# johndpope/SPEAK-hack

Measured on NVIDIA B200. Metric: irfd_train_pairs_per_sec_256, higher is better.
Workload: dtype bf16

## Files before the change

### include/irfd_b200.h

```cpp
#ifndef IRFD_B200_H_
#define IRFD_B200_H_

#include <stddef.h>
#include <stdint.h>

#ifdef __cplusplus
extern "C" {
#endif

#define IRFD_ABI_VERSION 1

#define IRFD_OK 0
#define IRFD_ERR_INVALID_ARGUMENT (-1)
#define IRFD_ERR_CUDA (-2)

typedef struct CUstream_st* irfd_stream_t;

int irfd_abi_version(void);
const char* irfd_last_error(void);

int irfd_conv_gemm_m_tiles(int n, int h, int w);
int irfd_conv_gemm(const void* x, int n, int h, int w, int cin, const void* wk, int cout, int ksize, void* out,
                   void* out2, int mode, const float* bias, const float* nw, const float* noise, const float* sp1,
                   const float* s1, float* stat_sum, float* stat_sq, int force_block_n, irfd_stream_t stream);

int irfd_conv_gemm_style_split(const void* x, int n, int h, int w, int cin, const void* wk, int cout, int ksize,
                               void* out_a, void* out_y, void* out_y_lo, const float* bias, const float* nw,
                               const float* noise, const float* sp1, const float* s1, int force_block_n,
                               irfd_stream_t stream);

int irfd_conv_gemm_grouped(const void* x, int n, int h, int w, int cin, const void* wk, int cout, int ksize, void* out,
                           int mode, float* stat_sum, float* stat_sq, int wgroups, int a_shared, int force_block_n,
                           irfd_stream_t stream);
int irfd_conv_gemm_affine_grouped(const void* x, int n, int h, int w, int cin, const void* wk, int cout, int ksize,
                                  void* out, const float* scale, const float* shift, const void* res, int relu,
                                  int wgroups, int a_shared, int force_block_n, irfd_stream_t stream);

int irfd_conv_gemm_affine(const void* x, int n, int h, int w, int cin, const void* wk, int cout, int ksize, void* out,
                          const float* scale, const float* shift, const void* res, int relu, int force_block_n,
                          irfd_stream_t stream);

long long irfd_wgrad_workspace_bytes(int n, int h, int w, int cin, int cout, int ksize);
int irfd_conv_wgrad(const void* x, const void* dy, int n, int h, int w, int cin, int cout, int ksize, float* dw,
                    float beta, int reduce_cin, int reduce_taps, void* workspace, long long workspace_bytes,
                    irfd_stream_t stream);
long long irfd_wgrad_workspace_bytes_grouped(int n, int h, int w, int cin, int cout, int ksize, int groups);
int irfd_conv_wgrad_grouped(const void* x, const void* dy, int n, int h, int w, int cin, int cout, int ksize,
                            float* const* dw, float beta, int reduce_cin, int reduce_taps, int groups, int x_shared,
                            void* workspace, long long workspace_bytes, irfd_stream_t stream);

int irfd_bn_finalize(const float* psum, const float* psq, int tiles, int c, long long count, float eps, float momentum,
                     float* mean, float* rstd, float* running_mean, float* running_var, int running_updates,
                     int groups, irfd_stream_t stream);
int irfd_bn_eval_rstd(const float* running_var, float eps, float* rstd, int c, irfd_stream_t stream);
int irfd_bn_eval_affine(const float* running_mean, const float* running_var, const float* gamma, const float* beta,
                        float eps, float* scale, float* shift, int c, irfd_stream_t stream);
int irfd_bn_running_update(const float* mean, const float* rstd, float eps, long long count, float momentum,
                           float* running_mean, float* running_var, int c, irfd_stream_t stream);
int irfd_bn_apply(const void* z, const float* mean, const float* rstd, const float* gamma, const float* beta,
                  const void* res, const float* mean2, const float* rstd2, const float* gamma2, const float* beta2,
                  void* out, long long rows, int c, int relu, int groups, irfd_stream_t stream);
long long irfd_bn_bwd_workspace_bytes(long long rows, int c, int groups);
int irfd_bn_backward(const void* g1, const void* g2, const void* act, const void* z, const float* mean,
                     const float* rstd, const float* gamma, const float* beta, void* dz, void* g_out, float* dgamma,
                     float* dbeta, float grad_beta, int batch_stats, long long rows, int c, int groups, void* workspace,
                     long long workspace_bytes, irfd_stream_t stream);

int irfd_bn_eval_affine_sets(const float* const* running_mean, const float* const* running_var,
                             const float* const* gamma, const float* const* beta, float eps, float* scale, float* shift,
                             int c, int nsets, irfd_stream_t stream);
int irfd_bn_finalize_sets(const float* psum, const float* psq, int tiles, int c, long long count, float eps,
                          float momentum, float* mean, float* rstd, float* const* running_mean,
                          float* const* running_var, int running_updates, int groups, int nsets,
                          irfd_stream_t stream);
int irfd_bn_apply_sets(const void* z, const float* mean, const float* rstd, const float* const* gamma,
                       const float* const* beta, const void* res, const float* mean2, const float* rstd2,
                       const float* const* gamma2, const float* const* beta2, void* out, void* mask_bits,
                       long long rows, int c, int relu, int groups, int nsets, irfd_stream_t stream);
int irfd_bn_backward_sets(const void* g1, const void* g2, const void* act, int act_is_bits, const void* z,
                          const float* mean, const float* rstd, const float* const* gamma, const float* const* beta,
                          void* dz, void* g_out, float* const* dgamma, float* const* dbeta, float grad_beta,
                          int batch_stats, long long rows, int c, int groups, int nsets, void* workspace,
                          long long workspace_bytes, irfd_stream_t stream);

int irfd_conv_gemm_bnbwd_grouped(const void* x, int n, int h, int w, int cin, const void* wk, int cout, int ksize,
                                 void* out, const void* bn_z, const float* bn_mean, const float* bn_rstd,
                                 const float* const* bn_gamma, const float* const* bn_beta, float* partial,
                                 int stat_groups, int wgroups, int force_block_n, irfd_stream_t stream);
int irfd_conv_gemm_bnbwd_res_grouped(const void* x, int n, int h, int w, int cin, const void* wk, int cout, int ksize,
                                     void* out, const void* bn_z, const float* bn_mean, const float* bn_rstd,
                                     const void* g2, const void* mask_bits, float* partial, int stat_groups,
                                     int wgroups, int force_block_n, irfd_stream_t stream);
int irfd_bn_backward_finish_sets(const void* g, const void* z, const float* mean, const float* rstd,
                                 const float* const* gamma, void* dz, float* const* dgamma, float* const* dbeta,
                                 float grad_beta, int batch_stats, long long rows, int c, int groups, int nsets,
                                 const float* partial, int tiles, void* workspace, long long workspace_bytes,
                                 irfd_stream_t stream);

int irfd_pack_conv_weight(const float* w, void* dst, int o, int i, int taps, int mode, int kpad, irfd_stream_t stream);
int irfd_im2col_stem(const float* x, void* col, int n, int h, int w, int kpad, irfd_stream_t stream);
int irfd_im2col_3x3s2(const void* a, void* col, int n, int h, int w, int c, irfd_stream_t stream);
int irfd_col2im_3x3s2(const void* dcol, void* dx, int n, int h, int w, int c, irfd_stream_t stream);
int irfd_subsample2(const void* a, void* out, int n, int h, int w, int c, irfd_stream_t stream);
int irfd_scatter_add_s2(const void* a, const void* b, void* out, int n, int h, int w, int c, irfd_stream_t stream);
int irfd_maxpool_fwd(const void* a, void* out, void* argmax, int n, int h, int w, int c, irfd_stream_t stream);
int irfd_maxpool_bwd(const void* dout, const void* dout2, const void* argmax, void* dx, int n, int h, int w, int c,
                     irfd_stream_t stream);
int irfd_avgpool_fwd(const void* a, float* out, int n, int hw, int c, irfd_stream_t stream);
int irfd_avgpool_bwd(const float* dfeat, void* g, int n, int hw, int c, irfd_stream_t stream);
int irfd_nchw_to_nhwc_bf16(const float* in, void* out, int b, int c, int hw, int c_pad, irfd_stream_t stream);
int irfd_nhwc_bf16_to_nchw(const void* in, float* out, int b, int c, int hw, int c_pad, irfd_stream_t stream);

int irfd_const_input_fwd(const float* cst, const float* bias, const float* nw, const float* noise, const float* sp1,
                         const float* s1, void* a0, void* y0, int b, int c, irfd_stream_t stream);
int irfd_const_input_bwd(const void* dy, const void* a0, const float* noise, const float* sp1, float* dsp1, float* ds1,
                         float* dconst, float* dbias, float* dnw, int b, int c, irfd_stream_t stream);
int irfd_upsample2x_fwd(const void* in, void* out, int b, int h, int w, int c, irfd_stream_t stream);
int irfd_upsample2x_split_fwd(const void* in, const void* in_lo, void* out, int b, int h, int w, int c,
                              irfd_stream_t stream);
int irfd_const_input_split_fwd(const float* cst, const float* bias, const float* nw, const float* noise,
                               const float* sp1, const float* s1, void* a0, void* y0, void* y0_lo, int b, int c,
                               irfd_stream_t stream);
int irfd_upsample2x_bwd(const void* dout, void* din, int b, int h, int w, int c, irfd_stream_t stream);
int irfd_apply_noise_nchw(const float* x, const float* w, const float* noise, float* out, int b, int c, int hw,
                          irfd_stream_t stream);
int irfd_apply_style_nchw(const float* x, const float* style, float* out, int b, int c, int hw, irfd_stream_t stream);
long long irfd_style_bwd_workspace_bytes(int b, int hw, int c);
int irfd_style_bwd(const void* dy, const void* a, const float* noise, const float* sp1, void* dz, float* ds1,
                   float* dsp1, float* dbias, float* dnw, int b, int hw, int c, void* workspace,
                   long long workspace_bytes, irfd_stream_t stream);
int irfd_to_rgb_fwd(const void* y, const float* w, const float* bias, float* out, int b, int hw, int c,
                    irfd_stream_t stream);
long long irfd_to_rgb_bwd_workspace_bytes(int b, int hw, int c);
int irfd_to_rgb_bwd(const float* drgb, const void* y, const float* w, void* dy, float* dw, float* dbias, int b, int hw,
                    int c, void* workspace, long long workspace_bytes, irfd_stream_t stream);

int irfd_linear_fwd(const float* x, const float* w, const float* bias, float* y, int b, int n, int k, float wmul,
                    float bmul, int lrelu, irfd_stream_t stream);
int irfd_lrelu_bwd(const float* dy, const float* y, float* dz, long long n, irfd_stream_t stream);
int irfd_linear_bwd(const float* dz, const float* x, const float* w, float* dx, float dx_beta, float* dw, float* db,
                    float dw_beta, int b, int n, int k, float wmul, float bmul, irfd_stream_t stream);
int irfd_softmax_rows(const float* x, float* y, int b, int n, irfd_stream_t stream);
int irfd_scale_copy(const float* src, float* dst, float scale, long long n, irfd_stream_t stream);
int irfd_split_style(const float* style, float* sp1, float* s1, int b, int c, irfd_stream_t stream);
int irfd_merge_style_grad(const float* dsp1, const float* ds1, float* dstyle, int b, int c, irfd_stream_t stream);

int irfd_style_rows_fwd(const float* w, const float* w2, const int* ctrl, int ctrl_idx, float psi, int cutoff,
                        float* rows_t, int l, int b, int k, irfd_stream_t stream);
int irfd_style_rows_pair_fwd(const float* w, const float* w2, const int* ctrl, int ctrl_idx, float psi, int cutoff,
                             float* rows_t, int l, int b, int k, int b_first, irfd_stream_t stream);
int irfd_style_rows_bwd(const float* drows_t, float psi, int cutoff, float* dw, int l, int b, int k,
                        irfd_stream_t stream);
int irfd_swap_cat_fwd(const float* fi_s, const float* fe_s, const float* fp_s, const float* fi_t, const float* fe_t,
                      const float* fp_t, const int* ctrl, float* gen_s, float* gen_t, int b, int c,
                      irfd_stream_t stream);
int irfd_swap_cat_bwd(const float* dgen_s, const float* dgen_t, const int* ctrl, float* dfi_s, float* dfe_s,
                      float* dfp_s, float* dfi_t, float* dfe_t, float* dfp_t, int b, int c, irfd_stream_t stream);

long long irfd_reduce_workspace_bytes(void);
int irfd_mse_fwd(const float* a, const float* b, long long n, float* out, float out_beta, void* workspace,
                 long long workspace_bytes, irfd_stream_t stream);
int irfd_mse_bwd(const float* a, const float* b, long long n, const float* gscale, float* da, float* db,
                 irfd_stream_t stream);
int irfd_sumsq(const float* g, long long n, float* out, float out_beta, void* workspace, long long workspace_bytes,
               irfd_stream_t stream);
int irfd_adam_step(float* p, const float* g, float* m, float* v, long long n, float lr, float beta1, float beta2,
                   float eps, int step, int* step_dev, const float* total_sumsq, float max_norm, irfd_stream_t stream);

int irfd_from_rgb_fwd(const float* x, const float* w, const float* bias, void* out, int b, int hw, int c, int lrelu,
                      irfd_stream_t stream);
long long irfd_bias_lrelu_bwd_workspace_bytes(long long rows, int c);
int irfd_bias_lrelu_bwd(const void* g, const void* y, void* dz, float* dbias, long long rows, int c, void* workspace,
                        long long workspace_bytes, irfd_stream_t stream);

#ifdef __cplusplus
}
#endif
#endif
```

### speak_hack_b200/csrc/conv_gemm.cu

```cuda
#include <stdlib.h>

#include "host_util.h"
#include "ptx.cuh"

namespace irfd {

enum { EPI_PLAIN = 0, EPI_STATS = 1, EPI_STYLE = 2, EPI_AFFINE = 3, EPI_BNBWD = 4, EPI_BNBWD_RES = 5 };

struct ConvGemmArgs {
  int M_total, N_total;
  int num_m_tiles, num_n_tiles;
  int taps, kw, pad, cin_chunks;
  int H, W, HW, B;
  const float* bias;
  const float* nw;
  const float* noise;
  const float* sp1;
  const float* s1;
  float* stat_sum;
  float* stat_sq;
  const __nv_bfloat16* res;
  __nv_bfloat16* y_lo;
  int wg_tiles;
  int a_mod_tiles;
  int relu;
  const __nv_bfloat16* bn_z;
  const __nv_bfloat16* bn_g2;
  const uint8_t* bn_bits;
  const float* bn_mean;
  const float* bn_rstd;
  const float* bn_gamma[4];
  const float* bn_beta[4];
  int sg_tiles;
  int warp_epi;
};

constexpr int kNumThreads = 320;
constexpr int kEpiThreads = 256;
constexpr int kMiscBytes = 12 * 1024;
constexpr int kStgBytes = 16384;
constexpr int kSmemLimit = 232448;

template <int BLOCK_N, int MODE>
struct GemmCfg {
  static constexpr int A_BYTES = 128 * 128;
  static constexpr int B_BYTES = BLOCK_N * 128;
  static constexpr int STAGE_BYTES = A_BYTES + B_BYTES;
  static constexpr int NUM_OUT = (MODE == EPI_STYLE) ? 2 : 1;
  static constexpr int STG_TOTAL = 4 * kStgBytes;
  static constexpr int RAW_STAGES = (kSmemLimit - 1024 - STG_TOTAL - kMiscBytes) / STAGE_BYTES;
  static constexpr int STAGES = RAW_STAGES > 8 ? 8 : RAW_STAGES;
  static constexpr int SMEM_BYTES = 1024 + STAGES * STAGE_BYTES + STG_TOTAL + kMiscBytes;
  static constexpr uint32_t TMEM_COLS = (2 * BLOCK_N <= 128) ? 128 : (2 * BLOCK_N <= 256 ? 256 : 512);
};

template <int BLOCK_N, int MODE, int NBUF>
__device__ __forceinline__ void epilogue_acc(const ConvGemmArgs& p, const CUtensorMap* map_out,
                                             const CUtensorMap* map_out2, uint32_t tmem_base, uint32_t acc_col,
                                             int m0, int n_tile, uint64_t* release_bar, uint8_t* stg_base, float* vec,
                                             uint32_t& chunk_counter) {
  const int warp = threadIdx.x >> 5;
  const int lane = threadIdx.x & 31;
  const int e = warp - 2;
  const int q = warp & 3;
  const int half = e >> 2;
  const int etid = threadIdx.x - 64;
  const int r = q * 32 + lane;
  float* vb = vec;
  float* vnw = vec + 256;
  float* vsp1 = vec + 512;
  float* vs1 = vec + 1024;
  const int m_tile = m0 >> 7;
  const int ng0 = n_tile * BLOCK_N;
  const int pg0 = (m_tile / p.wg_tiles) * p.N_total + ng0;
  float noise_r = 0.f;
  int img_local = 0;
  if constexpr (MODE == EPI_STYLE) {
    const int nimg = p.HW < 128 ? 128 / p.HW : 1;
    const int b0 = m0 / p.HW;
    for (int i = etid; i < BLOCK_N; i += kEpiThreads) {
      vb[i] = p.bias[ng0 + i];
      vnw[i] = p.nw[ng0 + i];
    }
    for (int i = etid; i < nimg * BLOCK_N; i += kEpiThreads) {
      const int img = i / BLOCK_N, c = i - img * BLOCK_N;
      int bb = b0 + img;
      if (bb >= p.B) bb = p.B - 1;
      vsp1[img * 256 + c] = p.sp1[(size_t)bb * p.N_total + ng0 + c];
      vs1[img * 256 + c] = p.s1[(size_t)bb * p.N_total + ng0 + c];
    }
    named_bar_sync(1, kEpiThreads);
    if (m0 + r < p.M_total) noise_r = p.noise[m0 + r];
    img_local = p.HW < 128 ? r / p.HW : 0;
  } else if constexpr (MODE == EPI_PLAIN) {
    if (p.bias != nullptr) {
      for (int i = etid; i < BLOCK_N; i += kEpiThreads) vb[i] = p.bias[pg0 + i];
      named_bar_sync(1, kEpiThreads);
    }
  } else if constexpr (MODE == EPI_AFFINE) {
    for (int i = etid; i < BLOCK_N; i += kEpiThreads) {
      vb[i] = p.bias[pg0 + i];
      vnw[i] = p.nw[pg0 + i];
    }
    named_bar_sync(1, kEpiThreads);
  }
#pragma unroll 1
  for (int chunk = 0; chunk < BLOCK_N / 64; ++chunk, ++chunk_counter) {
    uint32_t v[32];
    uint32_t zw[16];
    uint32_t gw[16];
    uint8_t bw[16];
    if constexpr (MODE == EPI_BNBWD || MODE == EPI_BNBWD_RES) {
      const size_t cell0 = (size_t)(m0 + (etid >> 5) * 16) * p.N_total + ng0 + chunk * 64 + 2 * (etid & 31);
#pragma unroll
      for (int i = 0; i < 16; ++i) {
        zw[i] = __ldg(reinterpret_cast<const uint32_t*>(p.bn_z + cell0 + (size_t)i * p.N_total));
        if constexpr (MODE == EPI_BNBWD_RES) {
          gw[i] = __ldg(reinterpret_cast<const uint32_t*>(p.bn_g2 + cell0 + (size_t)i * p.N_total));
          bw[i] = __ldg(p.bn_bits + ((cell0 + (size_t)i * p.N_total) >> 3));
        }
      }
    }
    const uint32_t taddr = tmem_base + (uint32_t(q * 32) << 16) + acc_col + chunk * 64 + half * 32;
    tmem_ld32(taddr, v);
    tmem_ld_wait();
    if (chunk == BLOCK_N / 64 - 1 && release_bar != nullptr) {
      tc_fence_before();
      __syncwarp();
      if (lane == 0) mbar_arrive(release_bar);
    }
    const int buf = (NBUF == 2) ? (chunk_counter & 1) : 0;
    uint8_t* stg0 = stg_base + buf * kStgBytes;
    uint8_t* stg1 = stg_base + (NBUF + buf) * kStgBytes;
    if (warp == 2) {
      __syncwarp();
      if (elect_one_sync()) tma_store_wait_read<NBUF - 1>();
    }
    named_bar_sync(1, kEpiThreads);
    const int cbase = chunk * 64 + half * 32;
#pragma unroll
    for (int jj = 0; jj < 4; ++jj) {
      float o[8], o2[8];
      float rres[8];
      if constexpr (MODE == EPI_AFFINE) {
        if (p.res != nullptr && m0 + r < p.M_total) {
          const uint4 u = *reinterpret_cast<const uint4*>(p.res + (size_t)(m0 + r) * p.N_total + ng0 + cbase + jj * 8);
          const float2 a0 = unpack_bf16x2(u.x), a1 = unpack_bf16x2(u.y), a2 = unpack_bf16x2(u.z), a3 = unpack_bf16x2(u.w);
          rres[0] = a0.x; rres[1] = a0.y; rres[2] = a1.x; rres[3] = a1.y;
          rres[4] = a2.x; rres[5] = a2.y; rres[6] = a3.x; rres[7] = a3.y;
        } else {
#pragma unroll
          for (int t = 0; t < 8; ++t) rres[t] = 0.f;
        }
      }
#pragma unroll
      for (int t = 0; t < 8; ++t) {
        const int c = cbase + jj * 8 + t;
        float acc = __uint_as_float(v[jj * 8 + t]);
        if constexpr (MODE == EPI_STYLE) {
          float z = acc + vb[c] + vnw[c] * noise_r;
          float a = z > 0.f ? z : 0.2f * z;
          o[t] = a;
          o2[t] = a * vsp1[img_local * 256 + c] + vs1[img_local * 256 + c];
        } else if constexpr (MODE == EPI_PLAIN) {
          o[t] = (p.bias != nullptr) ? acc + vb[c] : acc;
        } else if constexpr (MODE == EPI_AFFINE) {
          const float y = acc * vnw[c] + vb[c] + rres[t];
          o[t] = p.relu == 1 ? fmaxf(y, 0.f) : (p.relu == 2 ? (y > 0.f ? y : 0.2f * y) : y);
        } else {
          o[t] = acc;
        }
      }
      const int j = half * 4 + jj;
      const int phys = j ^ (r & 7);
      uint4 pk;
      pk.x = pack_bf16x2(o[0], o[1]);
      pk.y = pack_bf16x2(o[2], o[3]);
      pk.z = pack_bf16x2(o[4], o[5]);
      pk.w = pack_bf16x2(o[6], o[7]);
      *reinterpret_cast<uint4*>(stg0 + r * 128 + phys * 16) = pk;
      if constexpr (MODE == EPI_STYLE) {
        uint4 pk2;
        pk2.x = pack_bf16x2(o2[0], o2[1]);
        pk2.y = pack_bf16x2(o2[2], o2[3]);
        pk2.z = pack_bf16x2(o2[4], o2[5]);
        pk2.w = pack_bf16x2(o2[6], o2[7]);
        *reinterpret_cast<uint4*>(stg1 + r * 128 + phys * 16) = pk2;
        if (p.y_lo != nullptr && m0 + r < p.M_total) {
          const float2 h0 = unpack_bf16x2(pk2.x), h1 = unpack_bf16x2(pk2.y), h2 = unpack_bf16x2(pk2.z),
                       h3 = unpack_bf16x2(pk2.w);
          uint4 lo;
          lo.x = pack_bf16x2(o2[0] - h0.x, o2[1] - h0.y);
          lo.y = pack_bf16x2(o2[2] - h1.x, o2[3] - h1.y);
          lo.z = pack_bf16x2(o2[4] - h2.x, o2[5] - h2.y);
          lo.w = pack_bf16x2(o2[6] - h3.x, o2[7] - h3.y);
          *reinterpret_cast<uint4*>(p.y_lo + (size_t)(m0 + r) * p.N_total + ng0 + cbase + jj * 8) = lo;
        }
      }
    }
    fence_proxy_async_smem();
    named_bar_sync(1, kEpiThreads);
    if constexpr (MODE == EPI_BNBWD || MODE == EPI_BNBWD_RES) {
      const int pr = etid & 31;
      const int g = etid >> 5;
      const int cc = ng0 + chunk * 64 + 2 * pr;
      const size_t so = (size_t)(m_tile / p.sg_tiles) * p.N_total + cc;
      const float2 mm = __ldg(reinterpret_cast<const float2*>(p.bn_mean + so));
      const float2 rs = __ldg(reinterpret_cast<const float2*>(p.bn_rstd + so));
      float2 ga = make_float2(0.f, 0.f), be = make_float2(0.f, 0.f);
      if constexpr (MODE == EPI_BNBWD) {
        const int grp = m_tile / p.wg_tiles;
        const float* gam =
            grp == 0 ? p.bn_gamma[0] : (grp == 1 ? p.bn_gamma[1] : (grp == 2 ? p.bn_gamma[2] : p.bn_gamma[3]));
        const float* bet = grp == 0 ? p.bn_beta[0] : (grp == 1 ? p.bn_beta[1] : (grp == 2 ? p.bn_beta[2] : p.bn_beta[3]));
        ga = __ldg(reinterpret_cast<const float2*>(gam + cc));
        be = __ldg(reinterpret_cast<const float2*>(bet + cc));
      }
      const int bit0 = (2 * pr) & 7;
      float s0 = 0.f, s1 = 0.f, q0 = 0.f, q1 = 0.f;
#pragma unroll
      for (int i = 0; i < 16; ++i) {
        const int row = g * 16 + i;
        const int phys = (pr >> 2) ^ (row & 7);
        uint32_t* cell = reinterpret_cast<uint32_t*>(stg0 + row * 128 + phys * 16 + (pr & 3) * 4);
        float2 f = unpack_bf16x2(*cell);
        const float2 z = unpack_bf16x2(zw[i]);
        const float x0 = (z.x - mm.x) * rs.x, x1 = (z.y - mm.y) * rs.y;
        if constexpr (MODE == EPI_BNBWD) {
          f.x = (ga.x * x0 + be.x) > 0.f ? f.x : 0.f;
          f.y = (ga.y * x1 + be.y) > 0.f ? f.y : 0.f;
        } else {
          const float2 h = unpack_bf16x2(gw[i]);
          f.x = ((bw[i] >> bit0) & 1) ? f.x + h.x : 0.f;
          f.y = ((bw[i] >> (bit0 + 1)) & 1) ? f.y + h.y : 0.f;
        }
        *cell = pack_bf16x2(f.x, f.y);
        s0 += f.x;
        q0 += f.x * x0;
        s1 += f.y;
        q1 += f.y * x1;
      }
      float* red = vec;
      red[(g * 64 + 2 * pr) * 2 + 0] = s0;
      red[(g * 64 + 2 * pr) * 2 + 1] = q0;
      red[(g * 64 + 2 * pr + 1) * 2 + 0] = s1;
      red[(g * 64 + 2 * pr + 1) * 2 + 1] = q1;
      fence_proxy_async_smem();
      named_bar_sync(1, kEpiThreads);
      if (warp == 2) {
        __syncwarp();
        if (elect_one_sync()) {
          tma_store_2d(map_out, stg0, ng0 + chunk * 64, m0);
          tma_store_commit();
        }
      }
      if (etid < 128) {
        const int ch = etid & 63, which = etid >> 6;
        float acc = 0.f;
#pragma unroll
        for (int gg = 0; gg < 8; ++gg) acc += red[(gg * 64 + ch) * 2 + which];
        p.stat_sum[((size_t)m_tile * 2 + which) * p.N_total + ng0 + chunk * 64 + ch] = acc;
      }
      continue;
    }
    if (warp == 2) {
      __syncwarp();
      if (elect_one_sync()) {
        tma_store_2d(map_out, stg0, ng0 + chunk * 64, m0);
        if constexpr (MODE == EPI_STYLE) tma_store_2d(map_out2, stg1, ng0 + chunk * 64, m0);
        tma_store_commit();
      }
    }
    if constexpr (MODE == EPI_STATS) {
      const int pr = etid & 31;
      const int g = etid >> 5;
      float s0 = 0.f, s1 = 0.f, q0 = 0.f, q1 = 0.f;
#pragma unroll
      for (int i = 0; i < 16; ++i) {
        const int row = g * 16 + i;
        const int phys = (pr >> 2) ^ (row & 7);
        const uint32_t w = *reinterpret_cast<const uint32_t*>(stg0 + row * 128 + phys * 16 + (pr & 3) * 4);
        const float2 f = unpack_bf16x2(w);
        s0 += f.x;
        q0 += f.x * f.x;
        s1 += f.y;
        q1 += f.y * f.y;
      }
      float* red = vec;
      red[(g * 64 + 2 * pr) * 2 + 0] = s0;
      red[(g * 64 + 2 * pr) * 2 + 1] = q0;
      red[(g * 64 + 2 * pr + 1) * 2 + 0] = s1;
      red[(g * 64 + 2 * pr + 1) * 2 + 1] = q1;
      named_bar_sync(1, kEpiThreads);
      if (etid < 128) {
        const int ch = etid & 63, which = etid >> 6;
        float acc = 0.f;
#pragma unroll
        for (int gg = 0; gg < 8; ++gg) acc += red[(gg * 64 + ch) * 2 + which];
        float* dst = which ? p.stat_sq : p.stat_sum;
        dst[(size_t)m_tile * p.N_total + ng0 + chunk * 64 + ch] = acc;
      }
    }
  }
}

constexpr int kSlabBytes = 4096;

template <int BLOCK_N, int MODE>
__device__ __forceinline__ void epilogue_tile_warp(const ConvGemmArgs& p, const CUtensorMap* map_slab, uint32_t tmem_base,
                                                   uint32_t acc_col, int m0, int n_tile, uint64_t* release_bar,
                                                   uint8_t* stg_base, float* vec, uint32_t& chunk_counter,
                                                   uint32_t& my_slabs, bool release_at_leader = false) {
  static_assert(MODE != EPI_STYLE, "STYLE keeps the two-output epilogue");
  auto release = [&]() {
    if (release_at_leader) mbar_arrive_cluster(release_bar, 0);
    else mbar_arrive(release_bar);
  };
  constexpr int CHUNKS = BLOCK_N / 64;
  constexpr bool kSums = MODE == EPI_STATS || MODE == EPI_BNBWD || MODE == EPI_BNBWD_RES;
  const int warp = threadIdx.x >> 5;
  const int lane = threadIdx.x & 31;
  const int e = warp - 2;
  const int q = warp & 3;
  const int h = e >> 2;
  const int m_tile = m0 >> 7;
  const int ng0 = n_tile * BLOCK_N;
  const int pg0 = (m_tile / p.wg_tiles) * p.N_total + ng0;
  const int row = m0 + q * 32 + lane;
  uint8_t* slabs = stg_base + e * 2 * kSlabBytes;
  float* wvec = vec + e * 128;
  const int first = (h - (int)chunk_counter) & 1;
  const int last_mine = first < CHUNKS ? first + 2 * ((CHUNKS - 1 - first) / 2) : -1;
  if (last_mine < 0) {
    __syncwarp();
    if (lane == 0) release();
  }
#pragma unroll 1
  for (int chunk = first; chunk < CHUNKS; chunk += 2) {
    const int cg0 = ng0 + chunk * 64;
    uint32_t zw[32], gw[32];
    uint8_t bw[32];
    if constexpr (MODE == EPI_BNBWD || MODE == EPI_BNBWD_RES) {
      const size_t cell0 = (size_t)(m0 + q * 32) * p.N_total + cg0 + 2 * lane;
#pragma unroll
      for (int i = 0; i < 32; ++i) {
        zw[i] = __ldg(reinterpret_cast<const uint32_t*>(p.bn_z + cell0 + (size_t)i * p.N_total));
        if constexpr (MODE == EPI_BNBWD_RES) {
          gw[i] = __ldg(reinterpret_cast<const uint32_t*>(p.bn_g2 + cell0 + (size_t)i * p.N_total));
          bw[i] = __ldg(p.bn_bits + ((cell0 + (size_t)i * p.N_total) >> 3));
        }
      }
    }
    if constexpr (MODE == EPI_AFFINE || MODE == EPI_PLAIN) {
      if (MODE == EPI_AFFINE || p.bias != nullptr) {
        __syncwarp();
        wvec[lane] = MODE == EPI_AFFINE ? p.nw[pg0 + chunk * 64 + lane] : 0.f;
        wvec[lane + 32] = MODE == EPI_AFFINE ? p.nw[pg0 + chunk * 64 + 32 + lane] : 0.f;
        wvec[64 + lane] = p.bias[pg0 + chunk * 64 + lane];
        wvec[96 + lane] = p.bias[pg0 + chunk * 64 + 32 + lane];
        __syncwarp();
      }
    }
    uint32_t va[32], vb[32];
    const uint32_t taddr = tmem_base + (uint32_t(q * 32) << 16) + acc_col + chunk * 64;
    tmem_ld32(taddr, va);
    tmem_ld32(taddr + 32, vb);
    tmem_ld_wait();
    if (chunk == last_mine) {
      tc_fence_before();
      __syncwarp();
      if (lane == 0) release();
    }
    uint8_t* slab = slabs + (my_slabs & 1) * kSlabBytes;
    if (lane == 0) tma_store_wait_read<1>();
    __syncwarp();
#pragma unroll
    for (int j = 0; j < 8; ++j) {
      float o[8];
#pragma unroll
      for (int t = 0; t < 8; ++t) {
        const int c = j * 8 + t;
        const float acc = __uint_as_float(c < 32 ? va[c & 31] : vb[c & 31]);
        if constexpr (MODE == EPI_AFFINE) o[t] = acc * wvec[c] + wvec[64 + c];
        else if constexpr (MODE == EPI_PLAIN) o[t] = p.bias != nullptr ? acc + wvec[64 + c] : acc;
        else o[t] = acc;
      }
      if constexpr (MODE == EPI_AFFINE) {
        if (p.res != nullptr && row < p.M_total) {
          const uint4 u = *reinterpret_cast<const uint4*>(p.res + (size_t)row * p.N_total + cg0 + j * 8);
          const float2 a0 = unpack_bf16x2(u.x), a1 = unpack_bf16x2(u.y), a2 = unpack_bf16x2(u.z), a3 = unpack_bf16x2(u.w);
          o[0] += a0.x; o[1] += a0.y; o[2] += a1.x; o[3] += a1.y;
          o[4] += a2.x; o[5] += a2.y; o[6] += a3.x; o[7] += a3.y;
        }
#pragma unroll
        for (int t = 0; t < 8; ++t)
          o[t] = p.relu == 1 ? fmaxf(o[t], 0.f) : (p.relu == 2 ? (o[t] > 0.f ? o[t] : 0.2f * o[t]) : o[t]);
      }
      uint4 pk;
      pk.x = pack_bf16x2(o[0], o[1]);
      pk.y = pack_bf16x2(o[2], o[3]);
      pk.z = pack_bf16x2(o[4], o[5]);
      pk.w = pack_bf16x2(o[6], o[7]);
      *reinterpret_cast<uint4*>(slab + lane * 128 + ((j ^ (lane & 7)) << 4)) = pk;
    }
    if constexpr (kSums) {
      __syncwarp();
      float s0 = 0.f, s1 = 0.f, q0 = 0.f, q1 = 0.f;
      if constexpr (MODE == EPI_STATS) {
#pragma unroll
        for (int i = 0; i < 32; ++i) {
          const uint32_t w = *reinterpret_cast<const uint32_t*>(slab + i * 128 + (((lane >> 2) ^ (i & 7)) << 4) + (lane & 3) * 4);
          const float2 f = unpack_bf16x2(w);
          s0 += f.x;
          q0 += f.x * f.x;
          s1 += f.y;
          q1 += f.y * f.y;
        }
      } else {
        const int cc = cg0 + 2 * lane;
        const size_t so = (size_t)(m_tile / p.sg_tiles) * p.N_total + cc;
        const float2 mm = __ldg(reinterpret_cast<const float2*>(p.bn_mean + so));
        const float2 rs = __ldg(reinterpret_cast<const float2*>(p.bn_rstd + so));
        float2 ga = make_float2(0.f, 0.f), be = make_float2(0.f, 0.f);
        if constexpr (MODE == EPI_BNBWD) {
          const int grp = m_tile / p.wg_tiles;
          const float* gam =
              grp == 0 ? p.bn_gamma[0] : (grp == 1 ? p.bn_gamma[1] : (grp == 2 ? p.bn_gamma[2] : p.bn_gamma[3]));
          const float* bet = grp == 0 ? p.bn_beta[0] : (grp == 1 ? p.bn_beta[1] : (grp == 2 ? p.bn_beta[2] : p.bn_beta[3]));
          ga = __ldg(reinterpret_cast<const float2*>(gam + cc));
          be = __ldg(reinterpret_cast<const float2*>(bet + cc));
        }
        const int bit0 = (2 * lane) & 7;
#pragma unroll
        for (int i = 0; i < 32; ++i) {
          uint32_t* cell = reinterpret_cast<uint32_t*>(slab + i * 128 + (((lane >> 2) ^ (i & 7)) << 4) + (lane & 3) * 4);
          float2 f = unpack_bf16x2(*cell);
          const float2 z = unpack_bf16x2(zw[i]);
          const float x0 = (z.x - mm.x) * rs.x, x1 = (z.y - mm.y) * rs.y;
          if constexpr (MODE == EPI_BNBWD) {
            f.x = (ga.x * x0 + be.x) > 0.f ? f.x : 0.f;
            f.y = (ga.y * x1 + be.y) > 0.f ? f.y : 0.f;
          } else {
            const float2 g2 = unpack_bf16x2(gw[i]);
            f.x = ((bw[i] >> bit0) & 1) ? f.x + g2.x : 0.f;
            f.y = ((bw[i] >> (bit0 + 1)) & 1) ? f.y + g2.y : 0.f;
          }
          *cell = pack_bf16x2(f.x, f.y);
          s0 += f.x;
          q0 += f.x * x0;
          s1 += f.y;
          q1 += f.y * x1;
        }
      }
      float* red = vec + ((((my_slabs & 1) * 2 + h) * 4 + q) * 64) * 2;
      *reinterpret_cast<float4*>(red + 4 * lane) = make_float4(s0, q0, s1, q1);
    }
    fence_proxy_async_smem();
    __syncwarp();
    if (lane == 0) {
      tma_store_2d(map_slab, slab, cg0, m0 + q * 32);
      tma_store_commit();
    }
    if constexpr (kSums) {
      named_bar_sync(1 + h, 128);
      if (q == 0) {
        const float* r0 = vec + ((((my_slabs & 1) * 2 + h) * 4) * 64) * 2 + 4 * lane;
        float4 t = *reinterpret_cast<const float4*>(r0);
#pragma unroll
        for (int k = 1; k < 4; ++k) {
          const float4 u = *reinterpret_cast<const float4*>(r0 + k * 128);
          t.x += u.x;
          t.y += u.y;
          t.z += u.z;
          t.w += u.w;
        }
        if constexpr (MODE == EPI_STATS) {
          const size_t d = (size_t)m_tile * p.N_total + cg0 + 2 * lane;
          *reinterpret_cast<float2*>(p.stat_sum + d) = make_float2(t.x, t.z);
          *reinterpret_cast<float2*>(p.stat_sq + d) = make_float2(t.y, t.w);
        } else {
          const size_t d = (size_t)m_tile * 2 * p.N_total + cg0 + 2 * lane;
          *reinterpret_cast<float2*>(p.stat_sum + d) = make_float2(t.x, t.z);
          *reinterpret_cast<float2*>(p.stat_sum + d + p.N_total) = make_float2(t.y, t.w);
        }
      }
    }
    ++my_slabs;
  }
  chunk_counter += CHUNKS;
}

template <int BLOCK_N, int MODE, int CL = 1, bool MMA2 = false>
__global__ void __launch_bounds__(kNumThreads, 1)
conv_gemm_kernel(const __grid_constant__ CUtensorMap map_a, const __grid_constant__ CUtensorMap map_b,
                 const __grid_constant__ CUtensorMap map_out, const __grid_constant__ CUtensorMap map_out2,
                 const ConvGemmArgs p) {
  using Cfg = GemmCfg<BLOCK_N, MODE>;
  constexpr int STAGES = Cfg::STAGES;
  static_assert(STAGES >= 2, "pipeline too shallow");
  static_assert(!MMA2 || (CL == 2 && MODE != EPI_STYLE), "the 2-SM MMA needs a CTA pair and the per-warp epilogue");

  extern __shared__ uint8_t smem_raw[];
  uint8_t* smem = reinterpret_cast<uint8_t*>((reinterpret_cast<uintptr_t>(smem_raw) + 1023) & ~uintptr_t(1023));
  uint8_t* stg_base = smem + STAGES * Cfg::STAGE_BYTES;
  uint8_t* misc = stg_base + Cfg::STG_TOTAL;
  float* vec = reinterpret_cast<float*>(misc);
  uint64_t* full_bar = reinterpret_cast<uint64_t*>(misc + 8192);
  uint64_t* empty_bar = full_bar + STAGES;
  uint64_t* tmem_full = empty_bar + STAGES;
  uint64_t* tmem_empty = tmem_full + 2;
  uint32_t* tmem_ptr = reinterpret_cast<uint32_t*>(tmem_empty + 2);

  const int warp = threadIdx.x >> 5;
  const int lane = threadIdx.x & 31;
  const int crank = CL > 1 ? (int)cluster_ctarank() : 0;
  const int unit0 = blockIdx.x / CL, unit_step = gridDim.x / CL;
  const int total_units = (p.num_m_tiles / CL) * p.num_n_tiles;
  const int num_kb = p.taps * p.cin_chunks;
  constexpr uint16_t kClusterMask = (1u << CL) - 1;

  if (threadIdx.x == 0) {
    for (int i = 0; i < STAGES; ++i) {
      mbar_init(&full_bar[i], 1);
      mbar_init(&empty_bar[i], MMA2 ? 1 : CL);
    }
    for (int i = 0; i < 2; ++i) {
      mbar_init(&tmem_full[i], 1);
      mbar_init(&tmem_empty[i], MMA2 ? 16 : 8);
    }
    fence_mbar_init();
  }
  __syncwarp();
  if (warp == 0) {
    if (MMA2) tmem_alloc_2sm<Cfg::TMEM_COLS>(tmem_ptr);
    else tmem_alloc<Cfg::TMEM_COLS>(tmem_ptr);
  }
  tc_fence_before();
  __syncthreads();
  if (CL > 1) cluster_sync_all();
  tc_fence_after();
  const uint32_t tmem_base = *tmem_ptr;

  if (warp == 0) {
    {
      if (lane == 0) {
        tma_prefetch_desc(&map_a);
        tma_prefetch_desc(&map_b);
      }
      __syncwarp();
      int stage = 0;
      uint32_t phase = 0;
      for (int unit = unit0; unit < total_units; unit += unit_step) {
        const int m_tile = (unit / p.num_n_tiles) * CL + crank;
        const int n_tile = unit % p.num_n_tiles;
        const int m0 = (p.a_mod_tiles > 0 ? m_tile % p.a_mod_tiles : m_tile) * 128;
        const int w0 = m0 % p.W;
        const int h0 = (m0 / p.W) % p.H;
        const int n0 = m0 / (p.W * p.H);
        const int b_row = (m_tile / p.wg_tiles) * p.N_total + n_tile * BLOCK_N;
        for (int tap = 0; tap < p.taps; ++tap) {
          const int dh = tap / p.kw - p.pad;
          const int dw = tap % p.kw - p.pad;
          for (int ch = 0; ch < p.cin_chunks; ++ch) {
            mbar_wait(&empty_bar[stage], phase ^ 1);
            uint8_t* sa = smem + stage * Cfg::STAGE_BYTES;
            if (MMA2) {
              if (elect_one_sync()) {
                if (crank == 0) mbar_expect_tx(&full_bar[stage], 2 * (Cfg::A_BYTES + Cfg::B_BYTES / 2));
                tma_load_4d_2sm(sa, &map_a, &full_bar[stage], ch * 64, w0 + dw, h0 + dh, n0);
                tma_load_2d_2sm(sa + Cfg::A_BYTES, &map_b, &full_bar[stage], (tap * p.cin_chunks + ch) * 64,
                                b_row + crank * (BLOCK_N / 2));
              }
            } else if (elect_one_sync()) {
              mbar_expect_tx(&full_bar[stage], Cfg::STAGE_BYTES);
              tma_load_4d(sa, &map_a, &full_bar[stage], ch * 64, w0 + dw, h0 + dh, n0);
              if (CL == 1)
                tma_load_2d(sa + Cfg::A_BYTES, &map_b, &full_bar[stage], (tap * p.cin_chunks + ch) * 64, b_row);
              else
                tma_load_2d_mc(sa + Cfg::A_BYTES + crank * (Cfg::B_BYTES / CL), &map_b, &full_bar[stage],
                               (tap * p.cin_chunks + ch) * 64, b_row + crank * (BLOCK_N / CL), kClusterMask);
            }
            __syncwarp();
            if (++stage == STAGES) {
              stage = 0;
              phase ^= 1;
            }
          }
        }
      }
    }
  } else if (warp == 1) {
    if (!MMA2 || crank == 0) {
      constexpr uint32_t idesc = make_idesc_bf16(MMA2 ? 256 : 128, BLOCK_N, 0, 0);
      int stage = 0;
      uint32_t phase = 0;
      int iter = 0;
      for (int unit = unit0; unit < total_units; unit += unit_step, ++iter) {
        const int as = iter & 1;
        const uint32_t aphase = (iter >> 1) & 1;
        mbar_wait(&tmem_empty[as], aphase ^ 1);
        tc_fence_after();
        const uint32_t d_tmem = tmem_base + as * BLOCK_N;
        for (int kb = 0; kb < num_kb; ++kb) {
          mbar_wait(&full_bar[stage], phase);
          tc_fence_after();
          const uint32_t a_addr = smem_u32(smem + stage * Cfg::STAGE_BYTES);
          const uint64_t adesc0 = make_smem_desc_sw128(a_addr, 0, 1024);
          const uint64_t bdesc0 = make_smem_desc_sw128(a_addr + Cfg::A_BYTES, 0, 1024);
          if (elect_one_sync()) {
#pragma unroll
            for (int k = 0; k < 4; ++k)
              if (MMA2) umma_bf16_2sm(d_tmem, adesc0 + 2 * k, bdesc0 + 2 * k, idesc, (kb | k) != 0 ? 1u : 0u);
              else umma_bf16(d_tmem, adesc0 + 2 * k, bdesc0 + 2 * k, idesc, (kb | k) != 0 ? 1u : 0u);
            if (MMA2) umma_commit_2sm_mc(&empty_bar[stage], kClusterMask);
            else if (CL == 1) umma_commit(&empty_bar[stage]);
            else umma_commit_mc(&empty_bar[stage], kClusterMask);
          }
          __syncwarp();
          if (++stage == STAGES) {
            stage = 0;
            phase ^= 1;
          }
        }
        if (elect_one_sync()) {
          if (MMA2) umma_commit_2sm_mc(&tmem_full[as], kClusterMask);
          else umma_commit(&tmem_full[as]);
        }
        __syncwarp();
      }
    }
  } else {
    int iter = 0;
    uint32_t chunk_counter = 0, my_slabs = 0;
    for (int unit = unit0; unit < total_units; unit += unit_step, ++iter) {
      const int as = iter & 1;
      const uint32_t aphase = (iter >> 1) & 1;
      const int m_tile = (unit / p.num_n_tiles) * CL + crank;
      const int n_tile = unit % p.num_n_tiles;
      mbar_wait(&tmem_full[as], aphase);
      tc_fence_after();
      if constexpr (MODE != EPI_STYLE) {
        if (p.warp_epi) {
          epilogue_tile_warp<BLOCK_N, MODE>(p, &map_out2, tmem_base, as * BLOCK_N, m_tile * 128, n_tile, &tmem_empty[as],
                                            stg_base, vec, chunk_counter, my_slabs, MMA2);
          continue;
        }
      }
      epilogue_acc<BLOCK_N, MODE, 2>(p, &map_out, &map_out2, tmem_base, as * BLOCK_N, m_tile * 128, n_tile,
                                     &tmem_empty[as], stg_base, vec, chunk_counter);
    }
    if (MODE != EPI_STYLE && p.warp_epi) {
      if (lane == 0) tma_store_wait_read<0>();
    } else if (warp == 2) {
      __syncwarp();
      if (elect_one_sync()) tma_store_wait_read<0>();
    }
  }

  tc_fence_before();
  __syncthreads();
  if (CL > 1) cluster_sync_all();
  if (warp == 0) {
    if (MMA2) tmem_dealloc_2sm<Cfg::TMEM_COLS>(tmem_base);
    else tmem_dealloc<Cfg::TMEM_COLS>(tmem_base);
  }
}


constexpr int kHaloThreads = 352;
constexpr int kHaloCols = 130;
constexpr int kHaloRows = 4;

template <int BLOCK_N, int MODE>
struct HaloCfg {
  static_assert(BLOCK_N == 64 || BLOCK_N == 128, "two double-buffered accumulators need 4 x BLOCK_N <= 512 TMEM columns");
  static constexpr int A_BYTES = kHaloRows * kHaloCols * 128;
  static constexpr int A_STAGES = 2;
  static constexpr int B_BYTES = BLOCK_N * 128;
  static constexpr int NUM_OUT = (MODE == EPI_STYLE) ? 2 : 1;
  static constexpr int NBUF = (NUM_OUT == 2) ? 1 : 2;
  static constexpr int STG_TOTAL = NUM_OUT * NBUF * kStgBytes;
  static constexpr int RAW_B = (kSmemLimit - 1024 - A_STAGES * A_BYTES - STG_TOTAL - kMiscBytes) / B_BYTES;
  static constexpr int B_STAGES = RAW_B > 8 ? 8 : RAW_B;
  static constexpr int SMEM_BYTES = 1024 + A_STAGES * A_BYTES + B_STAGES * B_BYTES + STG_TOTAL + kMiscBytes;
  static constexpr uint32_t TMEM_COLS = 4 * BLOCK_N <= 256 ? 256 : 512;
  static_assert(A_BYTES % 1024 == 0 && B_STAGES >= 2, "halo stage must keep 1024-byte alignment");
};

struct HaloArgs {
  int wsegs, hpairs;
  int total_tiles;
};

template <int BLOCK_N, int MODE>
__global__ void __launch_bounds__(kHaloThreads, 1)
conv_halo_kernel(const __grid_constant__ CUtensorMap map_a, const __grid_constant__ CUtensorMap map_b,
                 const __grid_constant__ CUtensorMap map_out, const __grid_constant__ CUtensorMap map_out2,
                 const ConvGemmArgs p, const HaloArgs hp) {
  using Cfg = HaloCfg<BLOCK_N, MODE>;
  constexpr int BST = Cfg::B_STAGES;
  extern __shared__ uint8_t smem_raw[];
  uint8_t* smem = reinterpret_cast<uint8_t*>((reinterpret_cast<uintptr_t>(smem_raw) + 1023) & ~uintptr_t(1023));
  uint8_t* smem_b = smem + Cfg::A_STAGES * Cfg::A_BYTES;
  uint8_t* stg_base = smem_b + BST * Cfg::B_BYTES;
  uint8_t* misc = stg_base + Cfg::STG_TOTAL;
  float* vec = reinterpret_cast<float*>(misc);
  uint64_t* full_a = reinterpret_cast<uint64_t*>(misc + 8192);
  uint64_t* empty_a = full_a + 2;
  uint64_t* full_b = empty_a + 2;
  uint64_t* empty_b = full_b + BST;
  uint64_t* tmem_full = empty_b + BST;
  uint64_t* tmem_empty = tmem_full + 2;
  uint32_t* tmem_ptr = reinterpret_cast<uint32_t*>(tmem_empty + 2);

  const int warp = threadIdx.x >> 5;
  const int lane = threadIdx.x & 31;
  const int chunks = p.cin_chunks;

  if (threadIdx.x == 0) {
    for (int i = 0; i < 2; ++i) {
      mbar_init(&full_a[i], 1);
      mbar_init(&empty_a[i], 1);
      mbar_init(&tmem_full[i], 1);
      mbar_init(&tmem_empty[i], 8);
    }
    for (int i = 0; i < BST; ++i) {
      mbar_init(&full_b[i], 1);
      mbar_init(&empty_b[i], 1);
    }
    fence_mbar_init();
  }
  __syncwarp();
  if (warp == 0) tmem_alloc<Cfg::TMEM_COLS>(tmem_ptr);
  tc_fence_before();
  __syncthreads();
  tc_fence_after();
  const uint32_t tmem_base = *tmem_ptr;

  auto decode = [&](int tile, int& n_tile, int& n0, int& h0, int& w0) {
    const int m2 = tile / p.num_n_tiles;
    n_tile = tile - m2 * p.num_n_tiles;
    const int wseg = m2 % hp.wsegs;
    const int t = m2 / hp.wsegs;
    const int hpair = t % hp.hpairs;
    n0 = t / hp.hpairs;
    h0 = hpair * 2;
    w0 = wseg * 128;
  };

  if (warp == 0) {
    {
      if (lane == 0) tma_prefetch_desc(&map_a);
      __syncwarp();
      int stage = 0;
      uint32_t phase = 0;
      for (int tile = blockIdx.x; tile < hp.total_tiles; tile += gridDim.x) {
        int n_tile, n0, h0, w0;
        decode(tile, n_tile, n0, h0, w0);
        for (int ch = 0; ch < chunks; ++ch) {
          mbar_wait(&empty_a[stage], phase ^ 1);
          if (elect_one_sync()) {
            mbar_expect_tx(&full_a[stage], Cfg::A_BYTES);
            tma_load_4d(smem + stage * Cfg::A_BYTES, &map_a, &full_a[stage], ch * 64, w0 - 1, h0 - 1, n0);
          }
          __syncwarp();
          if (++stage == Cfg::A_STAGES) {
            stage = 0;
            phase ^= 1;
          }
        }
      }
    }
  } else if (warp == 10) {
    {
      if (lane == 0) tma_prefetch_desc(&map_b);
      __syncwarp();
      int stage = 0;
      uint32_t phase = 0;
      for (int tile = blockIdx.x; tile < hp.total_tiles; tile += gridDim.x) {
        const int n_tile = tile % p.num_n_tiles;
        for (int ch = 0; ch < chunks; ++ch) {
          for (int tap = 0; tap < 9; ++tap) {
            mbar_wait(&empty_b[stage], phase ^ 1);
            if (elect_one_sync()) {
              mbar_expect_tx(&full_b[stage], Cfg::B_BYTES);
              tma_load_2d(smem_b + stage * Cfg::B_BYTES, &map_b, &full_b[stage], (tap * chunks + ch) * 64,
                          n_tile * BLOCK_N);
            }
            __syncwarp();
            if (++stage == BST) {
              stage = 0;
              phase ^= 1;
            }
          }
        }
      }
    }
  } else if (warp == 1) {
    {
      constexpr uint32_t idesc = make_idesc_bf16(128, BLOCK_N, 0, 0);
      int sa = 0, sb = 0;
      uint32_t pa = 0, pb = 0;
      int iter = 0;
      for (int tile = blockIdx.x; tile < hp.total_tiles; tile += gridDim.x, ++iter) {
        const int as = iter & 1;
        const uint32_t aphase = (iter >> 1) & 1;
        mbar_wait(&tmem_empty[as], aphase ^ 1);
        tc_fence_after();
        const uint32_t d_tmem = tmem_base + as * 2 * BLOCK_N;
        for (int ch = 0; ch < chunks; ++ch) {
          mbar_wait(&full_a[sa], pa);
          const uint64_t adesc0 = make_smem_desc_sw128(smem_u32(smem + sa * Cfg::A_BYTES), 0, 1024);
#pragma unroll
          for (int tap = 0; tap < 9; ++tap) {
            constexpr int kLine = 128 / 16;
            const int dy = tap / 3, dx = tap % 3;
            mbar_wait(&full_b[sb], pb);
            tc_fence_after();
            const uint64_t bdesc0 = make_smem_desc_sw128(smem_u32(smem_b + sb * Cfg::B_BYTES), 0, 1024);
            if (elect_one_sync()) {
#pragma unroll
              for (int j = 0; j < 2; ++j) {
#pragma unroll
                for (int k = 0; k < 4; ++k)
                  umma_bf16(d_tmem + j * BLOCK_N, adesc0 + ((j + dy) * kHaloCols + dx) * kLine + 2 * k, bdesc0 + 2 * k,
                            idesc, (tap | k) != 0 ? 1u : (ch != 0 ? 1u : 0u));
              }
              umma_commit(&empty_b[sb]);
            }
            __syncwarp();
            if (++sb == BST) {
              sb = 0;
              pb ^= 1;
            }
          }
          if (elect_one_sync()) umma_commit(&empty_a[sa]);
          __syncwarp();
          if (++sa == Cfg::A_STAGES) {
            sa = 0;
            pa ^= 1;
          }
        }
        if (elect_one_sync()) umma_commit(&tmem_full[as]);
        __syncwarp();
      }
    }
  } else {
    int iter = 0;
    uint32_t chunk_counter = 0;
    for (int tile = blockIdx.x; tile < hp.total_tiles; tile += gridDim.x, ++iter) {
      const int as = iter & 1;
      const uint32_t aphase = (iter >> 1) & 1;
      int n_tile, n0, h0, w0;
      decode(tile, n_tile, n0, h0, w0);
      const int m0 = (n0 * p.H + h0) * p.W + w0;
      mbar_wait(&tmem_full[as], aphase);
      tc_fence_after();
      epilogue_acc<BLOCK_N, MODE, Cfg::NBUF>(p, &map_out, &map_out2, tmem_base, as * 2 * BLOCK_N, m0, n_tile, nullptr,
                                             stg_base, vec, chunk_counter);
      epilogue_acc<BLOCK_N, MODE, Cfg::NBUF>(p, &map_out, &map_out2, tmem_base, as * 2 * BLOCK_N + BLOCK_N, m0 + p.W,
                                             n_tile, &tmem_empty[as], stg_base, vec, chunk_counter);
    }
    if (warp == 2) {
      __syncwarp();
      if (elect_one_sync()) tma_store_wait_read<0>();
    }
  }

  tc_fence_before();
  __syncthreads();
  if (warp == 0) tmem_dealloc<Cfg::TMEM_COLS>(tmem_base);
}

template <int BLOCK_N, int MODE, int CL = 1, bool MMA2 = false>
static int launch_conv_gemm(const CUtensorMap& ma, const CUtensorMap& mb, const CUtensorMap& mo, const CUtensorMap& mo2,
                            const ConvGemmArgs& a, cudaStream_t stream) {
  using Cfg = GemmCfg<BLOCK_N, MODE>;
  static bool configured = false;
  auto kern = conv_gemm_kernel<BLOCK_N, MODE, CL, MMA2>;
  if (!configured) {
    cudaError_t e = cudaFuncSetAttribute(kern, cudaFuncAttributeMaxDynamicSharedMemorySize, Cfg::SMEM_BYTES);
    if (e != cudaSuccess) {
      set_last_error("cudaFuncSetAttribute(smem=%d): %s", Cfg::SMEM_BYTES, cudaGetErrorString(e));
      return IRFD_ERR_CUDA;
    }
    configured = true;
  }
  const int units = (a.num_m_tiles / CL) * a.num_n_tiles;
  const int slots = num_sms() / CL;
  const int grid = (units < slots ? units : slots) * CL;
  if (CL == 1) {
    kern<<<grid, kNumThreads, Cfg::SMEM_BYTES, stream>>>(ma, mb, mo, mo2, a);
  } else {
    cudaLaunchConfig_t cfg = {};
    cfg.gridDim = dim3(grid);
    cfg.blockDim = dim3(kNumThreads);
    cfg.dynamicSmemBytes = Cfg::SMEM_BYTES;
    cfg.stream = stream;
    cudaLaunchAttribute attr[1];
    attr[0].id = cudaLaunchAttributeClusterDimension;
    attr[0].val.clusterDim.x = CL;
    attr[0].val.clusterDim.y = 1;
    attr[0].val.clusterDim.z = 1;
    cfg.attrs = attr;
    cfg.numAttrs = 1;
    cudaLaunchKernelEx(&cfg, kern, ma, mb, mo, mo2, a);
  }
  IRFD_CHECK_LAUNCH();
  return IRFD_OK;
}

template <int MODE>
static int dispatch_block_n(int block_n, const CUtensorMap& ma, const CUtensorMap& mb, const CUtensorMap& mo,
                            const CUtensorMap& mo2, const ConvGemmArgs& a, cudaStream_t stream, int cluster = 1) {
  if constexpr (MODE == EPI_PLAIN || MODE == EPI_STATS || MODE == EPI_BNBWD) {
    if (cluster == 3) {
      if (block_n == 128) return launch_conv_gemm<128, MODE, 2, true>(ma, mb, mo, mo2, a, stream);
      if (block_n == 256) return launch_conv_gemm<256, MODE, 2, true>(ma, mb, mo, mo2, a, stream);
    }
  }
  if (cluster >= 2) {
    if (block_n == 128) return launch_conv_gemm<128, MODE, 2>(ma, mb, mo, mo2, a, stream);
    if (block_n == 256) return launch_conv_gemm<256, MODE, 2>(ma, mb, mo, mo2, a, stream);
  }
  switch (block_n) {
    case 64: return launch_conv_gemm<64, MODE>(ma, mb, mo, mo2, a, stream);
    case 128: return launch_conv_gemm<128, MODE>(ma, mb, mo, mo2, a, stream);
    case 256: return launch_conv_gemm<256, MODE>(ma, mb, mo, mo2, a, stream);
  }
  set_last_error("bad BLOCK_N %d", block_n);
  return IRFD_ERR_INVALID_ARGUMENT;
}


template <int BLOCK_N, int MODE>
static int launch_conv_halo(const CUtensorMap& ma, const CUtensorMap& mb, const CUtensorMap& mo, const CUtensorMap& mo2,
                            const ConvGemmArgs& a, const HaloArgs& h, cudaStream_t stream) {
  using Cfg = HaloCfg<BLOCK_N, MODE>;
  static bool configured = false;
  auto kern = conv_halo_kernel<BLOCK_N, MODE>;
  if (!configured) {
    cudaError_t e = cudaFuncSetAttribute(kern, cudaFuncAttributeMaxDynamicSharedMemorySize, Cfg::SMEM_BYTES);
    if (e != cudaSuccess) {
      set_last_error("cudaFuncSetAttribute(halo smem=%d): %s", Cfg::SMEM_BYTES, cudaGetErrorString(e));
      return IRFD_ERR_CUDA;
    }
    configured = true;
  }
  const int grid = h.total_tiles < num_sms() ? h.total_tiles : num_sms();
  kern<<<grid, kHaloThreads, Cfg::SMEM_BYTES, stream>>>(ma, mb, mo, mo2, a, h);
  IRFD_CHECK_LAUNCH();
  return IRFD_OK;
}

template <int MODE>
static int dispatch_halo(int block_n, const CUtensorMap& ma, const CUtensorMap& mb, const CUtensorMap& mo,
                         const CUtensorMap& mo2, const ConvGemmArgs& a, const HaloArgs& h, cudaStream_t stream) {
  if (block_n == 64) return launch_conv_halo<64, MODE>(ma, mb, mo, mo2, a, h, stream);
  return launch_conv_halo<128, MODE>(ma, mb, mo, mo2, a, h, stream);
}

static int cluster_mode() {
  const char* e = getenv("IRFD_GEMM_CLUSTER");
  return e ? atoi(e) : 0;
}
static int mma2_mode() {
  const char* e = getenv("IRFD_GEMM_2SM");
  return e ? atoi(e) : 0;
}

static int warp_epi_mode() {
  const char* e = getenv("IRFD_WARP_EPI");
  return e ? atoi(e) : 1;
}

static int halo_mode() {
  const char* e = getenv("IRFD_CONV_HALO");
  return e ? atoi(e) : 1;
}

}

using namespace irfd;

extern "C" int irfd_conv_gemm_m_tiles(int n, int h, int w) {
  long long m = (long long)n * h * w;
  return (int)((m + 127) / 128);
}

struct BnBwdFold {
  const void* z;
  const float *mean, *rstd;
  const float* const* gamma;
  const float* const* beta;
  const void* g2;
  const void* bits;
  int stat_groups;
};

static int conv_gemm_impl(const void* x, int n, int h, int w, int cin, const void* wk, int cout, int ksize, void* out,
                          void* out2, void* out_lo, int mode, const float* bias, const float* nw, const float* noise,
                          const float* sp1, const float* s1, float* stat_sum, float* stat_sq, const void* res, int relu,
                          int force_block_n, cudaStream_t stream, int wgroups = 1, int a_shared = 0,
                          const BnBwdFold* fold = nullptr) {
  IRFD_CHECK_ARG(x && wk && out, "conv_gemm: null pointer");
  IRFD_CHECK_ARG(ksize == 1 || ksize == 3, "conv_gemm: ksize must be 1 or 3 (got %d)", ksize);
  IRFD_CHECK_ARG(cin % 64 == 0 && cin > 0, "conv_gemm: Cin must be a multiple of 64 (got %d)", cin);
  IRFD_CHECK_ARG(cout % 64 == 0 && cout > 0, "conv_gemm: Cout must be a multiple of 64 (got %d)", cout);
  IRFD_CHECK_ARG(mode >= 0 && mode <= 5, "conv_gemm: bad mode %d", mode);
  const long long m_total_ll = (long long)n * h * w;
  IRFD_CHECK_ARG(m_total_ll > 0 && m_total_ll < (1ll << 31) - 256, "conv_gemm: bad pixel count");
  const int m_total = (int)m_total_ll;
  IRFD_CHECK_ARG(wgroups == 1 || (wgroups > 1 && m_total_ll % (128ll * wgroups) == 0),
                 "conv_gemm: %d weight groups need a whole number of 128-pixel tiles per group (pixels %lld)", wgroups,
                 m_total_ll);
  IRFD_CHECK_ARG(wgroups == 1 || (mode != EPI_STYLE), "conv_gemm: weight groups are not available in STYLE mode");
  IRFD_CHECK_ARG(!a_shared || (ksize == 1 && wgroups > 1), "conv_gemm: a shared A operand needs ksize 1 and groups > 1");

  int H = h, W = w, NB = n;
  if (ksize == 1) {
    H = 1;
    W = a_shared ? m_total / wgroups : m_total;
    NB = 1;
  }
  int tw, th, tn;
  if (W >= 128) {
    IRFD_CHECK_ARG(ksize == 1 || W % 128 == 0, "conv_gemm: W=%d must be a multiple of 128", W);
    tw = 128; th = 1; tn = 1;
  } else {
    IRFD_CHECK_ARG(128 % W == 0, "conv_gemm: W=%d must divide 128", W);
    tw = W;
    const int rows = 128 / W;
    if (H >= rows) {
      IRFD_CHECK_ARG(H % rows == 0, "conv_gemm: H=%d must be a multiple of %d", H, rows);
      th = rows; tn = 1;
    } else {
      IRFD_CHECK_ARG(rows % H == 0, "conv_gemm: H=%d must divide %d", H, rows);
      th = H; tn = rows / H;
    }
  }

  ConvGemmArgs a;
  a.M_total = m_total;
  a.N_total = cout;
  a.num_m_tiles = (m_total + 127) / 128;
  a.taps = ksize * ksize;
  a.kw = ksize;
  a.pad = ksize / 2;
  a.cin_chunks = cin / 64;
  a.H = H; a.W = W; a.HW = h * w; a.B = n;
  a.bias = bias; a.nw = nw; a.noise = noise; a.sp1 = sp1; a.s1 = s1;
  a.stat_sum = stat_sum; a.stat_sq = stat_sq;
  a.res = reinterpret_cast<const __nv_bfloat16*>(res);
  a.y_lo = reinterpret_cast<__nv_bfloat16*>(out_lo);
  a.wg_tiles = wgroups > 1 ? a.num_m_tiles / wgroups : 0x7fffffff;
  a.a_mod_tiles = a_shared ? a.num_m_tiles / wgroups : 0;
  a.relu = relu;
  if (mode == EPI_AFFINE) IRFD_CHECK_ARG(bias && nw, "conv_gemm: AFFINE mode needs scale and shift");
  if (mode == EPI_STYLE) {
    IRFD_CHECK_ARG(bias && nw && noise && sp1 && s1 && out2, "conv_gemm: STYLE mode needs bias/nw/noise/sp1/s1/out2");
    IRFD_CHECK_ARG(h * w >= 64, "conv_gemm: STYLE mode needs >= 64 pixels per image");
  }
  if (mode == EPI_STATS) IRFD_CHECK_ARG(stat_sum && stat_sq, "conv_gemm: STATS mode needs stat buffers");
  a.warp_epi = (mode != EPI_STYLE && m_total % 128 == 0 && warp_epi_mode() != 0) ? 1 : 0;
  a.bn_z = nullptr;
  a.bn_mean = a.bn_rstd = nullptr;
  for (int i = 0; i < 4; ++i) a.bn_gamma[i] = a.bn_beta[i] = nullptr;
  a.sg_tiles = 0x7fffffff;
  a.bn_g2 = nullptr;
  a.bn_bits = nullptr;
  if (mode == EPI_BNBWD || mode == EPI_BNBWD_RES) {
    IRFD_CHECK_ARG(fold && fold->z && fold->mean && fold->rstd && stat_sum,
                   "conv_gemm: BNBWD modes need z, mean, rstd and the partial buffer");
    if (mode == EPI_BNBWD) IRFD_CHECK_ARG(fold->gamma && fold->beta, "conv_gemm: BNBWD mode needs gamma and beta");
    if (mode == EPI_BNBWD_RES)
      IRFD_CHECK_ARG(fold->g2 && fold->bits && cout % 8 == 0, "conv_gemm: BNBWD_RES mode needs g2 and the mask plane");
    IRFD_CHECK_ARG(wgroups <= 4 && m_total % 128 == 0 && fold->stat_groups >= wgroups &&
                       fold->stat_groups % wgroups == 0 && a.num_m_tiles % fold->stat_groups == 0,
                   "conv_gemm: BNBWD needs whole 128-pixel tiles per statistic group (%d tiles, %d groups, %d sets)",
                   a.num_m_tiles, fold->stat_groups, wgroups);
    a.bn_z = reinterpret_cast<const __nv_bfloat16*>(fold->z);
    a.bn_mean = fold->mean;
    a.bn_rstd = fold->rstd;
    for (int i = 0; i < wgroups && mode == EPI_BNBWD; ++i) {
      IRFD_CHECK_ARG(fold->gamma[i] && fold->beta[i], "conv_gemm: BNBWD gamma/beta pointer %d is null", i);
      a.bn_gamma[i] = fold->gamma[i];
      a.bn_beta[i] = fold->beta[i];
    }
    a.bn_g2 = reinterpret_cast<const __nv_bfloat16*>(fold->g2);
    a.bn_bits = reinterpret_cast<const uint8_t*>(fold->bits);
    a.sg_tiles = a.num_m_tiles / fold->stat_groups;
  }

  int block_n = force_block_n;
  if (block_n == 0) {
    block_n = 64;
    const int cands[3] = {256, 128, 64};
    for (int i = 0; i < 3; ++i) {
      if (cout % cands[i] == 0 && (long long)a.num_m_tiles * (cout / cands[i]) >= num_sms()) {
        block_n = cands[i];
        break;
      }
    }
    if (block_n == 64 && cout % 128 == 0 && (long long)a.num_m_tiles * (cout / 128) * 3 >= 2ll * num_sms()) block_n = 128;
  }
  IRFD_CHECK_ARG((block_n == 64 || block_n == 128 || block_n == 256) && cout % block_n == 0,
                 "conv_gemm: BLOCK_N %d incompatible with Cout %d", block_n, cout);
  const int hmode = halo_mode();
  const bool use_halo = hmode != 0 && mode != EPI_BNBWD && mode != EPI_BNBWD_RES && wgroups == 1 && ksize == 3 && W % 128 == 0 && H % 2 == 0 &&
                        (cout == 64 || cout == 128) &&
                        (force_block_n == 0 || force_block_n == cout);
  if (use_halo) block_n = cout;
  a.num_n_tiles = cout / block_n;
  int cluster = 1;
  if (!use_halo && (cluster_mode() != 0 || mma2_mode() != 0) && block_n >= 128 && a.num_m_tiles % 2 == 0 &&
      (wgroups == 1 || a.wg_tiles % 2 == 0) && (a.a_mod_tiles == 0 || a.a_mod_tiles % 2 == 0))
    cluster = (mma2_mode() != 0 && a.warp_epi && (mode == EPI_PLAIN || mode == EPI_STATS || mode == EPI_BNBWD)) ? 3 : 2;

  CUtensorMap ma, mb, mo, mo2;
  {
    const uint64_t dims[4] = {(uint64_t)cin, (uint64_t)W, (uint64_t)H, (uint64_t)NB};
    const uint64_t str[3] = {(uint64_t)cin * 2, (uint64_t)W * cin * 2, (uint64_t)H * W * cin * 2};
    uint32_t box[4] = {64, (uint32_t)tw, (uint32_t)th, (uint32_t)tn};
    if (use_halo) {
      box[1] = kHaloCols;
      box[2] = kHaloRows;
      box[3] = 1;
    }
    int rc = make_tmap_bf16(&ma, x, 4, dims, str, box, true);
    if (rc) return rc;
  }
  {
    const uint64_t ktot = (uint64_t)a.taps * cin;
    const uint64_t dims[2] = {ktot, (uint64_t)cout * wgroups};
    const uint64_t str[1] = {ktot * 2};
    const uint32_t box[2] = {64, (uint32_t)(block_n / (cluster > 1 ? 2 : 1))};
    int rc = make_tmap_bf16(&mb, wk, 2, dims, str, box, true);
    if (rc) return rc;
  }
  {
    const uint64_t dims[2] = {(uint64_t)cout, (uint64_t)m_total};
    const uint64_t str[1] = {(uint64_t)cout * 2};
    const uint32_t box[2] = {64, 128};
    int rc = make_tmap_bf16(&mo, out, 2, dims, str, box, true);
    if (rc) return rc;
    if (mode == EPI_STYLE) {
      rc = make_tmap_bf16(&mo2, out2 ? out2 : out, 2, dims, str, box, true);
    } else {
      const uint32_t slab_box[2] = {64, 32};
      rc = make_tmap_bf16(&mo2, out, 2, dims, str, slab_box, true);
    }
    if (rc) return rc;
  }
  if (use_halo) {
    HaloArgs hargs;
    hargs.wsegs = W / 128;
    hargs.hpairs = H / 2;
    hargs.total_tiles = NB * hargs.hpairs * hargs.wsegs * a.num_n_tiles;
    switch (mode) {
      case EPI_PLAIN: return dispatch_halo<EPI_PLAIN>(block_n, ma, mb, mo, mo2, a, hargs, stream);
      case EPI_STATS: return dispatch_halo<EPI_STATS>(block_n, ma, mb, mo, mo2, a, hargs, stream);
      case EPI_STYLE: return dispatch_halo<EPI_STYLE>(block_n, ma, mb, mo, mo2, a, hargs, stream);
      case EPI_AFFINE: return dispatch_halo<EPI_AFFINE>(block_n, ma, mb, mo, mo2, a, hargs, stream);
    }
    return IRFD_ERR_INVALID_ARGUMENT;
  }
  switch (mode) {
    case EPI_PLAIN: return dispatch_block_n<EPI_PLAIN>(block_n, ma, mb, mo, mo2, a, stream, cluster);
    case EPI_STATS: return dispatch_block_n<EPI_STATS>(block_n, ma, mb, mo, mo2, a, stream, cluster);
    case EPI_STYLE: return dispatch_block_n<EPI_STYLE>(block_n, ma, mb, mo, mo2, a, stream, cluster);
    case EPI_AFFINE: return dispatch_block_n<EPI_AFFINE>(block_n, ma, mb, mo, mo2, a, stream, cluster);
    case EPI_BNBWD: return dispatch_block_n<EPI_BNBWD>(block_n, ma, mb, mo, mo2, a, stream, cluster);
    case EPI_BNBWD_RES: return dispatch_block_n<EPI_BNBWD_RES>(block_n, ma, mb, mo, mo2, a, stream, cluster);
  }
  return IRFD_ERR_INVALID_ARGUMENT;
}

extern "C" int irfd_conv_gemm(const void* x, int n, int h, int w, int cin, const void* wk, int cout, int ksize,
                              void* out, void* out2, int mode, const float* bias, const float* nw, const float* noise,
                              const float* sp1, const float* s1, float* stat_sum, float* stat_sq, int force_block_n,
                              cudaStream_t stream) {
  IRFD_CHECK_ARG(mode >= 0 && mode <= 2, "conv_gemm: bad mode %d", mode);
  return conv_gemm_impl(x, n, h, w, cin, wk, cout, ksize, out, out2, nullptr, mode, bias, nw, noise, sp1, s1, stat_sum,
                        stat_sq, nullptr, 0, force_block_n, stream);
}

extern "C" int irfd_conv_gemm_style_split(const void* x, int n, int h, int w, int cin, const void* wk, int cout,
                                          int ksize, void* out_a, void* out_y, void* out_y_lo, const float* bias,
                                          const float* nw, const float* noise, const float* sp1, const float* s1,
                                          int force_block_n, cudaStream_t stream) {
  IRFD_CHECK_ARG(out_y_lo != nullptr, "conv_gemm_style_split: out_y_lo is required");
  return conv_gemm_impl(x, n, h, w, cin, wk, cout, ksize, out_a, out_y, out_y_lo, EPI_STYLE, bias, nw, noise, sp1, s1,
                        nullptr, nullptr, nullptr, 0, force_block_n, stream);
}

extern "C" int irfd_conv_gemm_grouped(const void* x, int n, int h, int w, int cin, const void* wk, int cout, int ksize,
                                      void* out, int mode, float* stat_sum, float* stat_sq, int wgroups, int a_shared,
                                      int force_block_n, cudaStream_t stream) {
  IRFD_CHECK_ARG(mode == EPI_PLAIN || mode == EPI_STATS, "conv_gemm_grouped: mode must be 0 (plain) or 1 (stats)");
  return conv_gemm_impl(x, n, h, w, cin, wk, cout, ksize, out, nullptr, nullptr, mode, nullptr, nullptr, nullptr,
                        nullptr, nullptr, stat_sum, stat_sq, nullptr, 0, force_block_n, stream, wgroups, a_shared);
}

extern "C" int irfd_conv_gemm_bnbwd_grouped(const void* x, int n, int h, int w, int cin, const void* wk, int cout,
                                            int ksize, void* out, const void* bn_z, const float* bn_mean,
                                            const float* bn_rstd, const float* const* bn_gamma,
                                            const float* const* bn_beta, float* partial, int stat_groups, int wgroups,
                                            int force_block_n, cudaStream_t stream) {
  IRFD_CHECK_ARG(wgroups >= 1 && wgroups <= 4, "conv_gemm_bnbwd: 1..4 weight groups");
  const BnBwdFold fold{bn_z, bn_mean, bn_rstd, bn_gamma, bn_beta, nullptr, nullptr, stat_groups};
  return conv_gemm_impl(x, n, h, w, cin, wk, cout, ksize, out, nullptr, nullptr, EPI_BNBWD, nullptr, nullptr, nullptr,
                        nullptr, nullptr, partial, nullptr, nullptr, 0, force_block_n, stream, wgroups, 0, &fold);
}

extern "C" int irfd_conv_gemm_bnbwd_res_grouped(const void* x, int n, int h, int w, int cin, const void* wk, int cout,
                                                int ksize, void* out, const void* bn_z, const float* bn_mean,
                                                const float* bn_rstd, const void* g2, const void* mask_bits,
                                                float* partial, int stat_groups, int wgroups, int force_block_n,
                                                cudaStream_t stream) {
  IRFD_CHECK_ARG(wgroups >= 1 && wgroups <= 4, "conv_gemm_bnbwd_res: 1..4 weight groups");
  const BnBwdFold fold{bn_z, bn_mean, bn_rstd, nullptr, nullptr, g2, mask_bits, stat_groups};
  return conv_gemm_impl(x, n, h, w, cin, wk, cout, ksize, out, nullptr, nullptr, EPI_BNBWD_RES, nullptr, nullptr,
                        nullptr, nullptr, nullptr, partial, nullptr, nullptr, 0, force_block_n, stream, wgroups, 0,
                        &fold);
}

extern "C" int irfd_conv_gemm_affine_grouped(const void* x, int n, int h, int w, int cin, const void* wk, int cout,
                                             int ksize, void* out, const float* scale, const float* shift,
                                             const void* res, int relu, int wgroups, int a_shared, int force_block_n,
                                             cudaStream_t stream) {
  return conv_gemm_impl(x, n, h, w, cin, wk, cout, ksize, out, nullptr, nullptr, EPI_AFFINE, shift, scale, nullptr,
                        nullptr, nullptr, nullptr, nullptr, res, relu, force_block_n, stream, wgroups, a_shared);
}

extern "C" int irfd_conv_gemm_affine(const void* x, int n, int h, int w, int cin, const void* wk, int cout, int ksize,
                                     void* out, const float* scale, const float* shift, const void* res, int relu,
                                     int force_block_n, cudaStream_t stream) {
  return conv_gemm_impl(x, n, h, w, cin, wk, cout, ksize, out, nullptr, nullptr, EPI_AFFINE, shift, scale, nullptr, nullptr,
                        nullptr, nullptr, nullptr, res, relu, force_block_n, stream);
}
```

### speak_hack_b200/csrc/host_util.cu

```cuda
#include "host_util.h"

#include <mutex>
#include <unordered_set>

#include <stdarg.h>
#include <string.h>

namespace irfd {

static thread_local char g_last_error[512] = "";

void set_last_error(const char* fmt, ...) {
  va_list ap;
  va_start(ap, fmt);
  vsnprintf(g_last_error, sizeof(g_last_error), fmt, ap);
  va_end(ap);
}

EncodeTiledFn get_encode_tiled() {
  static EncodeTiledFn fn = nullptr;
  if (fn) return fn;
  void* p = nullptr;
  cudaDriverEntryPointQueryResult qres;
  cudaError_t e = cudaGetDriverEntryPoint("cuTensorMapEncodeTiled", &p, cudaEnableDefault, &qres);
  if (e != cudaSuccess || qres != cudaDriverEntryPointSuccess || p == nullptr) {
    set_last_error("cuTensorMapEncodeTiled entry point unavailable: %s", cudaGetErrorString(e));
    return nullptr;
  }
  fn = reinterpret_cast<EncodeTiledFn>(p);
  return fn;
}

int num_sms() {
  static int n = 0;
  if (n) return n;
  int dev = 0;
  cudaGetDevice(&dev);
  cudaDeviceGetAttribute(&n, cudaDevAttrMultiProcessorCount, dev);
  if (n <= 0) n = 148;
  return n;
}

int make_tmap_bf16(CUtensorMap* out, const void* base, int rank, const uint64_t* dims, const uint64_t* strides_bytes,
                   const uint32_t* box, bool swizzle128) {
  EncodeTiledFn enc = get_encode_tiled();
  if (!enc) return IRFD_ERR_CUDA;
  cuuint64_t gdims[5];
  cuuint64_t gstr[4];
  cuuint32_t gbox[5];
  cuuint32_t estr[5];
  for (int i = 0; i < rank; ++i) {
    gdims[i] = dims[i];
    gbox[i] = box[i];
    estr[i] = 1;
  }
  for (int i = 0; i + 1 < rank; ++i) gstr[i] = strides_bytes[i];
  CUresult r = enc(out, CU_TENSOR_MAP_DATA_TYPE_BFLOAT16, (cuuint32_t)rank, const_cast<void*>(base), gdims, gstr, gbox,
                   estr, CU_TENSOR_MAP_INTERLEAVE_NONE,
                   swizzle128 ? CU_TENSOR_MAP_SWIZZLE_128B : CU_TENSOR_MAP_SWIZZLE_NONE,
                   CU_TENSOR_MAP_L2_PROMOTION_L2_256B, CU_TENSOR_MAP_FLOAT_OOB_FILL_NONE);
  if (r != CUDA_SUCCESS) {
    set_last_error("cuTensorMapEncodeTiled failed (CUresult %d) rank=%d dims=[%llu,%llu,%llu,%llu] box=[%u,%u,%u,%u]",
                   (int)r, rank, (unsigned long long)dims[0], (unsigned long long)(rank > 1 ? dims[1] : 0),
                   (unsigned long long)(rank > 2 ? dims[2] : 0), (unsigned long long)(rank > 3 ? dims[3] : 0), box[0],
                   rank > 1 ? box[1] : 0, rank > 2 ? box[2] : 0, rank > 3 ? box[3] : 0);
    return IRFD_ERR_CUDA;
  }
  return IRFD_OK;
}

}

extern "C" const char* irfd_last_error(void) { return irfd::g_last_error; }

namespace irfd {
void prefer_max_shared_carveout(const void* kernel) {
  static std::mutex mu;
  static std::unordered_set<const void*> done;
  std::lock_guard<std::mutex> lock(mu);
  if (done.insert(kernel).second)
    cudaFuncSetAttribute(kernel, cudaFuncAttributePreferredSharedMemoryCarveout, cudaSharedmemCarveoutMaxShared);
}
}

extern "C" int irfd_abi_version(void) { return IRFD_ABI_VERSION; }
```

### speak_hack_b200/csrc/host_util.h

```cpp
#pragma once
#include <cuda.h>
#include <cuda_runtime.h>
#include <stdint.h>
#include <stdio.h>

#include "../../include/irfd_b200.h"

namespace irfd {

typedef CUresult (*EncodeTiledFn)(CUtensorMap*, CUtensorMapDataType, cuuint32_t, void*, const cuuint64_t*,
                                  const cuuint64_t*, const cuuint32_t*, const cuuint32_t*, CUtensorMapInterleave,
                                  CUtensorMapSwizzle, CUtensorMapL2promotion, CUtensorMapFloatOOBfill);

EncodeTiledFn get_encode_tiled();
int num_sms();
void set_last_error(const char* fmt, ...);

int make_tmap_bf16(CUtensorMap* out, const void* base, int rank, const uint64_t* dims, const uint64_t* strides_bytes,
                   const uint32_t* box, bool swizzle128);

void prefer_max_shared_carveout(const void* kernel);

#define IRFD_CHECK_ARG(cond, ...)            \
  do {                                       \
    if (!(cond)) {                           \
      irfd::set_last_error(__VA_ARGS__);     \
      return IRFD_ERR_INVALID_ARGUMENT;      \
    }                                        \
  } while (0)

#define IRFD_CHECK_LAUNCH()                                                        \
  do {                                                                             \
    cudaError_t e__ = cudaGetLastError();                                          \
    if (e__ != cudaSuccess) {                                                      \
      irfd::set_last_error("%s:%d CUDA launch: %s", __FILE__, __LINE__, cudaGetErrorString(e__)); \
      return IRFD_ERR_CUDA;                                                        \
    }                                                                              \
  } while (0)

}
```

### speak_hack_b200/csrc/ptx.cuh

```cuda
#pragma once
#include <cuda.h>
#include <cuda_runtime.h>
#include <cuda_bf16.h>
#include <stdint.h>

namespace irfd {

__device__ __forceinline__ uint32_t smem_u32(const void* p) {
  return static_cast<uint32_t>(__cvta_generic_to_shared(p));
}
__device__ __forceinline__ uint32_t lane_id() { return threadIdx.x & 31u; }

__device__ __forceinline__ bool elect_one_sync() {
  uint32_t pred;
  asm volatile(
      "{\n\t.reg .pred P;\n\t"
      "elect.sync _|P, 0xffffffff;\n\t"
      "selp.u32 %0, 1, 0, P;\n\t}"
      : "=r"(pred));
  return pred != 0;
}

__device__ __forceinline__ void mbar_init(uint64_t* bar, uint32_t count) {
  asm volatile("mbarrier.init.shared::cta.b64 [%0], %1;" ::"r"(smem_u32(bar)), "r"(count) : "memory");
}
__device__ __forceinline__ void fence_mbar_init() {
  asm volatile("fence.mbarrier_init.release.cluster;" ::: "memory");
}
__device__ __forceinline__ void mbar_expect_tx(uint64_t* bar, uint32_t bytes) {
  asm volatile("mbarrier.arrive.expect_tx.shared::cta.b64 _, [%0], %1;" ::"r"(smem_u32(bar)), "r"(bytes)
               : "memory");
}
__device__ __forceinline__ void mbar_arrive(uint64_t* bar) {
  asm volatile("mbarrier.arrive.shared::cta.b64 _, [%0];" ::"r"(smem_u32(bar)) : "memory");
}
__device__ __forceinline__ bool mbar_try_wait(uint64_t* bar, uint32_t parity) {
  uint32_t ok;
  asm volatile(
      "{\n\t.reg .pred p;\n\t"
      "mbarrier.try_wait.parity.shared::cta.b64 p, [%1], %2;\n\t"
      "selp.u32 %0, 1, 0, p;\n\t}"
      : "=r"(ok)
      : "r"(smem_u32(bar)), "r"(parity)
      : "memory");
  return ok != 0;
}
__device__ __forceinline__ void mbar_wait(uint64_t* bar, uint32_t parity) {
  uint32_t spins = 0;
  long long t0 = 0;
  while (!mbar_try_wait(bar, parity)) {
    if ((++spins & 1023u) == 0) {
      const long long now = clock64();
      if (t0 == 0) t0 = now;
      else if (now - t0 > 4000000000ll) __trap();
    }
  }
}

__device__ __forceinline__ void fence_proxy_async_smem() {
  asm volatile("fence.proxy.async.shared::cta;" ::: "memory");
}
__device__ __forceinline__ void named_bar_sync(uint32_t id, uint32_t nthreads) {
  asm volatile("bar.sync %0, %1;" ::"r"(id), "r"(nthreads) : "memory");
}

__device__ __forceinline__ void tma_prefetch_desc(const CUtensorMap* m) {
  asm volatile("prefetch.tensormap [%0];" ::"l"(reinterpret_cast<uint64_t>(m)) : "memory");
}
__device__ __forceinline__ void tma_load_2d(void* dst, const CUtensorMap* m, uint64_t* bar, int c0, int c1) {
  asm volatile(
      "cp.async.bulk.tensor.2d.shared::cluster.global.tile.mbarrier::complete_tx::bytes [%0], [%1, {%3, %4}], [%2];"
      ::"r"(smem_u32(dst)), "l"(reinterpret_cast<uint64_t>(m)), "r"(smem_u32(bar)), "r"(c0), "r"(c1)
      : "memory");
}
__device__ __forceinline__ void tma_load_2d_mc(void* dst, const CUtensorMap* m, uint64_t* bar, int c0, int c1,
                                               uint16_t cta_mask) {
  asm volatile(
      "cp.async.bulk.tensor.2d.shared::cluster.global.mbarrier::complete_tx::bytes.multicast::cluster [%0], [%1, {%3, %4}], "
      "[%2], %5;" ::"r"(smem_u32(dst)),
      "l"(reinterpret_cast<uint64_t>(m)), "r"(smem_u32(bar)), "r"(c0), "r"(c1), "h"(cta_mask)
      : "memory");
}
__device__ __forceinline__ uint32_t cluster_ctarank() {
  uint32_t r;
  asm volatile("mov.u32 %0, %%cluster_ctarank;" : "=r"(r));
  return r;
}
__device__ __forceinline__ void cluster_sync_all() {
  asm volatile("barrier.cluster.arrive.release.aligned;" ::: "memory");
  asm volatile("barrier.cluster.wait.acquire.aligned;" ::: "memory");
}
__device__ __forceinline__ void tma_load_4d(void* dst, const CUtensorMap* m, uint64_t* bar, int c0, int c1, int c2,
                                            int c3) {
  asm volatile(
      "cp.async.bulk.tensor.4d.shared::cluster.global.tile.mbarrier::complete_tx::bytes [%0], [%1, {%3, %4, %5, %6}], "
      "[%2];" ::"r"(smem_u32(dst)),
      "l"(reinterpret_cast<uint64_t>(m)), "r"(smem_u32(bar)), "r"(c0), "r"(c1), "r"(c2), "r"(c3)
      : "memory");
}
__device__ __forceinline__ void tma_store_2d(const CUtensorMap* m, const void* src, int c0, int c1) {
  asm volatile("cp.async.bulk.tensor.2d.global.shared::cta.tile.bulk_group [%0, {%2, %3}], [%1];" ::"l"(
                   reinterpret_cast<uint64_t>(m)),
               "r"(smem_u32(src)), "r"(c0), "r"(c1)
               : "memory");
}
__device__ __forceinline__ void tma_store_commit() { asm volatile("cp.async.bulk.commit_group;" ::: "memory"); }
template <int N>
__device__ __forceinline__ void tma_store_wait_read() {
  asm volatile("cp.async.bulk.wait_group.read %0;" ::"n"(N) : "memory");
}
template <int N>
__device__ __forceinline__ void tma_store_wait_all() {
  asm volatile("cp.async.bulk.wait_group %0;" ::"n"(N) : "memory");
}

template <uint32_t NCOLS>
__device__ __forceinline__ void tmem_alloc(uint32_t* dst_smem) {
  asm volatile("tcgen05.alloc.cta_group::1.sync.aligned.shared::cta.b32 [%0], %1;" ::"r"(smem_u32(dst_smem)),
               "n"(NCOLS)
               : "memory");
  asm volatile("tcgen05.relinquish_alloc_permit.cta_group::1.sync.aligned;" ::: "memory");
}
template <uint32_t NCOLS>
__device__ __forceinline__ void tmem_dealloc(uint32_t taddr) {
  asm volatile("tcgen05.dealloc.cta_group::1.sync.aligned.b32 %0, %1;" ::"r"(taddr), "n"(NCOLS) : "memory");
}
__device__ __forceinline__ void tc_fence_before() { asm volatile("tcgen05.fence::before_thread_sync;" ::: "memory"); }
__device__ __forceinline__ void tc_fence_after() { asm volatile("tcgen05.fence::after_thread_sync;" ::: "memory"); }

__device__ __forceinline__ void umma_bf16(uint32_t tmem_d, uint64_t adesc, uint64_t bdesc, uint32_t idesc,
                                          uint32_t accumulate) {
  asm volatile(
      "{\n\t.reg .pred p;\n\t"
      "setp.ne.b32 p, %4, 0;\n\t"
      "tcgen05.mma.cta_group::1.kind::f16 [%0], %1, %2, %3, p;\n\t}" ::"r"(tmem_d),
      "l"(adesc), "l"(bdesc), "r"(idesc), "r"(accumulate)
      : "memory");
}
template <uint32_t NCOLS>
__device__ __forceinline__ void tmem_alloc_2sm(uint32_t* dst_smem) {
  asm volatile("tcgen05.alloc.cta_group::2.sync.aligned.shared::cta.b32 [%0], %1;" ::"r"(smem_u32(dst_smem)),
               "n"(NCOLS)
               : "memory");
  asm volatile("tcgen05.relinquish_alloc_permit.cta_group::2.sync.aligned;" ::: "memory");
}
template <uint32_t NCOLS>
__device__ __forceinline__ void tmem_dealloc_2sm(uint32_t taddr) {
  asm volatile("tcgen05.dealloc.cta_group::2.sync.aligned.b32 %0, %1;" ::"r"(taddr), "n"(NCOLS) : "memory");
}
__device__ __forceinline__ void umma_bf16_2sm(uint32_t tmem_d, uint64_t adesc, uint64_t bdesc, uint32_t idesc,
                                              uint32_t accumulate) {
  asm volatile(
      "{\n\t.reg .pred p;\n\t"
      "setp.ne.b32 p, %4, 0;\n\t"
      "tcgen05.mma.cta_group::2.kind::f16 [%0], %1, %2, %3, p;\n\t}" ::"r"(tmem_d),
      "l"(adesc), "l"(bdesc), "r"(idesc), "r"(accumulate)
      : "memory");
}
__device__ __forceinline__ void umma_commit_2sm_mc(uint64_t* bar, uint16_t cta_mask) {
  asm volatile("tcgen05.commit.cta_group::2.mbarrier::arrive::one.shared::cluster.multicast::cluster.b64 [%0], %1;" ::"r"(
                   smem_u32(bar)),
               "h"(cta_mask)
               : "memory");
}
constexpr uint32_t kPeerBitMask = 0xFEFFFFFFu;
__device__ __forceinline__ void tma_load_2d_2sm(void* dst, const CUtensorMap* m, uint64_t* bar, int c0, int c1) {
  asm volatile(
      "cp.async.bulk.tensor.2d.cta_group::2.shared::cluster.global.mbarrier::complete_tx::bytes [%0], [%1, {%3, %4}], [%2];"
      ::"r"(smem_u32(dst)), "l"(reinterpret_cast<uint64_t>(m)), "r"(smem_u32(bar) & kPeerBitMask), "r"(c0), "r"(c1)
      : "memory");
}
__device__ __forceinline__ void tma_load_4d_2sm(void* dst, const CUtensorMap* m, uint64_t* bar, int c0, int c1, int c2,
                                                int c3) {
  asm volatile(
      "cp.async.bulk.tensor.4d.cta_group::2.shared::cluster.global.mbarrier::complete_tx::bytes [%0], [%1, {%3, %4, %5, "
      "%6}], [%2];" ::"r"(smem_u32(dst)),
      "l"(reinterpret_cast<uint64_t>(m)), "r"(smem_u32(bar) & kPeerBitMask), "r"(c0), "r"(c1), "r"(c2), "r"(c3)
      : "memory");
}
__device__ __forceinline__ void mbar_arrive_cluster(uint64_t* bar, uint32_t rank) {
  asm volatile(
      "{\n\t.reg .b32 ra;\n\t"
      "mapa.shared::cluster.u32 ra, %0, %1;\n\t"
      "mbarrier.arrive.release.cluster.shared::cluster.b64 _, [ra];\n\t}" ::"r"(smem_u32(bar)),
      "r"(rank)
      : "memory");
}

__device__ __forceinline__ void umma_commit(uint64_t* bar) {
  asm volatile("tcgen05.commit.cta_group::1.mbarrier::arrive::one.shared::cluster.b64 [%0];" ::"r"(smem_u32(bar))
               : "memory");
}
__device__ __forceinline__ void umma_commit_mc(uint64_t* bar, uint16_t cta_mask) {
  asm volatile("tcgen05.commit.cta_group::1.mbarrier::arrive::one.shared::cluster.multicast::cluster.b64 [%0], %1;" ::"r"(
                   smem_u32(bar)),
               "h"(cta_mask)
               : "memory");
}
__device__ __forceinline__ void tmem_ld32(uint32_t taddr, uint32_t (&v)[32]) {
  asm volatile(
      "tcgen05.ld.sync.aligned.32x32b.x32.b32 "
      "{%0, %1, %2, %3, %4, %5, %6, %7, %8, %9, %10, %11, %12, %13, %14, %15, "
      "%16, %17, %18, %19, %20, %21, %22, %23, %24, %25, %26, %27, %28, %29, %30, %31}, [%32];"
      : "=r"(v[0]), "=r"(v[1]), "=r"(v[2]), "=r"(v[3]), "=r"(v[4]), "=r"(v[5]), "=r"(v[6]), "=r"(v[7]), "=r"(v[8]),
        "=r"(v[9]), "=r"(v[10]), "=r"(v[11]), "=r"(v[12]), "=r"(v[13]), "=r"(v[14]), "=r"(v[15]), "=r"(v[16]),
        "=r"(v[17]), "=r"(v[18]), "=r"(v[19]), "=r"(v[20]), "=r"(v[21]), "=r"(v[22]), "=r"(v[23]), "=r"(v[24]),
        "=r"(v[25]), "=r"(v[26]), "=r"(v[27]), "=r"(v[28]), "=r"(v[29]), "=r"(v[30]), "=r"(v[31])
      : "r"(taddr)
      : "memory");
}
__device__ __forceinline__ void tmem_ld_wait() { asm volatile("tcgen05.wait::ld.sync.aligned;" ::: "memory"); }

__host__ __device__ constexpr uint32_t make_idesc_bf16(uint32_t M, uint32_t N, uint32_t a_mn, uint32_t b_mn) {
  return (1u << 4)
         | (1u << 7)
         | (1u << 10)
         | (a_mn << 15) | (b_mn << 16) | ((N >> 3) << 17) | ((M >> 4) << 24);
}
__device__ __forceinline__ uint64_t make_smem_desc_sw128(uint32_t smem_addr, uint32_t lbo, uint32_t sbo) {
  uint64_t d = 0;
  d |= static_cast<uint64_t>((smem_addr >> 4) & 0x3FFFu);
  d |= static_cast<uint64_t>((lbo >> 4) & 0x3FFFu) << 16;
  d |= static_cast<uint64_t>((sbo >> 4) & 0x3FFFu) << 32;
  d |= 1ull << 46;
  d |= 2ull << 61;
  return d;
}

__device__ __forceinline__ uint32_t pack_bf16x2(float lo, float hi) {
  __nv_bfloat162 t = __floats2bfloat162_rn(lo, hi);
  return *reinterpret_cast<uint32_t*>(&t);
}
__device__ __forceinline__ float2 unpack_bf16x2(uint32_t u) {
  __nv_bfloat162 t = *reinterpret_cast<__nv_bfloat162*>(&u);
  return __bfloat1622float2(t);
}
__device__ __forceinline__ float warp_sum(float v) {
#pragma unroll
  for (int o = 16; o > 0; o >>= 1) v += __shfl_xor_sync(0xffffffffu, v, o);
  return v;
}

}
```

### speak_hack_b200/csrc/wgrad_gemm.cu

```cuda
#include <stdlib.h>

#include "host_util.h"
#include "ptx.cuh"

namespace irfd {

struct WgradArgs {
  int M_total, N_total, K_total;
  int num_pairs, num_n_tiles, splits;
  int num_kb, kb_per_split;
  int taps, kw, pad, cin_chunks, num_atoms;
  int H, W;
  float* partial;
  int groups, x_shared;
};

constexpr int kMaxWgGroups = 4;
struct WgDst {
  float* p[kMaxWgGroups];
};

constexpr int kWgThreads = 192;
constexpr int kWgWaves = 1;
constexpr int kWgMinKb = 16;

template <int BLOCK_N>
struct WgCfg {
  static constexpr int A_BYTES = 2 * 8192;
  static constexpr int B_BYTES = (BLOCK_N / 64) * 8192;
  static constexpr int STAGE_BYTES = A_BYTES + B_BYTES;
  static constexpr int RAW_STAGES = (200704 - 1024 - 1024) / STAGE_BYTES;
  static constexpr int STAGES = RAW_STAGES > 8 ? 8 : RAW_STAGES;
  static constexpr int SMEM_BYTES = 1024 + STAGES * STAGE_BYTES + 1024;
  static constexpr uint32_t TMEM_COLS = BLOCK_N <= 64 ? 64 : (BLOCK_N <= 128 ? 128 : 256);
};

template <int BLOCK_N>
__global__ void __launch_bounds__(kWgThreads, 1)
wgrad_gemm_kernel(const __grid_constant__ CUtensorMap map_x, const __grid_constant__ CUtensorMap map_dy,
                  const WgradArgs p) {
  using Cfg = WgCfg<BLOCK_N>;
  constexpr int STAGES = Cfg::STAGES;
  extern __shared__ uint8_t smem_raw[];
  uint8_t* smem = reinterpret_cast<uint8_t*>((reinterpret_cast<uintptr_t>(smem_raw) + 1023) & ~uintptr_t(1023));
  uint64_t* full_bar = reinterpret_cast<uint64_t*>(smem + STAGES * Cfg::STAGE_BYTES);
  uint64_t* empty_bar = full_bar + STAGES;
  uint64_t* done_bar = empty_bar + STAGES;
  uint32_t* tmem_ptr = reinterpret_cast<uint32_t*>(done_bar + 1);

  const int warp = threadIdx.x >> 5;
  const int lane = threadIdx.x & 31;

  int item = blockIdx.x;
  const int split = item % p.splits;
  item /= p.splits;
  const int n_tile = item % p.num_n_tiles;
  item /= p.num_n_tiles;
  const int pair = item % p.num_pairs;
  const int grp = item / p.num_pairs;
  int kb_begin = split * p.kb_per_split;
  int kb_end = kb_begin + p.kb_per_split;
  if (kb_end > p.num_kb) kb_end = p.num_kb;
  const int my_kb = kb_end > kb_begin ? kb_end - kb_begin : 0;
  const int kb_off = grp * p.num_kb;
  const int kb_off_x = p.x_shared ? 0 : kb_off;

  if (threadIdx.x == 0) {
    for (int i = 0; i < STAGES; ++i) {
      mbar_init(&full_bar[i], 1);
      mbar_init(&empty_bar[i], 1);
    }
    mbar_init(done_bar, 1);
    fence_mbar_init();
  }
  __syncwarp();
  if (warp == 0) tmem_alloc<Cfg::TMEM_COLS>(tmem_ptr);
  tc_fence_before();
  __syncthreads();
  tc_fence_after();
  const uint32_t tmem_base = *tmem_ptr;

  if (warp == 0) {
    if (lane == 0) {
      tma_prefetch_desc(&map_x);
      tma_prefetch_desc(&map_dy);
    }
    __syncwarp();
    int atom[2];
    atom[0] = pair * 2;
    atom[1] = pair * 2 + 1 < p.num_atoms ? pair * 2 + 1 : p.num_atoms - 1;
    int dh[2], dw[2], c0[2];
#pragma unroll
    for (int i = 0; i < 2; ++i) {
      const int tap = atom[i] / p.cin_chunks;
      c0[i] = (atom[i] - tap * p.cin_chunks) * 64;
      dh[i] = tap / p.kw - p.pad;
      dw[i] = tap % p.kw - p.pad;
    }
    int stage = 0;
    uint32_t phase = 0;
    for (int kb = kb_begin; kb < kb_end; ++kb) {
      const int p0 = (kb + kb_off) * 64;
      const int px = (kb + kb_off_x) * 64;
      const int w0 = px % p.W;
      const int h0 = (px / p.W) % p.H;
      const int n0 = px / (p.W * p.H);
      mbar_wait(&empty_bar[stage], phase ^ 1);
      uint8_t* sa = smem + stage * Cfg::STAGE_BYTES;
      uint8_t* sb = sa + Cfg::A_BYTES;
      if (elect_one_sync()) {
        mbar_expect_tx(&full_bar[stage], Cfg::STAGE_BYTES);
        tma_load_4d(sa, &map_x, &full_bar[stage], c0[0], w0 + dw[0], h0 + dh[0], n0);
        tma_load_4d(sa + 8192, &map_x, &full_bar[stage], c0[1], w0 + dw[1], h0 + dh[1], n0);
#pragma unroll
        for (int j = 0; j < BLOCK_N / 64; ++j)
          tma_load_2d(sb + j * 8192, &map_dy, &full_bar[stage], n_tile * BLOCK_N + j * 64, p0);
      }
      __syncwarp();
      if (++stage == STAGES) {
        stage = 0;
        phase ^= 1;
      }
    }
  } else if (warp == 1) {
    constexpr uint32_t idesc = make_idesc_bf16(128, BLOCK_N, 1, 1);
    int stage = 0;
    uint32_t phase = 0;
    for (int i = 0; i < my_kb; ++i) {
      mbar_wait(&full_bar[stage], phase);
      tc_fence_after();
      const uint32_t a_addr = smem_u32(smem + stage * Cfg::STAGE_BYTES);
      const uint64_t adesc0 = make_smem_desc_sw128(a_addr, 8192, 1024);
      const uint64_t bdesc0 = make_smem_desc_sw128(a_addr + Cfg::A_BYTES, 8192, 1024);
      if (elect_one_sync()) {
#pragma unroll
        for (int k = 0; k < 4; ++k)
          umma_bf16(tmem_base, adesc0 + 128 * k, bdesc0 + 128 * k, idesc, (i | k) != 0 ? 1u : 0u);
        umma_commit(&empty_bar[stage]);
      }
      __syncwarp();
      if (++stage == STAGES) {
        stage = 0;
        phase ^= 1;
      }
    }
    if (elect_one_sync()) umma_commit(done_bar);
    __syncwarp();
  } else {
    const int q = warp & 3;
    const int r = q * 32 + lane;
    const int atom_i = r >> 6;
    const bool valid = (pair * 2 + atom_i) < p.num_atoms;
    const size_t krow = (size_t)pair * 128 + r;
    float* dst = p.partial + (((size_t)grp * p.splits + split) * p.K_total + krow) * p.N_total + (size_t)n_tile * BLOCK_N;
    if (my_kb > 0) {
      mbar_wait(done_bar, 0);
      tc_fence_after();
    }
#pragma unroll 1
    for (int chunk = 0; chunk < BLOCK_N / 32; ++chunk) {
      uint32_t v[32];
      if (my_kb > 0) {
        tmem_ld32(tmem_base + (uint32_t(q * 32) << 16) + chunk * 32, v);
        tmem_ld_wait();
      } else {
#pragma unroll
        for (int t = 0; t < 32; ++t) v[t] = 0u;
      }
      if (valid) {
#pragma unroll
        for (int t = 0; t < 8; ++t) {
          float4 o = make_float4(__uint_as_float(v[4 * t]), __uint_as_float(v[4 * t + 1]),
                                 __uint_as_float(v[4 * t + 2]), __uint_as_float(v[4 * t + 3]));
          *reinterpret_cast<float4*>(dst + chunk * 32 + 4 * t) = o;
        }
      }
    }
  }
  tc_fence_before();
  __syncthreads();
  if (warp == 0) tmem_dealloc<Cfg::TMEM_COLS>(tmem_base);
}

template <int LANES>
__global__ void __launch_bounds__(256)
wgrad_reduce_kernel(const float* __restrict__ partial, WgDst dws, int splits, int K_total, int N_total, int cin,
                    int taps, float beta) {
  constexpr int OUTS = 256 / LANES;
  float* __restrict__ dw = dws.p[blockIdx.y];
  partial += (size_t)blockIdx.y * splits * K_total * N_total;
  __shared__ float part[LANES][OUTS + 1];
  const int o = threadIdx.x % OUTS, w = threadIdx.x / OUTS;
  const size_t idx = (size_t)blockIdx.x * OUTS + o;
  const size_t stride = (size_t)K_total * N_total;
  const bool in_range = idx < stride;
  float a0 = 0.f, a1 = 0.f, a2 = 0.f, a3 = 0.f;
  if (in_range) {
    const float* p = partial + idx;
    int s = w;
    for (; s + 3 * LANES < splits; s += 4 * LANES) {
      a0 += __ldg(p + (size_t)s * stride);
      a1 += __ldg(p + (size_t)(s + LANES) * stride);
      a2 += __ldg(p + (size_t)(s + 2 * LANES) * stride);
      a3 += __ldg(p + (size_t)(s + 3 * LANES) * stride);
    }
    for (; s < splits; s += LANES) a0 += __ldg(p + (size_t)s * stride);
  }
  float acc = (a0 + a1) + (a2 + a3);
  if (LANES > 1) {
    part[w][o] = acc;
    __syncthreads();
    if (w != 0) return;
    acc = 0.f;
#pragma unroll
    for (int i = 0; i < LANES; ++i) acc += part[i][o];
  }
  if (!in_range) return;
  const int n = (int)(idx % N_total);
  const int k = (int)(idx / N_total);
  if (k >= cin * taps) return;
  const int tap = k / cin, c = k - tap * cin;
  float* d = dw + ((size_t)n * cin + c) * taps + tap;
  *d = (beta != 0.f) ? beta * (*d) + acc : acc;
}

template <int TAPS>
__global__ void __launch_bounds__(256)
wgrad_reduce_transpose_kernel(const float* __restrict__ partial, WgDst dws, int splits, int K_total, int N_total,
                              int cin, float beta) {
  constexpr int ROW = 32 * TAPS;
  float* __restrict__ dw = dws.p[blockIdx.z];
  partial += (size_t)blockIdx.z * splits * K_total * N_total;
  __shared__ float tile[32][ROW + 1];
  const int tx = threadIdx.x & 31, ty = threadIdx.x >> 5;
  const int n0 = blockIdx.x * 32, c0 = blockIdx.y * 32;
  const size_t stride = (size_t)K_total * N_total;
  for (int i0 = ty; i0 < ROW; i0 += 32) {
    const float* p[4];
    float acc[4] = {0.f, 0.f, 0.f, 0.f};
#pragma unroll
    for (int u = 0; u < 4; ++u) {
      const int i = i0 + 8 * u, tap = i >> 5, cl = i & 31;
      p[u] = partial + ((size_t)tap * cin + c0 + cl) * N_total + n0 + tx;
    }
    for (int sidx = 0; sidx < splits; ++sidx) {
#pragma unroll
      for (int u = 0; u < 4; ++u) acc[u] += __ldg(p[u] + (size_t)sidx * stride);
    }
#pragma unroll
    for (int u = 0; u < 4; ++u) {
      const int i = i0 + 8 * u;
      tile[tx][(i & 31) * TAPS + (i >> 5)] = acc[u];
    }
  }
  __syncthreads();
  for (int r = ty; r < 32; r += 8) {
    float* d = dw + ((size_t)(n0 + r) * cin + c0) * TAPS;
    for (int j = tx; j < ROW; j += 32) d[j] = (beta != 0.f) ? beta * d[j] + tile[r][j] : tile[r][j];
  }
}

static void launch_wgrad_reduce(const float* partial, const WgDst& dws, int groups, int splits, int K_total, int N_total,
                                int cin, int taps, float beta, cudaStream_t stream) {
  const size_t total = (size_t)K_total * N_total;
  const bool tileable = cin % 32 == 0 && N_total % 32 == 0 && K_total == cin * taps && (taps == 9 || taps == 1);
  if (splits <= 6 && tileable && total >= (size_t)1 << 18) {
    const dim3 grid(N_total / 32, cin / 32, groups);
    if (taps == 9)
      wgrad_reduce_transpose_kernel<9><<<grid, 256, 0, stream>>>(partial, dws, splits, K_total, N_total, cin, beta);
    else
      wgrad_reduce_transpose_kernel<1><<<grid, 256, 0, stream>>>(partial, dws, splits, K_total, N_total, cin, beta);
    return;
  }
  if (splits <= 6)
    wgrad_reduce_kernel<1><<<dim3((unsigned)((total + 255) / 256), groups), 256, 0, stream>>>(
        partial, dws, splits, K_total, N_total, cin, taps, beta);
  else if (splits <= 24)
    wgrad_reduce_kernel<4><<<dim3((unsigned)((total + 63) / 64), groups), 256, 0, stream>>>(
        partial, dws, splits, K_total, N_total, cin, taps, beta);
  else
    wgrad_reduce_kernel<8><<<dim3((unsigned)((total + 31) / 32), groups), 256, 0, stream>>>(
        partial, dws, splits, K_total, N_total, cin, taps, beta);
}

struct WgHaloArgs {
  int N_total, K_total, cin;
  int chunks, num_n_tiles, splits;
  int num_kb, kb_per_split;
  int H, W, TH, TW, P;
  int hblocks, wsegs;
  int spr_shift;
  int a_tx_bytes;
  float* partial;
  int groups;
};

constexpr int kWhA = 50176;
constexpr int kWhB = 16384;
constexpr int kWhStages = 3;
constexpr int kWhSmem = 1024 + kWhStages * (kWhA + kWhB) + 1024;

__global__ void __launch_bounds__(kWgThreads, 1)
wgrad_halo_kernel(const __grid_constant__ CUtensorMap map_x, const __grid_constant__ CUtensorMap map_dy,
                  const WgHaloArgs p) {
  extern __shared__ uint8_t smem_raw[];
  uint8_t* smem = reinterpret_cast<uint8_t*>((reinterpret_cast<uintptr_t>(smem_raw) + 1023) & ~uintptr_t(1023));
  uint64_t* full_bar = reinterpret_cast<uint64_t*>(smem + kWhStages * (kWhA + kWhB));
  uint64_t* empty_bar = full_bar + kWhStages;
  uint64_t* done_bar = empty_bar + kWhStages;
  uint32_t* tmem_ptr = reinterpret_cast<uint32_t*>(done_bar + 1);

  const int warp = threadIdx.x >> 5;
  const int lane = threadIdx.x & 31;

  int item = blockIdx.x;
  const int split = item % p.splits;
  item /= p.splits;
  const int n_tile = item % p.num_n_tiles;
  item /= p.num_n_tiles;
  const int chunk = item % p.chunks;
  const int grp = item / p.chunks;
  const int kb_begin = split * p.kb_per_split;
  int kb_end = kb_begin + p.kb_per_split;
  if (kb_end > p.num_kb) kb_end = p.num_kb;
  const int my_kb = kb_end > kb_begin ? kb_end - kb_begin : 0;
  const int kb_off = grp * p.num_kb;

  if (threadIdx.x == 0) {
    for (int i = 0; i < kWhStages; ++i) {
      mbar_init(&full_bar[i], 1);
      mbar_init(&empty_bar[i], 1);
    }
    mbar_init(done_bar, 1);
    fence_mbar_init();
  }
  __syncwarp();
  if (warp == 0) tmem_alloc<512>(tmem_ptr);
  tc_fence_before();
  __syncthreads();
  tc_fence_after();
  const uint32_t tmem_base = *tmem_ptr;

  if (warp == 0) {
    if (lane == 0) {
      tma_prefetch_desc(&map_x);
      tma_prefetch_desc(&map_dy);
    }
    __syncwarp();
    int stage = 0;
    uint32_t phase = 0;
    for (int kbl = kb_begin; kbl < kb_end; ++kbl) {
      const int kb = kbl + kb_off;
      const int wseg = kb % p.wsegs;
      const int t = kb / p.wsegs;
      const int hb = t % p.hblocks;
      const int n0 = t / p.hblocks;
      const int h0 = hb * p.TH, w0 = wseg * p.TW;
      const int m0 = (n0 * p.H + h0) * p.W + w0;
      mbar_wait(&empty_bar[stage], phase ^ 1);
      uint8_t* sa = smem + stage * (kWhA + kWhB);
      if (elect_one_sync()) {
        mbar_expect_tx(&full_bar[stage], p.a_tx_bytes + kWhB);
        tma_load_4d(sa, &map_x, &full_bar[stage], chunk * 64, w0 - 1, h0 - 1, n0);
        tma_load_2d(sa + kWhA, &map_dy, &full_bar[stage], n_tile * 64, m0);
      }
      __syncwarp();
      if (++stage == kWhStages) {
        stage = 0;
        phase ^= 1;
      }
    }
  } else if (warp == 1) {
    constexpr uint32_t idesc = make_idesc_bf16(128, 64, 1, 1);
    const uint32_t P = (uint32_t)p.P;
    const uint32_t off[5] = {0u, 2u, P + 1u, 2u * P, 2u * P + 2u};
    const uint32_t lbo[5] = {1u, P - 2u, 1u, 1u, 1u};
    const uint32_t spr_mask = (1u << p.spr_shift) - 1u;
    int stage = 0;
    uint32_t phase = 0;
    for (int i = 0; i < my_kb; ++i) {
      mbar_wait(&full_bar[stage], phase);
      tc_fence_after();
      const uint32_t a_addr = smem_u32(smem + stage * (kWhA + kWhB));
      const uint64_t bdesc0 = make_smem_desc_sw128(a_addr + kWhA, 8192, 1024);
      uint64_t adesc[5];
#pragma unroll
      for (int q = 0; q < 5; ++q) adesc[q] = make_smem_desc_sw128(a_addr + off[q] * 128u, lbo[q] * 128u, 1024);
      if (elect_one_sync()) {
#pragma unroll
        for (int ks = 0; ks < 8; ++ks) {
          const uint32_t r = (uint32_t)ks >> p.spr_shift, sg = (uint32_t)ks & spr_mask;
          const uint64_t a_step = (uint64_t)((r * P + sg * 16u) * 8u);
#pragma unroll
          for (int q = 0; q < 5; ++q)
            umma_bf16(tmem_base + q * 64, adesc[q] + a_step, bdesc0 + 128 * ks, idesc, (i | ks) != 0 ? 1u : 0u);
        }
        umma_commit(&empty_bar[stage]);
      }
      __syncwarp();
      if (++stage == kWhStages) {
        stage = 0;
        phase ^= 1;
      }
    }
    if (elect_one_sync()) umma_commit(done_bar);
    __syncwarp();
  } else {
    const int q4 = warp & 3;
    const int ci = (q4 & 1) * 32 + lane;
    if (my_kb > 0) {
      mbar_wait(done_bar, 0);
      tc_fence_after();
    }
#pragma unroll 1
    for (int pr = 0; pr < 5; ++pr) {
      const int tap = 2 * pr + (q4 >> 1);
      const size_t krow = (size_t)tap * p.cin + (size_t)chunk * 64 + ci;
      float* dst = p.partial + (((size_t)grp * p.splits + split) * p.K_total + krow) * p.N_total + (size_t)n_tile * 64;
#pragma unroll 1
      for (int half = 0; half < 2; ++half) {
        uint32_t v[32];
        if (my_kb > 0) {
          tmem_ld32(tmem_base + (uint32_t(q4 * 32) << 16) + pr * 64 + half * 32, v);
          tmem_ld_wait();
        } else {
#pragma unroll
          for (int t = 0; t < 32; ++t) v[t] = 0u;
        }
        if (tap < 9) {
#pragma unroll
          for (int t = 0; t < 8; ++t) {
            float4 o = make_float4(__uint_as_float(v[4 * t]), __uint_as_float(v[4 * t + 1]),
                                   __uint_as_float(v[4 * t + 2]), __uint_as_float(v[4 * t + 3]));
            *reinterpret_cast<float4*>(dst + half * 32 + 4 * t) = o;
          }
        }
      }
    }
  }
  tc_fence_before();
  __syncthreads();
  if (warp == 0) tmem_dealloc<512>(tmem_base);
}

static int grouped_splits(int base_per_group, int groups, int num_kb, int max_splits) {
  const int sms = num_sms();
  if (max_splits < 1) max_splits = 1;
  int fit = sms / (base_per_group * groups);
  if (fit >= 1) return fit < max_splits ? fit : max_splits;
  int best = 1;
  long long best_cost = -1;
  for (int s = 1; s <= max_splits && s <= 8; ++s) {
    const long long ctas = (long long)base_per_group * groups * s;
    const long long waves = (ctas + sms - 1) / sms;
    const long long cost = waves * ((num_kb + s - 1) / s) * 16 + s;
    if (best_cost < 0 || cost < best_cost) {
      best_cost = cost;
      best = s;
    }
  }
  return best;
}

static bool wgrad_halo_plan(int n, int h, int w, int cin, int cout, int ksize, WgHaloArgs* a, int groups = 1) {
  const char* e = getenv("IRFD_WGRAD_HALO");
  if (e && atoi(e) == 0) return false;
  if (ksize != 3 || w < 16 || w % 16 != 0 || cin % 64 != 0 || cout % 64 != 0) return false;
  if (!(e && atoi(e) == 2) && (cout > 128 || w < 64)) return false;
  int TW, TH;
  if (w >= 128) {
    if (w % 128 != 0) return false;
    TW = 128;
    TH = 1;
  } else {
    if (128 % w != 0 || h % (128 / w) != 0) return false;
    TW = w;
    TH = 128 / w;
  }
  a->N_total = cout;
  a->K_total = 9 * cin;
  a->cin = cin;
  a->chunks = cin / 64;
  a->num_n_tiles = cout / 64;
  a->H = h; a->W = w; a->TH = TH; a->TW = TW; a->P = TW + 2;
  a->hblocks = h / TH;
  a->wsegs = w / TW;
  a->num_kb = n * a->hblocks * a->wsegs;
  int spr = TW / 16, sh = 0;
  while ((1 << sh) < spr) ++sh;
  a->spr_shift = sh;
  a->a_tx_bytes = (TH + 2) * (TW + 2) * 128;
  a->groups = groups;
  const int base = a->chunks * a->num_n_tiles;
  int splits;
  if (groups == 1) {
    splits = num_sms() / base;
    if (splits > a->num_kb) splits = a->num_kb;
    if (splits < 1) splits = 1;
  } else {
    splits = grouped_splits(base, groups, a->num_kb, a->num_kb);
  }
  a->kb_per_split = (a->num_kb + splits - 1) / splits;
  a->splits = (a->num_kb + a->kb_per_split - 1) / a->kb_per_split;
  return true;
}

template <int BLOCK_N>
static int launch_wgrad(const CUtensorMap& mx, const CUtensorMap& mdy, const WgradArgs& a, cudaStream_t stream) {
  using Cfg = WgCfg<BLOCK_N>;
  static bool configured = false;
  auto kern = wgrad_gemm_kernel<BLOCK_N>;
  if (!configured) {
    cudaError_t e = cudaFuncSetAttribute(kern, cudaFuncAttributeMaxDynamicSharedMemorySize, Cfg::SMEM_BYTES);
    if (e != cudaSuccess) {
      set_last_error("cudaFuncSetAttribute(smem=%d): %s", Cfg::SMEM_BYTES, cudaGetErrorString(e));
      return IRFD_ERR_CUDA;
    }
    configured = true;
  }
  const int grid = a.groups * a.num_pairs * a.num_n_tiles * a.splits;
  kern<<<grid, kWgThreads, Cfg::SMEM_BYTES, stream>>>(mx, mdy, a);
  IRFD_CHECK_LAUNCH();
  return IRFD_OK;
}

static void wgrad_plan(int n, int h, int w, int cin, int cout, int ksize, WgradArgs* a, int* block_n, int groups = 1) {
  const long long m_total = (long long)n * h * w;
  a->groups = groups;
  a->x_shared = 0;
  a->M_total = (int)m_total;
  a->N_total = cout;
  a->taps = ksize * ksize;
  a->kw = ksize;
  a->pad = ksize / 2;
  a->cin_chunks = cin / 64;
  a->K_total = a->taps * cin;
  a->num_atoms = a->taps * a->cin_chunks;
  a->num_pairs = (a->num_atoms + 1) / 2;
  *block_n = cout % 256 == 0 ? 256 : (cout % 128 == 0 ? 128 : 64);
  a->num_n_tiles = cout / *block_n;
  a->num_kb = (int)((m_total + 63) / 64);
  const int base = a->num_pairs * a->num_n_tiles;
  const int max_splits = (a->num_kb + kWgMinKb - 1) / kWgMinKb;
  int splits;
  if (groups == 1) {
    splits = (kWgWaves * num_sms()) / base;
    if (splits > max_splits) splits = max_splits;
    if (splits < 1) splits = 1;
  } else {
    splits = grouped_splits(base, groups, a->num_kb, max_splits);
  }
  a->kb_per_split = (a->num_kb + splits - 1) / splits;
  a->splits = (a->num_kb + a->kb_per_split - 1) / a->kb_per_split;
}

}

using namespace irfd;

static long long wgrad_ws_bytes(int n_g, int h, int w, int cin, int cout, int ksize, int groups) {
  WgHaloArgs ha;
  if (wgrad_halo_plan(n_g, h, w, cin, cout, ksize, &ha, groups))
    return (long long)groups * ha.splits * ha.K_total * ha.N_total * 4;
  WgradArgs a;
  int bn;
  wgrad_plan(n_g, h, w, cin, cout, ksize, &a, &bn, groups);
  return (long long)groups * a.splits * a.K_total * a.N_total * 4;
}

extern "C" long long irfd_wgrad_workspace_bytes(int n, int h, int w, int cin, int cout, int ksize) {
  return wgrad_ws_bytes(n, h, w, cin, cout, ksize, 1);
}

extern "C" long long irfd_wgrad_workspace_bytes_grouped(int n, int h, int w, int cin, int cout, int ksize, int groups) {
  if (groups < 1 || groups > kMaxWgGroups) return -1;
  if (n % groups == 0) return wgrad_ws_bytes(n / groups, h, w, cin, cout, ksize, groups);
  return wgrad_ws_bytes(1, 1, (int)(((long long)n * h * w) / groups), cin, cout, ksize, groups);
}

static int conv_wgrad_impl(const void* x, const void* dy, int n, int h, int w, int cin, int cout, int ksize,
                           const WgDst& dws, int groups, int x_shared, float beta, int reduce_cin, int reduce_taps,
                           void* workspace, long long workspace_bytes, cudaStream_t stream) {
  IRFD_CHECK_ARG(x && dy && workspace, "conv_wgrad: null pointer");
  IRFD_CHECK_ARG(ksize == 1 || ksize == 3, "conv_wgrad: ksize must be 1 or 3");
  IRFD_CHECK_ARG(cin % 64 == 0 && cout % 64 == 0, "conv_wgrad: channels must be multiples of 64");
  IRFD_CHECK_ARG(!x_shared || ksize == 1, "conv_wgrad: a shared x operand needs ksize 1");
  const long long m_group = (long long)n * h * w;
  IRFD_CHECK_ARG(groups == 1 || m_group % 128 == 0, "conv_wgrad: grouped launches need 128-pixel multiples per group");
  WgHaloArgs ha;
  if (!x_shared && wgrad_halo_plan(n, h, w, cin, cout, ksize, &ha, groups)) {
    IRFD_CHECK_ARG(workspace_bytes >= (long long)groups * ha.splits * ha.K_total * ha.N_total * 4,
                   "conv_wgrad: workspace too small");
    ha.partial = reinterpret_cast<float*>(workspace);
    CUtensorMap mx, mdy;
    {
      const uint64_t dims[4] = {(uint64_t)cin, (uint64_t)w, (uint64_t)h, (uint64_t)n * groups};
      const uint64_t str[3] = {(uint64_t)cin * 2, (uint64_t)w * cin * 2, (uint64_t)h * w * cin * 2};
      const uint32_t box[4] = {64, (uint32_t)(ha.TW + 2), (uint32_t)(ha.TH + 2), 1};
      int rc = make_tmap_bf16(&mx, x, 4, dims, str, box, true);
      if (rc) return rc;
    }
    {
      const uint64_t dims[2] = {(uint64_t)cout, (uint64_t)(m_group * groups)};
      const uint64_t str[1] = {(uint64_t)cout * 2};
      const uint32_t box[2] = {64, 128};
      int rc = make_tmap_bf16(&mdy, dy, 2, dims, str, box, true);
      if (rc) return rc;
    }
    static bool configured = false;
    if (!configured) {
      cudaError_t e = cudaFuncSetAttribute(wgrad_halo_kernel, cudaFuncAttributeMaxDynamicSharedMemorySize, kWhSmem);
      if (e != cudaSuccess) {
        set_last_error("cudaFuncSetAttribute(wgrad halo smem=%d): %s", kWhSmem, cudaGetErrorString(e));
        return IRFD_ERR_CUDA;
      }
      configured = true;
    }
    wgrad_halo_kernel<<<groups * ha.chunks * ha.num_n_tiles * ha.splits, kWgThreads, kWhSmem, stream>>>(mx, mdy, ha);
    IRFD_CHECK_LAUNCH();
    launch_wgrad_reduce(ha.partial, dws, groups, ha.splits, ha.K_total, ha.N_total, reduce_cin > 0 ? reduce_cin : cin,
                        reduce_cin > 0 ? reduce_taps : 9, beta, stream);
    IRFD_CHECK_LAUNCH();
    return IRFD_OK;
  }
  WgradArgs a;
  int block_n;
  wgrad_plan(n, h, w, cin, cout, ksize, &a, &block_n, groups);
  a.x_shared = x_shared;
  IRFD_CHECK_ARG(workspace_bytes >= (long long)groups * a.splits * a.K_total * a.N_total * 4,
                 "conv_wgrad: workspace too small");
  a.partial = reinterpret_cast<float*>(workspace);

  const int xg = x_shared ? 1 : groups;
  int H = h, W = w, NB = n * xg;
  if (ksize == 1) {
    H = 1; W = (int)(m_group * xg); NB = 1;
  }
  int tw, th, tn;
  if (W >= 64) {
    IRFD_CHECK_ARG(ksize == 1 || W % 64 == 0, "conv_wgrad: W=%d must be a multiple of 64", W);
    tw = 64; th = 1; tn = 1;
  } else {
    IRFD_CHECK_ARG(64 % W == 0, "conv_wgrad: W=%d must divide 64", W);
    tw = W;
    const int rows = 64 / W;
    if (H >= rows) {
      IRFD_CHECK_ARG(H % rows == 0, "conv_wgrad: H=%d must be a multiple of %d", H, rows);
      th = rows; tn = 1;
    } else {
      IRFD_CHECK_ARG(rows % H == 0, "conv_wgrad: H=%d must divide %d", H, rows);
      th = H; tn = rows / H;
    }
  }
  a.H = H; a.W = W;

  CUtensorMap mx, mdy;
  {
    const uint64_t dims[4] = {(uint64_t)cin, (uint64_t)W, (uint64_t)H, (uint64_t)NB};
    const uint64_t str[3] = {(uint64_t)cin * 2, (uint64_t)W * cin * 2, (uint64_t)H * W * cin * 2};
    const uint32_t box[4] = {64, (uint32_t)tw, (uint32_t)th, (uint32_t)tn};
    int rc = make_tmap_bf16(&mx, x, 4, dims, str, box, true);
    if (rc) return rc;
  }
  {
    const uint64_t dims[2] = {(uint64_t)cout, (uint64_t)(m_group * groups)};
    const uint64_t str[1] = {(uint64_t)cout * 2};
    const uint32_t box[2] = {64, 64};
    int rc = make_tmap_bf16(&mdy, dy, 2, dims, str, box, true);
    if (rc) return rc;
  }
  int rc;
  switch (block_n) {
    case 64: rc = launch_wgrad<64>(mx, mdy, a, stream); break;
    case 128: rc = launch_wgrad<128>(mx, mdy, a, stream); break;
    default: rc = launch_wgrad<256>(mx, mdy, a, stream); break;
  }
  if (rc) return rc;
  launch_wgrad_reduce(a.partial, dws, groups, a.splits, a.K_total, a.N_total, reduce_cin > 0 ? reduce_cin : cin,
                      reduce_cin > 0 ? reduce_taps : a.taps, beta, stream);
  IRFD_CHECK_LAUNCH();
  return IRFD_OK;
}

extern "C" int irfd_conv_wgrad(const void* x, const void* dy, int n, int h, int w, int cin, int cout, int ksize,
                               float* dw, float beta, int reduce_cin, int reduce_taps, void* workspace,
                               long long workspace_bytes, cudaStream_t stream) {
  IRFD_CHECK_ARG(dw != nullptr, "conv_wgrad: null pointer");
  WgDst dws;
  for (int i = 0; i < kMaxWgGroups; ++i) dws.p[i] = i == 0 ? dw : nullptr;
  return conv_wgrad_impl(x, dy, n, h, w, cin, cout, ksize, dws, 1, 0, beta, reduce_cin, reduce_taps, workspace,
                         workspace_bytes, stream);
}

extern "C" int irfd_conv_wgrad_grouped(const void* x, const void* dy, int n, int h, int w, int cin, int cout, int ksize,
                                       float* const* dw, float beta, int reduce_cin, int reduce_taps, int groups,
                                       int x_shared, void* workspace, long long workspace_bytes, cudaStream_t stream) {
  IRFD_CHECK_ARG(dw != nullptr && groups >= 1 && groups <= kMaxWgGroups, "conv_wgrad_grouped: 1..4 groups");
  WgDst dws;
  for (int i = 0; i < kMaxWgGroups; ++i) dws.p[i] = i < groups ? dw[i] : nullptr;
  for (int i = 0; i < groups; ++i) IRFD_CHECK_ARG(dws.p[i] != nullptr, "conv_wgrad_grouped: null gradient pointer");
  int ng = n, hg = h, wg = w;
  if (n % groups == 0) {
    ng = n / groups;
  } else {
    IRFD_CHECK_ARG(n == 1 && h == 1 && w % groups == 0, "conv_wgrad_grouped: rows do not split into groups");
    wg = w / groups;
  }
  return conv_wgrad_impl(x, dy, ng, hg, wg, cin, cout, ksize, dws, groups, x_shared, beta, reduce_cin, reduce_taps,
                         workspace, workspace_bytes, stream);
}
```

### speak_hack_b200/encoder_group.py

```python
from __future__ import annotations

import os
from typing import Dict, List, Optional

import torch
import torch.nn as nn

from . import ops
from .encoder import BN_EPS, BN_MOMENTUM, ResNet50Encoder


fold_bn_reduce = os.environ.get("IRFD_BN_FOLD", "1") != "0"
fold_bn3_reduce = os.environ.get("IRFD_BN3_FOLD", "0") != "0"


def _stack_pack(convs, mode, kpad=0):
    return ops.pack_conv_weights_stacked([c.weight for c in convs], mode, kpad)


class _Stats:
    __slots__ = ("mean", "rstd")

    def __init__(self, mean, rstd):
        self.mean, self.rstd = mean, rstd


def _group_inference(grp: "EncoderGroup", x, col0=None):
    encs = grp.encoders
    E = len(encs)
    x = x.contiguous().to(torch.float32)
    n, _, h, w = x.shape
    if col0 is None:
        col0 = ops.im2col_stem(x, 192)
    sc, sh = ops.bn_eval_affine_sets([e[1] for e in encs])
    a0 = ops.conv_gemm_affine_grouped(col0, _stack_pack([e[0] for e in encs], ops.PACK_FLAT, 192), 1, sc, sh, relu=True,
                                      wgroups=E, a_shared=True).view(E * n, h // 2, w // 2, 64)
    cur, _ = ops.maxpool_fwd(a0)
    for li in range(4, 8):
        for bi in range(len(encs[0][li])):
            blks = [e[li][bi] for e in encs]
            nb, hh, ww, _cin = cur.shape
            sc, sh = ops.bn_eval_affine_sets([b.bn1 for b in blks])
            a1 = ops.conv_gemm_affine_grouped(cur, _stack_pack([b.conv1 for b in blks], ops.PACK_FPROP), 1, sc, sh,
                                              relu=True, wgroups=E)
            planes = a1.shape[-1]
            sc, sh = ops.bn_eval_affine_sets([b.bn2 for b in blks])
            wk2 = _stack_pack([b.conv2 for b in blks], ops.PACK_FPROP)
            if blks[0].stride == 1:
                a2 = ops.conv_gemm_affine_grouped(a1, wk2, 3, sc, sh, relu=True, wgroups=E)
            else:
                col2 = ops.im2col_3x3s2(a1)
                a2 = ops.conv_gemm_affine_grouped(col2.view(1, 1, col2.shape[0], 9 * planes), wk2, 1, sc, sh, relu=True,
                                                  wgroups=E).view(nb, hh // 2, ww // 2, planes)
            if blks[0].downsample is not None:
                xs = ops.subsample2(cur) if blks[0].stride == 2 else cur
                sc, sh = ops.bn_eval_affine_sets([b.downsample[1] for b in blks])
                idn = ops.conv_gemm_affine_grouped(xs, _stack_pack([b.downsample[0] for b in blks], ops.PACK_FPROP), 1,
                                                   sc, sh, relu=False, wgroups=E)
            else:
                idn = cur
            sc, sh = ops.bn_eval_affine_sets([b.bn3 for b in blks])
            cur = ops.conv_gemm_affine_grouped(a2, _stack_pack([b.conv3 for b in blks], ops.PACK_FPROP), 1, sc, sh,
                                               res=idn, relu=True, wgroups=E)
    return ops.avgpool_fwd(cur).view(E, n, -1, 1, 1)


class _EncoderGroupFn(torch.autograd.Function):

    @staticmethod
    def forward(ctx, x, grp, stat_groups, col0, recorded, *params):
        encs: List[ResNet50Encoder] = grp.encoders
        E = len(encs)
        G = stat_groups
        GT = E * G
        U = 2 if (recorded and all(getattr(e, "_recompute_bn_update", False) for e in encs)) else 1
        x = x.contiguous().to(torch.float32)
        n, _, h, w = x.shape

        def stats(bns, s, q, rows_total):
            mean, rstd = ops.bn_finalize_sets(s, q, rows_total // GT, BN_EPS, BN_MOMENTUM,
                                              [b.running_mean for b in bns], [b.running_var for b in bns], U, G, E)
            return _Stats(mean, rstd)

        def apply(z, st, bns, relu=True, res=None, bn2=None, want_mask=False):
            return ops.bn_apply_sets(z, st.mean, st.rstd, [b.weight for b in bns], [b.bias for b in bns], res=res,
                                     bn2=bn2, relu=relu, groups=GT, want_mask=want_mask)

        S = {}
        if col0 is None:
            col0 = ops.im2col_stem(x, 192)
        bn0 = [e[1] for e in encs]
        z0, s, q = ops.conv_gemm_grouped(col0, _stack_pack([e[0] for e in encs], ops.PACK_FLAT, 192), 1, ops.EPI_STATS,
                                         wgroups=E, a_shared=True)
        h1, w1 = h // 2, w // 2
        z0 = z0.view(E * n, h1, w1, 64)
        st0 = stats(bn0, s, q, E * n * h1 * w1)
        a0 = apply(z0, st0, bn0)
        cur, arg0 = ops.maxpool_fwd(a0)
        S["stem"] = (col0, z0, st0, a0, arg0)
        S["blocks"] = []
        for li in range(4, 8):
            for bi in range(len(encs[0][li])):
                blks = [e[li][bi] for e in encs]
                xin = cur
                nb, hh, ww, _cin = xin.shape
                z1, s, q = ops.conv_gemm_grouped(xin, _stack_pack([b.conv1 for b in blks], ops.PACK_FPROP), 1,
                                                 ops.EPI_STATS, wgroups=E)
                bn1 = [b.bn1 for b in blks]
                st1 = stats(bn1, s, q, nb * hh * ww)
                a1 = apply(z1, st1, bn1)
                planes = a1.shape[-1]
                wk2 = _stack_pack([b.conv2 for b in blks], ops.PACK_FPROP)
                col2 = None
                if blks[0].stride == 1:
                    z2, s, q = ops.conv_gemm_grouped(a1, wk2, 3, ops.EPI_STATS, wgroups=E)
                    ho, wo = hh, ww
                else:
                    col2 = ops.im2col_3x3s2(a1)
                    ho, wo = hh // 2, ww // 2
                    z2, s, q = ops.conv_gemm_grouped(col2.view(1, 1, col2.shape[0], 9 * planes), wk2, 1, ops.EPI_STATS,
                                                     wgroups=E)
                    z2 = z2.view(nb, ho, wo, planes)
                bn2 = [b.bn2 for b in blks]
                st2 = stats(bn2, s, q, nb * ho * wo)
                a2 = apply(z2, st2, bn2)
                z3, s, q = ops.conv_gemm_grouped(a2, _stack_pack([b.conv3 for b in blks], ops.PACK_FPROP), 1,
                                                 ops.EPI_STATS, wgroups=E)
                bn3 = [b.bn3 for b in blks]
                st3 = stats(bn3, s, q, nb * ho * wo)
                xs = zd = std = None
                if blks[0].downsample is not None:
                    xs = ops.subsample2(xin) if blks[0].stride == 2 else xin
                    zd, s, q = ops.conv_gemm_grouped(xs, _stack_pack([b.downsample[0] for b in blks], ops.PACK_FPROP), 1,
                                                     ops.EPI_STATS, wgroups=E)
                    dbn = [b.downsample[1] for b in blks]
                    std = stats(dbn, s, q, nb * ho * wo)
                    out = apply(z3, st3, bn3, res=zd, want_mask=recorded,
                                bn2=(std.mean, std.rstd, [b.weight for b in dbn], [b.bias for b in dbn]))
                else:
                    out = apply(z3, st3, bn3, res=xin, want_mask=recorded)
                out, obits = out if recorded else (out, None)
                S["blocks"].append((li, blks, xin, z1, st1, a1, col2, z2, st2, a2, z3, st3, xs, zd, std, obits))
                cur = out
        feat = ops.avgpool_fwd(cur)
        counters = [c for e in encs for c in e._bn_counters()]
        torch._foreach_add_(counters, G * U)
        S["final_hw"] = (cur.shape[1], cur.shape[2])
        ctx.grp, ctx.S, ctx.G = grp, S, G
        return feat.view(E, n, -1, 1, 1)

    @staticmethod
    def backward(ctx, dfeat):
        grp, S, G = ctx.grp, ctx.S, ctx.G
        encs = grp.encoders
        E = len(encs)
        GT = E * G
        cb = grp._bwd_cb
        ops.side_stream(dfeat.device).join()
        if cb is not None:
            cb("pre", None)
        targets: Optional[Dict[nn.Parameter, torch.Tensor]] = grp.grad_targets
        grads = {}
        dfeat = dfeat.contiguous().view(dfeat.shape[0] * dfeat.shape[1], -1).to(torch.float32)
        fh, fw = S["final_hw"]
        g, g2 = ops.avgpool_bwd(dfeat, fh, fw), None

        def tgt(p):
            if targets is not None:
                return targets[p]
            t = torch.empty_like(p, dtype=torch.float32)
            grads[p] = t
            return t

        def bn_bwd(bns, st, g1, g2_, act, z, want_g_out=False, mask_from_z=False, act_bits=None):
            r = ops.bn_backward_sets(g1, g2_, None if mask_from_z else act, z, st.mean, st.rstd,
                                     [b.weight for b in bns], [b.bias for b in bns] if mask_from_z else None,
                                     dgammas=[tgt(b.weight) for b in bns], dbetas=[tgt(b.bias) for b in bns],
                                     want_g_out=want_g_out, batch_stats=True, groups=GT, act_bits=act_bits)
            return (r[0], r[3]) if want_g_out else r[0]

        def dgrad_bn(dy, convs, ksize, bns, st, z):
            wk = _stack_pack(convs, ops.PACK_DGRAD)
            if not fold_bn_reduce:
                d_a = ops.conv_gemm_grouped(dy, wk, ksize, wgroups=E)
                return lambda: bn_bwd(bns, st, d_a, None, None, z, mask_from_z=True)
            gm, part = ops.conv_gemm_bnbwd_grouped(dy, wk, ksize, z, st.mean, st.rstd, [b.weight for b in bns],
                                                   [b.bias for b in bns], GT)
            return lambda: ops.bn_backward_finish_sets(gm, z, st.mean, st.rstd, [b.weight for b in bns], part,
                                                       dgammas=[tgt(b.weight) for b in bns],
                                                       dbetas=[tgt(b.bias) for b in bns], groups=GT)[0]

        side = ops.side_stream(dfeat.device)

        def wgrad(convs, xx, dy, ksize, **kw):
            dws = [tgt(c.weight) for c in convs]
            side.launch(lambda: ops.conv_wgrad_grouped(xx, dy, ksize, dws, **kw), xx, dy, *dws)

        cur_li = None
        pre = None
        blocks = S["blocks"]
        for bidx in range(len(blocks) - 1, -1, -1):
            li, blks, xin, z1, st1, a1, col2, z2, st2, a2, z3, st3, xs, zd, std, obits = blocks[bidx]
            if cur_li is not None and li != cur_li and cb is not None:
                cb("stage", cur_li)
            cur_li = li
            nb, hh, ww, _cin = xin.shape
            planes = a1.shape[-1]
            if pre is not None:
                gmask, part3 = pre
                bn3 = [b.bn3 for b in blks]
                dz3 = ops.bn_backward_finish_sets(gmask, z3, st3.mean, st3.rstd, [b.weight for b in bn3], part3,
                                                  dgammas=[tgt(b.weight) for b in bn3],
                                                  dbetas=[tgt(b.bias) for b in bn3], groups=GT)[0]
                pre = None
            else:
                dz3, gmask = bn_bwd([b.bn3 for b in blks], st3, g, g2, None, z3, want_g_out=True, act_bits=obits)
            finish = dgrad_bn(dz3, [b.conv3 for b in blks], 1, [b.bn2 for b in blks], st2, z2)
            wgrad([b.conv3 for b in blks], a2, dz3, 1)
            dz2 = finish()
            if blks[0].stride == 1:
                finish = dgrad_bn(dz2, [b.conv2 for b in blks], 3, [b.bn1 for b in blks], st1, z1)
                wgrad([b.conv2 for b in blks], a1, dz2, 3)
                dz1 = finish()
            else:
                m2 = dz2.numel() // planes
                dcol = ops.conv_gemm_grouped(dz2.view(1, 1, m2, planes),
                                             _stack_pack([b.conv2 for b in blks], ops.PACK_DCOL), 1, wgroups=E)
                wgrad([b.conv2 for b in blks], col2, dz2.view(m2, planes), 1, reduce_cin=planes, reduce_taps=9)
                d_a1 = ops.col2im_3x3s2(dcol.view(m2, 9 * planes), nb, hh, ww, planes)
                dz1 = bn_bwd([b.bn1 for b in blks], st1, d_a1, None, a1, z1, mask_from_z=True)
            wk1 = _stack_pack([b.conv1 for b in blks], ops.PACK_DGRAD)
            if blks[0].downsample is None and fold_bn3_reduce:
                prev = blocks[bidx - 1]
                pre = ops.conv_gemm_bnbwd_res_grouped(dz1, wk1, 1, prev[10], prev[11].mean, prev[11].rstd, gmask,
                                                      prev[15], GT, wgroups=E)
                wgrad([b.conv1 for b in blks], xin, dz1, 1)
                continue
            d_in = ops.conv_gemm_grouped(dz1, wk1, 1, wgroups=E)
            wgrad([b.conv1 for b in blks], xin, dz1, 1)
            if blks[0].downsample is not None:
                dzd = bn_bwd([b.downsample[1] for b in blks], std, gmask, None, None, zd)
                d_xs = ops.conv_gemm_grouped(dzd, _stack_pack([b.downsample[0] for b in blks], ops.PACK_DGRAD), 1,
                                             wgroups=E)
                wgrad([b.downsample[0] for b in blks], xs, dzd, 1)
                if blks[0].stride == 2:
                    g, g2 = ops.scatter_add_s2(d_in, d_xs), None
                else:
                    g, g2 = d_in, d_xs
            else:
                g, g2 = d_in, gmask
        if cb is not None and cur_li is not None:
            cb("stage", cur_li)
        col0, z0, st0, a0, arg0 = S["stem"]
        d_a0 = ops.maxpool_bwd(g, arg0, g2)
        dz0 = bn_bwd([e[1] for e in encs], st0, d_a0, None, a0, z0, mask_from_z=True)
        wgrad([e[0] for e in encs], col0, dz0.view(-1, 64), 1, x_shared=True, reduce_cin=147, reduce_taps=1)
        side.join()
        if cb is not None:
            cb("stage", 3)
            cb("post", None)
        ctx.S = None
        if targets is not None:
            return (None,) * (5 + sum(len(e._flat_params()) for e in encs))
        return (None, None, None, None, None) + tuple(grads.get(p) for e in encs for p in e._flat_params())


class EncoderGroup:

    def __init__(self, encoders: List[ResNet50Encoder]):
        self.encoders = list(encoders)
        self.grad_targets: Optional[Dict[nn.Parameter, torch.Tensor]] = None
        self._bwd_cb = None

    def can_run(self, x: torch.Tensor, groups: int) -> bool:
        encs = self.encoders
        if not (x.is_cuda and x.dim() == 4 and x.shape[1] == 3 and x.size(0) % groups == 0):
            return False
        if x.shape[2] % 32 or x.shape[3] % 32 or len({e.training for e in encs}) != 1:
            return False
        per_group = x.size(0) // groups
        return (per_group * (x.shape[2] // 32) * (x.shape[3] // 32)) % 128 == 0

    def __call__(self, x: torch.Tensor, groups: int = 1, stem_cols=None):
        if not self.can_run(x, groups):
            raise ops._lib.IrfdError(f"EncoderGroup: shape {tuple(x.shape)} / modes cannot run as one grouped pass")
        encs = self.encoders
        params = [p for e in encs for p in e._flat_params()]
        recorded = torch.is_grad_enabled() and (x.requires_grad or any(p.requires_grad for p in params))
        if not encs[0].training:
            if recorded:
                raise ops._lib.IrfdError("EncoderGroup: eval-mode passes with autograd run per encoder")
            return _group_inference(self, x, stem_cols)
        return _EncoderGroupFn.apply(x, self, groups, stem_cols, recorded, *params)
```

### speak_hack_b200/ops.py

```python
from __future__ import annotations

import ctypes
import os
import weakref
from typing import Optional

import torch

from . import _lib

BF16 = torch.bfloat16
F32 = torch.float32

EPI_PLAIN, EPI_STATS, EPI_STYLE = 0, 1, 2
PACK_FPROP, PACK_DGRAD, PACK_DCOL, PACK_FLAT = 0, 1, 2, 3

launch_count = 0


def _stream() -> int:
    return torch.cuda.current_stream().cuda_stream


def _ptr(t: Optional[torch.Tensor]) -> Optional[int]:
    return None if t is None else t.data_ptr()


def _chk(t: torch.Tensor, dtype, name: str) -> None:
    if not t.is_cuda:
        raise _lib.IrfdError(f"{name}: expected a CUDA tensor (the IRFD hot path has no CPU fallback)")
    if t.dtype != dtype:
        raise _lib.IrfdError(f"{name}: expected dtype {dtype}, got {t.dtype}")
    if not t.is_contiguous():
        raise _lib.IrfdError(f"{name}: expected a contiguous tensor")


def _call(name: str, *args, launches: int = 1) -> None:
    global launch_count
    rc = getattr(_lib.load(), name)(*args)
    _lib.check(rc, name)
    launch_count += launches


_gemm_timing = None


def gemm_timing_begin() -> None:
    global _gemm_timing
    _gemm_timing = []


def gemm_timing_end():
    global _gemm_timing
    rec, _gemm_timing = _gemm_timing or [], None
    fam = {}
    for name, flops, nbytes, e0, e1 in rec:
        f = fam.setdefault(name, {"name": name, "ms": 0.0, "flops": 0.0, "bytes": 0.0, "launches": 0, "records": []})
        ms = e0.elapsed_time(e1)
        f["ms"] += ms
        f["flops"] += flops
        f["bytes"] += nbytes
        f["launches"] += 1
        f["records"].append((ms, flops, nbytes))
    return fam


class _timed:

    def __init__(self, name, flops, nbytes=0.0):
        self.name, self.flops, self.nbytes = name, flops, nbytes

    def __enter__(self):
        if _gemm_timing is not None:
            self.e0 = torch.cuda.Event(enable_timing=True)
            self.e1 = torch.cuda.Event(enable_timing=True)
            self.e0.record()
        return self

    def __exit__(self, *exc):
        if _gemm_timing is not None:
            self.e1.record()
            _gemm_timing.append((self.name, self.flops, self.nbytes, self.e0, self.e1))
        return False


use_side_stream = os.environ.get("IRFD_SIDE_STREAM", "1") != "0"
_side_streams = {}


class SideStream:
    def __init__(self, device):
        self.stream = torch.cuda.Stream(device)
        self.keep = []
        self.active = False

    def launch(self, fn, *keep):
        if not use_side_stream:
            fn()
            return
        ev = torch.cuda.Event()
        ev.record()
        self.stream.wait_event(ev)
        with torch.cuda.stream(self.stream):
            fn()
        self.keep.extend(keep)
        self.active = True

    def join(self):
        if self.active:
            torch.cuda.current_stream().wait_stream(self.stream)
            self.active = False
        self.keep.clear()


def side_stream(device) -> SideStream:
    key = device.index if device.index is not None else torch.cuda.current_device()
    s = _side_streams.get(key)
    if s is None:
        s = _side_streams[key] = SideStream(device)
    return s


_workspace = {}
_workspace_retired = []


def workspace(nbytes: int, device) -> torch.Tensor:
    key = (device.type, device.index, torch.cuda.current_stream(device).cuda_stream if device.type == "cuda" else 0)
    buf = _workspace.get(key)
    if buf is None or buf.numel() < nbytes:
        if buf is not None:
            _workspace_retired.append(buf)
        buf = torch.empty(max(int(nbytes), 1 << 22), dtype=torch.uint8, device=device)
        _workspace[key] = buf
    return buf


def conv_gemm(x, wk, ksize, mode=EPI_PLAIN, bias=None, nw=None, noise=None, sp1=None, s1=None, force_block_n=0,
              split_y=False):
    lib = _lib.load()
    _chk(x, BF16, "x")
    _chk(wk, BF16, "wk")
    n, h, w, cin = x.shape
    cout = wk.shape[0]
    if wk.shape[1] != ksize * ksize * cin:
        raise _lib.IrfdError(f"wk shape {tuple(wk.shape)} does not match ksize={ksize}, cin={cin}")
    out = torch.empty((n, h, w, cout), dtype=BF16, device=x.device)
    out2 = torch.empty_like(out) if mode == EPI_STYLE else None
    ssum = ssq = None
    if mode == EPI_STATS:
        mt = lib.irfd_conv_gemm_m_tiles(n, h, w)
        ssum = torch.empty((mt, cout), dtype=F32, device=x.device)
        ssq = torch.empty((mt, cout), dtype=F32, device=x.device)
    for t, nm in ((bias, "bias"), (nw, "nw"), (noise, "noise"), (sp1, "sp1"), (s1, "s1")):
        if t is not None:
            _chk(t, F32, nm)
    m = n * h * w
    nbytes = 2.0 * m * cin + 2.0 * m * cout * (2 if mode == EPI_STYLE else 1) + 2.0 * cin * cout * ksize * ksize
    out_lo = torch.empty_like(out) if (mode == EPI_STYLE and split_y) else None
    with _timed("conv_gemm_kernel (tcgen05 fprop/dgrad)", 2.0 * m * cout * cin * ksize * ksize, nbytes):
        if out_lo is not None:
            _call("irfd_conv_gemm_style_split", x.data_ptr(), n, h, w, cin, wk.data_ptr(), cout, ksize, out.data_ptr(),
                  out2.data_ptr(), out_lo.data_ptr(), _ptr(bias), _ptr(nw), _ptr(noise), _ptr(sp1), _ptr(s1),
                  force_block_n, _stream())
        else:
            _call("irfd_conv_gemm", x.data_ptr(), n, h, w, cin, wk.data_ptr(), cout, ksize, out.data_ptr(), _ptr(out2),
                  mode, _ptr(bias), _ptr(nw), _ptr(noise), _ptr(sp1), _ptr(s1), _ptr(ssum), _ptr(ssq), force_block_n,
                  _stream())
    if mode == EPI_STATS:
        return out, ssum, ssq
    if mode == EPI_STYLE:
        return (out, out2, out_lo) if split_y else (out, out2)
    return out


def conv_gemm_affine(x, wk, ksize, scale, shift, res=None, relu=True, force_block_n=0):
    _chk(x, BF16, "x")
    _chk(wk, BF16, "wk")
    n, h, w, cin = x.shape
    cout = wk.shape[0]
    out = torch.empty((n, h, w, cout), dtype=BF16, device=x.device)
    if res is not None:
        _chk(res, BF16, "res")
        if res.numel() != out.numel():
            raise _lib.IrfdError("conv_gemm_affine: residual shape mismatch")
    m = n * h * w
    nbytes = 2.0 * m * cin + 2.0 * m * cout * (2 if res is not None else 1) + 2.0 * cin * cout * ksize * ksize
    with _timed("conv_gemm_kernel (tcgen05 fprop/dgrad)", 2.0 * m * cout * cin * ksize * ksize, nbytes):
        _call("irfd_conv_gemm_affine", x.data_ptr(), n, h, w, cin, wk.data_ptr(), cout, ksize, out.data_ptr(),
              scale.data_ptr(), shift.data_ptr(), _ptr(res), int(relu), force_block_n, _stream())
    return out


def conv_gemm_grouped(x, wk, ksize, mode=EPI_PLAIN, wgroups=3, a_shared=False, rows=None, force_block_n=0):
    lib = _lib.load()
    _chk(x, BF16, "x")
    _chk(wk, BF16, "wk")
    if wk.shape[0] % wgroups:
        raise _lib.IrfdError(f"conv_gemm_grouped: {wk.shape[0]} weight rows do not split into {wgroups} groups")
    cout = wk.shape[0] // wgroups
    if a_shared:
        m_g, cin = x.shape
        n, h, w = 1, 1, m_g * wgroups
        out = torch.empty((m_g * wgroups, cout), dtype=BF16, device=x.device)
    else:
        n, h, w, cin = x.shape
        out = torch.empty((n, h, w, cout), dtype=BF16, device=x.device)
    if wk.shape[1] != ksize * ksize * cin:
        raise _lib.IrfdError(f"wk shape {tuple(wk.shape)} does not match ksize={ksize}, cin={cin}")
    m = n * h * w
    ssum = ssq = None
    if mode == EPI_STATS:
        mt = lib.irfd_conv_gemm_m_tiles(n, h, w)
        ssum = torch.empty((mt, cout), dtype=F32, device=x.device)
        ssq = torch.empty((mt, cout), dtype=F32, device=x.device)
    nbytes = 2.0 * m * cin / (wgroups if a_shared else 1) + 2.0 * m * cout + 2.0 * wgroups * cin * cout * ksize * ksize
    with _timed("conv_gemm_kernel (tcgen05 fprop/dgrad)", 2.0 * m * cout * cin * ksize * ksize, nbytes):
        _call("irfd_conv_gemm_grouped", x.data_ptr(), n, h, w, cin, wk.data_ptr(), cout, ksize, out.data_ptr(), mode,
              _ptr(ssum), _ptr(ssq), wgroups, 1 if a_shared else 0, force_block_n, _stream())
    if mode == EPI_STATS:
        return out, ssum, ssq
    return out


def conv_gemm_bnbwd_grouped(dy, wk, ksize, z, mean, rstd, gammas, betas, stat_groups, force_block_n=0):
    lib = _lib.load()
    _chk(dy, BF16, "dy")
    _chk(wk, BF16, "wk")
    _chk(z, BF16, "z")
    wgroups = len(gammas)
    n, h, w, cin = dy.shape
    cout = wk.shape[0] // wgroups
    if wk.shape[0] % wgroups or wk.shape[1] != ksize * ksize * cin or z.shape != (n, h, w, cout):
        raise _lib.IrfdError(f"conv_gemm_bnbwd_grouped: wk {tuple(wk.shape)} / z {tuple(z.shape)} do not match dy "
                             f"{tuple(dy.shape)}, ksize={ksize}, {wgroups} groups")
    m = n * h * w
    out = torch.empty((n, h, w, cout), dtype=BF16, device=dy.device)
    partial = torch.empty((lib.irfd_conv_gemm_m_tiles(n, h, w), 2, cout), dtype=F32, device=dy.device)
    nbytes = 2.0 * m * cin + 2 * 2.0 * m * cout + 2.0 * wgroups * cin * cout * ksize * ksize
    with _timed("conv_gemm_kernel (tcgen05 fprop/dgrad)", 2.0 * m * cout * cin * ksize * ksize, nbytes):
        _call("irfd_conv_gemm_bnbwd_grouped", dy.data_ptr(), n, h, w, cin, wk.data_ptr(), cout, ksize, out.data_ptr(),
              z.data_ptr(), mean.data_ptr(), rstd.data_ptr(), _ptr_array(gammas), _ptr_array(betas), partial.data_ptr(),
              stat_groups, wgroups, force_block_n, _stream())
    return out, partial


def conv_gemm_bnbwd_res_grouped(dy, wk, ksize, z, mean, rstd, g2, bits, stat_groups, wgroups=3, force_block_n=0):
    lib = _lib.load()
    _chk(dy, BF16, "dy")
    _chk(wk, BF16, "wk")
    _chk(z, BF16, "z")
    _chk(g2, BF16, "g2")
    n, h, w, cin = dy.shape
    cout = wk.shape[0] // wgroups
    m = n * h * w
    if (wk.shape[0] % wgroups or wk.shape[1] != ksize * ksize * cin or z.shape != (n, h, w, cout) or g2.shape != z.shape
            or bits.dtype != torch.uint8 or bits.numel() != m * cout // 8):
        raise _lib.IrfdError(f"conv_gemm_bnbwd_res_grouped: wk {tuple(wk.shape)} / z {tuple(z.shape)} / g2 "
                             f"{tuple(g2.shape)} / bits {tuple(bits.shape)} do not match dy {tuple(dy.shape)}")
    out = torch.empty((n, h, w, cout), dtype=BF16, device=dy.device)
    partial = torch.empty((lib.irfd_conv_gemm_m_tiles(n, h, w), 2, cout), dtype=F32, device=dy.device)
    nbytes = 2.0 * m * cin + (3 + 1.0 / 16) * 2.0 * m * cout + 2.0 * wgroups * cin * cout * ksize * ksize
    with _timed("conv_gemm_kernel (tcgen05 fprop/dgrad)", 2.0 * m * cout * cin * ksize * ksize, nbytes):
        _call("irfd_conv_gemm_bnbwd_res_grouped", dy.data_ptr(), n, h, w, cin, wk.data_ptr(), cout, ksize, out.data_ptr(),
              z.data_ptr(), mean.data_ptr(), rstd.data_ptr(), g2.data_ptr(), bits.data_ptr(), partial.data_ptr(),
              stat_groups, wgroups, force_block_n, _stream())
    return out, partial


def conv_gemm_affine_grouped(x, wk, ksize, scale, shift, res=None, relu=True, wgroups=3, a_shared=False,
                             force_block_n=0):
    _chk(x, BF16, "x")
    _chk(wk, BF16, "wk")
    _chk(scale, F32, "scale")
    _chk(shift, F32, "shift")
    cout = wk.shape[0] // wgroups
    if a_shared:
        m_g, cin = x.shape
        n, h, w = 1, 1, m_g * wgroups
        out = torch.empty((m_g * wgroups, cout), dtype=BF16, device=x.device)
    else:
        n, h, w, cin = x.shape
        out = torch.empty((n, h, w, cout), dtype=BF16, device=x.device)
    if scale.numel() != wgroups * cout or shift.numel() != wgroups * cout:
        raise _lib.IrfdError("conv_gemm_affine_grouped: scale/shift must be [wgroups, Cout]")
    if res is not None:
        _chk(res, BF16, "res")
        if res.numel() != out.numel():
            raise _lib.IrfdError("conv_gemm_affine_grouped: residual shape mismatch")
    m = n * h * w
    nbytes = (2.0 * m * cin / (wgroups if a_shared else 1) + 2.0 * m * cout * (2 if res is not None else 1)
              + 2.0 * wgroups * cin * cout * ksize * ksize)
    with _timed("conv_gemm_kernel (tcgen05 fprop/dgrad)", 2.0 * m * cout * cin * ksize * ksize, nbytes):
        _call("irfd_conv_gemm_affine_grouped", x.data_ptr(), n, h, w, cin, wk.data_ptr(), cout, ksize, out.data_ptr(),
              scale.data_ptr(), shift.data_ptr(), _ptr(res), int(relu), wgroups, 1 if a_shared else 0, force_block_n,
              _stream())
    return out


def bn_eval_affine(bn):
    c = bn.weight.numel()
    scale = torch.empty(c, dtype=F32, device=bn.weight.device)
    shift = torch.empty(c, dtype=F32, device=bn.weight.device)
    _call("irfd_bn_eval_affine", bn.running_mean.data_ptr(), bn.running_var.data_ptr(), bn.weight.data_ptr(),
          bn.bias.data_ptr(), float(bn.eps), scale.data_ptr(), shift.data_ptr(), c, _stream())
    return scale, shift


def gemm_rows(a2d, wk, mode=EPI_PLAIN):
    m, k = a2d.shape
    r = conv_gemm(a2d.view(1, 1, m, k), wk, 1, mode)
    if mode == EPI_STATS:
        return r[0].view(m, -1), r[1], r[2]
    return r.view(m, -1)


def conv_wgrad(x, dy, ksize, dw=None, beta=0.0, reduce_cin=0, reduce_taps=0, out_shape=None):
    lib = _lib.load()
    _chk(x, BF16, "x")
    _chk(dy, BF16, "dy")
    n, h, w, cin = x.shape
    cout = dy.shape[-1]
    if dw is None:
        shape = out_shape if out_shape is not None else (cout, cin, ksize, ksize)
        dw = torch.empty(shape, dtype=F32, device=x.device)
        beta = 0.0
    _chk(dw, F32, "dw")
    need = lib.irfd_wgrad_workspace_bytes(n, h, w, cin, cout, ksize)
    ws = workspace(need, x.device)
    nbytes = 2.0 * n * h * w * (cin + cout) + 4.0 * cin * cout * ksize * ksize
    with _timed("wgrad_gemm_kernel (tcgen05 split-K + reduce)", 2.0 * n * h * w * cout * cin * ksize * ksize, nbytes):
        _call("irfd_conv_wgrad", x.data_ptr(), dy.data_ptr(), n, h, w, cin, cout, ksize, dw.data_ptr(), beta,
              reduce_cin, reduce_taps, ws.data_ptr(), ws.numel(), _stream(), launches=2)
    return dw


def conv_wgrad_grouped(x, dy, ksize, dws, x_shared=False, reduce_cin=0, reduce_taps=0):
    lib = _lib.load()
    _chk(x, BF16, "x")
    _chk(dy, BF16, "dy")
    groups = len(dws)
    for d in dws:
        _chk(d, F32, "dw")
    cin, cout = x.shape[-1], dy.shape[-1]
    if dy.dim() == 4 and not x_shared:
        n, h, w = dy.shape[0], dy.shape[1], dy.shape[2]
    else:
        n, h, w = 1, 1, dy.numel() // cout
    need = lib.irfd_wgrad_workspace_bytes_grouped(n, h, w, cin, cout, ksize, groups)
    if need < 0:
        raise _lib.IrfdError(f"conv_wgrad_grouped: {groups} groups not supported")
    ws = workspace(need, x.device)
    m = n * h * w
    nbytes = 2.0 * m * cout + 2.0 * m * cin / (groups if x_shared else 1) + 4.0 * groups * cin * cout * ksize * ksize
    with _timed("wgrad_gemm_kernel (tcgen05 split-K + reduce)", 2.0 * m * cout * cin * ksize * ksize, nbytes):
        _call("irfd_conv_wgrad_grouped", x.data_ptr(), dy.data_ptr(), n, h, w, cin, cout, ksize, _ptr_array(dws), 0.0,
              reduce_cin, reduce_taps, groups, 1 if x_shared else 0, ws.data_ptr(), ws.numel(), _stream(), launches=2)
    return dws


_pack_cache = {}


def invalidate_packed(params) -> None:
    ptrs = {p.data_ptr() for p in params}
    def hit(k0):
        return any(q in ptrs for q in k0) if isinstance(k0, tuple) else k0 in ptrs

    for key in [k for k in _pack_cache if hit(k[0])]:
        del _pack_cache[key]


def pack_conv_weight(w: torch.Tensor, mode: int, kpad: int = 0) -> torch.Tensor:
    key = (w.data_ptr(), mode, kpad, tuple(w.shape))
    hit = _pack_cache.get(key)
    if hit is not None and hit[0] == w._version and hit[2]() is w:
        return hit[1]
    packed = _pack_conv_weight(w, mode, kpad)
    _pack_cache[key] = (w._version, packed, weakref.ref(w))
    return packed


def prepack_conv_weights(items, side) -> int:
    todo = []
    for w, mode in items:
        key = (w.data_ptr(), mode, 0, tuple(w.shape))
        hit = _pack_cache.get(key)
        if hit is not None and hit[0] == w._version and hit[2]() is w:
            continue
        o, i, kh, kw = w.shape
        shape = (o, kh * kw * i) if mode == PACK_FPROP else (i, kh * kw * o)
        dst = torch.empty(shape, dtype=BF16, device=w.device)
        todo.append((w, mode, dst))
        _pack_cache[key] = (w._version, dst, weakref.ref(w))
    if todo:
        side.launch(lambda: [_pack_conv_weight(w, m, out=d) for w, m, d in todo], *[d for _, _, d in todo])
    return len(todo)


def pack_conv_weights_stacked(ws, mode: int, kpad: int = 0) -> torch.Tensor:
    key = (tuple(w.data_ptr() for w in ws), mode, kpad, tuple(ws[0].shape))
    vers = tuple(w._version for w in ws)
    hit = _pack_cache.get(key)
    if hit is not None and hit[0] == vers and all(r() is w for r, w in zip(hit[2], ws)):
        return hit[1]
    o, i, kh, kw = ws[0].shape
    taps = kh * kw
    rows, cols = {PACK_FPROP: (o, taps * i), PACK_DGRAD: (i, taps * o), PACK_DCOL: (taps * i, o)}.get(mode, (o, kpad))
    dst = torch.empty((len(ws) * rows, cols), dtype=BF16, device=ws[0].device)
    for e, w in enumerate(ws):
        _pack_conv_weight(w, mode, kpad, out=dst[e * rows: (e + 1) * rows])
    _pack_cache[key] = (vers, dst, [weakref.ref(w) for w in ws])
    return dst


def _pack_conv_weight(w: torch.Tensor, mode: int, kpad: int = 0, out: Optional[torch.Tensor] = None) -> torch.Tensor:
    _chk(w, F32, "w")
    o, i, kh, kw = w.shape
    taps = kh * kw
    if mode == PACK_FPROP:
        shape = (o, taps * i)
    elif mode == PACK_DGRAD:
        shape = (i, taps * o)
    elif mode == PACK_DCOL:
        shape = (taps * i, o)
    else:
        shape = (o, kpad)
    dst = out if out is not None else torch.empty(shape, dtype=BF16, device=w.device)
    if tuple(dst.shape) != tuple(shape) or not dst.is_contiguous():
        raise _lib.IrfdError(f"_pack_conv_weight: destination {tuple(dst.shape)} != {tuple(shape)}")
    _call("irfd_pack_conv_weight", w.data_ptr(), dst.data_ptr(), o, i, taps, mode, kpad, _stream())
    return dst


def bn_finalize(ssum, ssq, count, eps, momentum, running_mean=None, running_var=None, running_updates=1, groups=1):
    tiles, c = ssum.shape
    if tiles % groups:
        raise _lib.IrfdError(f"bn_finalize: {tiles} tiles do not split into {groups} groups")
    shape = (c,) if groups == 1 else (groups, c)
    mean = torch.empty(shape, dtype=F32, device=ssum.device)
    rstd = torch.empty(shape, dtype=F32, device=ssum.device)
    _call("irfd_bn_finalize", ssum.data_ptr(), ssq.data_ptr(), tiles // groups, c, int(count), eps, momentum,
          mean.data_ptr(), rstd.data_ptr(), _ptr(running_mean), _ptr(running_var), running_updates, groups, _stream())
    return mean, rstd


def bn_running_update(mean, rstd, eps, count, momentum, running_mean, running_var):
    _call("irfd_bn_running_update", mean.data_ptr(), rstd.data_ptr(), eps, int(count), momentum,
          running_mean.data_ptr(), running_var.data_ptr(), mean.numel(), _stream())


def bn_eval_rstd(running_var, eps):
    rstd = torch.empty_like(running_var)
    _call("irfd_bn_eval_rstd", running_var.data_ptr(), eps, rstd.data_ptr(), running_var.numel(), _stream())
    return rstd


def bn_apply(z, mean, rstd, gamma, beta, res=None, bn2=None, relu=True, groups=1):
    _chk(z, BF16, "z")
    c = z.shape[-1]
    rows = z.numel() // c
    out = torch.empty_like(z)
    m2 = r2 = g2 = b2 = None
    if bn2 is not None:
        m2, r2, g2, b2 = bn2
    _call("irfd_bn_apply", z.data_ptr(), mean.data_ptr(), rstd.data_ptr(), gamma.data_ptr(), beta.data_ptr(),
          _ptr(res), _ptr(m2), _ptr(r2), _ptr(g2), _ptr(b2), out.data_ptr(), rows, c, 1 if relu else 0, groups,
          _stream())
    return out


def bn_backward(g1, g2, act, z, mean, rstd, gamma, want_g_out=False, batch_stats=True, groups=1, beta=None):
    lib = _lib.load()
    c = z.shape[-1]
    rows = z.numel() // c
    dz = torch.empty_like(z)
    g_out = torch.empty_like(z) if want_g_out else None
    dgamma = torch.empty(c, dtype=F32, device=z.device)
    dbeta = torch.empty(c, dtype=F32, device=z.device)
    ws = workspace(lib.irfd_bn_bwd_workspace_bytes(rows, c, groups), z.device)
    nbytes = _bn_bwd_bytes(rows, c, g2 is not None, 1.0 if act is not None else 0.0, want_g_out)
    with _timed("bn_backward (reduce+finalize+apply, HBM)", nbytes):
        _bn_backward_call(g1, g2, act, z, mean, rstd, gamma, beta, dz, g_out, dgamma, dbeta, batch_stats, rows, c, groups,
                          ws)
    if want_g_out:
        return dz, dgamma, dbeta, g_out
    return dz, dgamma, dbeta


def _bn_backward_call(g1, g2, act, z, mean, rstd, gamma, beta, dz, g_out, dgamma, dbeta, batch_stats, rows, c, groups, ws):
    _call("irfd_bn_backward", g1.data_ptr(), _ptr(g2), _ptr(act), z.data_ptr(), mean.data_ptr(), rstd.data_ptr(),
          gamma.data_ptr(), _ptr(beta), dz.data_ptr(), _ptr(g_out), dgamma.data_ptr(), dbeta.data_ptr(), 0.0,
          1 if batch_stats else 0, rows, c, groups,
          ws.data_ptr(), ws.numel(), _stream(), launches=3)


def _ptr_array(tensors):
    if tensors is None:
        return None
    return (ctypes.c_void_p * len(tensors))(*[None if t is None else t.data_ptr() for t in tensors])


def bn_eval_affine_sets(bns):
    c = bns[0].weight.numel()
    dev = bns[0].weight.device
    scale = torch.empty((len(bns), c), dtype=F32, device=dev)
    shift = torch.empty((len(bns), c), dtype=F32, device=dev)
    _call("irfd_bn_eval_affine_sets", _ptr_array([b.running_mean for b in bns]), _ptr_array([b.running_var for b in bns]),
          _ptr_array([b.weight for b in bns]), _ptr_array([b.bias for b in bns]), float(bns[0].eps), scale.data_ptr(),
          shift.data_ptr(), c, len(bns), _stream())
    return scale, shift


def bn_finalize_sets(ssum, ssq, count, eps, momentum, running_means, running_vars, running_updates, groups, nsets):
    tiles, c = ssum.shape
    tot = groups * nsets
    if tiles % tot:
        raise _lib.IrfdError(f"bn_finalize_sets: {tiles} tiles do not split into {nsets} sets x {groups} groups")
    mean = torch.empty((tot, c), dtype=F32, device=ssum.device)
    rstd = torch.empty((tot, c), dtype=F32, device=ssum.device)
    _call("irfd_bn_finalize_sets", ssum.data_ptr(), ssq.data_ptr(), tiles // tot, c, int(count), eps, momentum,
          mean.data_ptr(), rstd.data_ptr(), _ptr_array(running_means), _ptr_array(running_vars), running_updates, groups,
          nsets, _stream())
    return mean, rstd


def bn_apply_sets(z, mean, rstd, gammas, betas, res=None, bn2=None, relu=True, groups=1, want_mask=False):
    _chk(z, BF16, "z")
    c = z.shape[-1]
    rows = z.numel() // c
    out = torch.empty_like(z)
    bits = torch.empty((rows, c // 8), dtype=torch.uint8, device=z.device) if want_mask else None
    m2 = r2 = g2 = b2 = None
    if bn2 is not None:
        m2, r2, g2, b2 = bn2
    _call("irfd_bn_apply_sets", z.data_ptr(), mean.data_ptr(), rstd.data_ptr(), _ptr_array(gammas), _ptr_array(betas),
          _ptr(res), _ptr(m2), _ptr(r2), _ptr_array(g2) if g2 is not None else _ptr_array([None] * len(gammas)),
          _ptr_array(b2) if b2 is not None else _ptr_array([None] * len(gammas)), out.data_ptr(), _ptr(bits), rows, c,
          1 if relu else 0, groups, len(gammas), _stream())
    return (out, bits) if want_mask else out


def _bn_bwd_bytes(rows, c, has_g2, mask_units, want_g_out):
    n_in = 2 + (1 if has_g2 else 0) + mask_units
    if want_g_out:
        return 2.0 * rows * c * (n_in + 1 + 3)
    return 2.0 * rows * c * (2 * n_in + 1)


def bn_backward_sets(g1, g2, act, z, mean, rstd, gammas, betas=None, dgammas=None, dbetas=None, want_g_out=False,
                     batch_stats=True, groups=1, act_bits=None):
    lib = _lib.load()
    c = z.shape[-1]
    rows = z.numel() // c
    nsets = len(gammas)
    dz = torch.empty_like(z)
    g_out = torch.empty_like(z) if want_g_out else None
    if dgammas is None:
        dg_all = torch.empty((nsets, c), dtype=F32, device=z.device)
        db_all = torch.empty((nsets, c), dtype=F32, device=z.device)
        dgammas, dbetas = list(dg_all.unbind(0)), list(db_all.unbind(0))
    ws = workspace(lib.irfd_bn_bwd_workspace_bytes(rows, c, groups), z.device)
    if act_bits is not None and act is not None:
        raise _lib.IrfdError("bn_backward_sets: pass act or act_bits, not both")
    mask_units = 1.0 if act is not None else (1.0 / 16 if act_bits is not None else 0.0)
    nbytes = _bn_bwd_bytes(rows, c, g2 is not None, mask_units, want_g_out)
    with _timed("bn_backward (reduce+finalize+apply, HBM)", nbytes):
        _call("irfd_bn_backward_sets", g1.data_ptr(), _ptr(g2), _ptr(act if act_bits is None else act_bits),
              0 if act_bits is None else 1, z.data_ptr(), mean.data_ptr(),
              rstd.data_ptr(), _ptr_array(gammas), _ptr_array(betas) if betas is not None else None, dz.data_ptr(),
              _ptr(g_out), _ptr_array(dgammas), _ptr_array(dbetas), 0.0, 1 if batch_stats else 0, rows, c, groups, nsets,
              ws.data_ptr(), ws.numel(), _stream(), launches=3)
    if want_g_out:
        return dz, dgammas, dbetas, g_out
    return dz, dgammas, dbetas


def bn_backward_finish_sets(g, z, mean, rstd, gammas, partial, dgammas=None, dbetas=None, batch_stats=True, groups=1):
    c = z.shape[-1]
    rows = z.numel() // c
    nsets = len(gammas)
    dz = torch.empty_like(z)
    if dgammas is None:
        dg_all = torch.empty((nsets, c), dtype=F32, device=z.device)
        db_all = torch.empty((nsets, c), dtype=F32, device=z.device)
        dgammas, dbetas = list(dg_all.unbind(0)), list(db_all.unbind(0))
    if partial.shape[0] % groups:
        raise _lib.IrfdError("bn_backward_finish_sets: partial rows do not split into the statistic groups")
    ws = workspace(2 * groups * c * 4, z.device)
    with _timed("bn_backward (reduce+finalize+apply, HBM)", 2.0 * rows * c * 3):
        _call("irfd_bn_backward_finish_sets", g.data_ptr(), z.data_ptr(), mean.data_ptr(), rstd.data_ptr(),
              _ptr_array(gammas), dz.data_ptr(), _ptr_array(dgammas), _ptr_array(dbetas), 0.0, 1 if batch_stats else 0,
              rows, c, groups, nsets, partial.data_ptr(), partial.shape[0] // groups, ws.data_ptr(), ws.numel(), _stream(),
              launches=2)
    return dz, dgammas, dbetas


def im2col_stem(x: torch.Tensor, kpad: int = 192) -> torch.Tensor:
    _chk(x, F32, "x")
    n, c, h, w = x.shape
    if c != 3:
        raise _lib.IrfdError("im2col_stem expects 3 input channels")
    col = torch.empty((n * (h // 2) * (w // 2), kpad), dtype=BF16, device=x.device)
    _call("irfd_im2col_stem", x.data_ptr(), col.data_ptr(), n, h, w, kpad, _stream())
    return col


def im2col_3x3s2(a: torch.Tensor) -> torch.Tensor:
    n, h, w, c = a.shape
    col = torch.empty((n * (h // 2) * (w // 2), 9 * c), dtype=BF16, device=a.device)
    _call("irfd_im2col_3x3s2", a.data_ptr(), col.data_ptr(), n, h, w, c, _stream())
    return col


def col2im_3x3s2(dcol: torch.Tensor, n, h, w, c) -> torch.Tensor:
    dx = torch.empty((n, h, w, c), dtype=BF16, device=dcol.device)
    _call("irfd_col2im_3x3s2", dcol.data_ptr(), dx.data_ptr(), n, h, w, c, _stream())
    return dx


def subsample2(a: torch.Tensor) -> torch.Tensor:
    n, h, w, c = a.shape
    out = torch.empty((n, h // 2, w // 2, c), dtype=BF16, device=a.device)
    _call("irfd_subsample2", a.data_ptr(), out.data_ptr(), n, h, w, c, _stream())
    return out


def scatter_add_s2(a: Optional[torch.Tensor], b: torch.Tensor) -> torch.Tensor:
    n, h2, w2, c = b.shape
    out = torch.empty((n, h2 * 2, w2 * 2, c), dtype=BF16, device=b.device)
    _call("irfd_scatter_add_s2", _ptr(a), b.data_ptr(), out.data_ptr(), n, h2 * 2, w2 * 2, c, _stream())
    return out


def maxpool_fwd(a: torch.Tensor):
    n, h, w, c = a.shape
    out = torch.empty((n, h // 2, w // 2, c), dtype=BF16, device=a.device)
    arg = torch.empty((n, h // 2, w // 2, c), dtype=torch.uint8, device=a.device)
    _call("irfd_maxpool_fwd", a.data_ptr(), out.data_ptr(), arg.data_ptr(), n, h, w, c, _stream())
    return out, arg


def maxpool_bwd(dout: torch.Tensor, arg: torch.Tensor, dout2: Optional[torch.Tensor] = None) -> torch.Tensor:
    n, h2, w2, c = dout.shape
    dx = torch.empty((n, h2 * 2, w2 * 2, c), dtype=BF16, device=dout.device)
    _call("irfd_maxpool_bwd", dout.data_ptr(), _ptr(dout2), arg.data_ptr(), dx.data_ptr(), n, h2 * 2, w2 * 2, c,
          _stream())
    return dx


def avgpool_fwd(a: torch.Tensor) -> torch.Tensor:
    n, h, w, c = a.shape
    out = torch.empty((n, c), dtype=F32, device=a.device)
    _call("irfd_avgpool_fwd", a.data_ptr(), out.data_ptr(), n, h * w, c, _stream())
    return out


def avgpool_bwd(dfeat: torch.Tensor, h: int, w: int) -> torch.Tensor:
    _chk(dfeat, F32, "dfeat")
    n, c = dfeat.shape
# ... 292 lines not shown
```

Measured before the change: 915.6.

## Read stride-2 convolution inputs through parity tensor-map views instead of im2col

Adds a 5D parity-split TMA descriptor so stride-2 3x3 and 1x1 downsample convolutions, plus their weight gradients, load directly from the full-resolution NHWC input. This removes the im2col, subsample and scatter-add staging copies. The downsample dgrad now adds its result in place into the strided positions of d_in through the epilogue with a 5D TMA store. The cost is that these spatial paths turn off the halo and cluster/2-SM modes, and the in-place add rounds through bf16 twice.

```diff
diff --git a/include/irfd_b200.h b/include/irfd_b200.h
--- a/include/irfd_b200.h
+++ b/include/irfd_b200.h
@@ -35,6 +35,11 @@
 int irfd_conv_gemm_affine_grouped(const void* x, int n, int h, int w, int cin, const void* wk, int cout, int ksize,
                                   void* out, const float* scale, const float* shift, const void* res, int relu,
                                   int wgroups, int a_shared, int force_block_n, irfd_stream_t stream);
+int irfd_conv_gemm_s2_grouped(const void* x, int n, int h, int w, int cin, const void* wk, int cout, int ksize,
+                              void* out, int mode, float* stat_sum, float* stat_sq, const float* scale,
+                              const float* shift, int relu, int wgroups, int force_block_n, irfd_stream_t stream);
+int irfd_conv_gemm_dgrad_add_s2_grouped(const void* dy, int n, int h, int w, int cin, const void* wk, int cout,
+                                        void* d_in, int wgroups, int force_block_n, irfd_stream_t stream);
 
 int irfd_conv_gemm_affine(const void* x, int n, int h, int w, int cin, const void* wk, int cout, int ksize, void* out,
                           const float* scale, const float* shift, const void* res, int relu, int force_block_n,
@@ -48,6 +53,10 @@
 int irfd_conv_wgrad_grouped(const void* x, const void* dy, int n, int h, int w, int cin, int cout, int ksize,
                             float* const* dw, float beta, int reduce_cin, int reduce_taps, int groups, int x_shared,
                             void* workspace, long long workspace_bytes, irfd_stream_t stream);
+long long irfd_wgrad_workspace_bytes_s2_grouped(int n, int h, int w, int cin, int cout, int ksize, int groups);
+int irfd_conv_wgrad_s2_grouped(const void* x, const void* dy, int n, int h, int w, int cin, int cout, int ksize,
+                               float* const* dw, int groups, void* workspace, long long workspace_bytes,
+                               irfd_stream_t stream);
 
 int irfd_bn_finalize(const float* psum, const float* psq, int tiles, int c, long long count, float eps, float momentum,
                      float* mean, float* rstd, float* running_mean, float* running_var, int running_updates,
diff --git a/speak_hack_b200/csrc/conv_gemm.cu b/speak_hack_b200/csrc/conv_gemm.cu
--- a/speak_hack_b200/csrc/conv_gemm.cu
+++ b/speak_hack_b200/csrc/conv_gemm.cu
@@ -33,6 +33,8 @@
   const float* bn_beta[4];
   int sg_tiles;
   int warp_epi;
+  int s2;
+  const __nv_bfloat16* add_s2;
 };
 
 constexpr int kNumThreads = 320;
@@ -327,6 +329,13 @@
   const int ng0 = n_tile * BLOCK_N;
   const int pg0 = (m_tile / p.wg_tiles) * p.N_total + ng0;
   const int row = m0 + q * 32 + lane;
+  const __nv_bfloat16* add_row = nullptr;
+  if constexpr (MODE == EPI_PLAIN) {
+    if (p.add_s2 != nullptr) {
+      const int ow = row % p.W, oh = (row / p.W) % p.H, img = row / (p.W * p.H);
+      add_row = p.add_s2 + (((size_t)img * 2 * p.H + 2 * oh) * 2 * p.W + 2 * ow) * p.N_total;
+    }
+  }
   uint8_t* slabs = stg_base + e * 2 * kSlabBytes;
   float* wvec = vec + e * 128;
   const int first = (h - (int)chunk_counter) & 1;
@@ -395,6 +404,19 @@
 #pragma unroll
         for (int t = 0; t < 8; ++t)
           o[t] = p.relu == 1 ? fmaxf(o[t], 0.f) : (p.relu == 2 ? (o[t] > 0.f ? o[t] : 0.2f * o[t]) : o[t]);
+      }
+      if constexpr (MODE == EPI_PLAIN) {
+        if (add_row != nullptr) {
+          const uint4 u = *reinterpret_cast<const uint4*>(add_row + cg0 + j * 8);
+          const uint32_t uw[4] = {u.x, u.y, u.z, u.w};
+#pragma unroll
+          for (int t = 0; t < 4; ++t) {
+            const float2 mine = unpack_bf16x2(pack_bf16x2(o[2 * t], o[2 * t + 1]));
+            const float2 old = unpack_bf16x2(uw[t]);
+            o[2 * t] = old.x + mine.x;
+            o[2 * t + 1] = old.y + mine.y;
+          }
+        }
       }
       uint4 pk;
       pk.x = pack_bf16x2(o[0], o[1]);
@@ -458,7 +480,12 @@
     fence_proxy_async_smem();
     __syncwarp();
     if (lane == 0) {
-      tma_store_2d(map_slab, slab, cg0, m0 + q * 32);
+      if (MODE == EPI_PLAIN && add_row != nullptr) {
+        const int r0 = m0 + q * 32;
+        tma_store_5d(map_slab, slab, cg0, r0 % p.W, 0, (r0 / p.W) % p.H, r0 / (p.W * p.H));
+      } else {
+        tma_store_2d(map_slab, slab, cg0, m0 + q * 32);
+      }
       tma_store_commit();
     }
     if constexpr (kSums) {
@@ -564,7 +591,14 @@
           for (int ch = 0; ch < p.cin_chunks; ++ch) {
             mbar_wait(&empty_bar[stage], phase ^ 1);
             uint8_t* sa = smem + stage * Cfg::STAGE_BYTES;
-            if (MMA2) {
+            if (p.s2) {
+              if (elect_one_sync()) {
+                mbar_expect_tx(&full_bar[stage], Cfg::STAGE_BYTES);
+                tma_load_5d(sa, &map_a, &full_bar[stage], (dw & 1) * p.cin_chunks * 64 + ch * 64, w0 + (dw >> 1), dh & 1,
+                            h0 + (dh >> 1), n0);
+                tma_load_2d(sa + Cfg::A_BYTES, &map_b, &full_bar[stage], (tap * p.cin_chunks + ch) * 64, b_row);
+              }
+            } else if (MMA2) {
               if (elect_one_sync()) {
                 if (crank == 0) mbar_expect_tx(&full_bar[stage], 2 * (Cfg::A_BYTES + Cfg::B_BYTES / 2));
                 tma_load_4d_2sm(sa, &map_a, &full_bar[stage], ch * 64, w0 + dw, h0 + dh, n0);
@@ -1002,12 +1036,21 @@
                           void* out2, void* out_lo, int mode, const float* bias, const float* nw, const float* noise,
                           const float* sp1, const float* s1, float* stat_sum, float* stat_sq, const void* res, int relu,
                           int force_block_n, cudaStream_t stream, int wgroups = 1, int a_shared = 0,
-                          const BnBwdFold* fold = nullptr) {
+                          const BnBwdFold* fold = nullptr, int stride = 1, void* add_s2 = nullptr) {
   IRFD_CHECK_ARG(x && wk && out, "conv_gemm: null pointer");
   IRFD_CHECK_ARG(ksize == 1 || ksize == 3, "conv_gemm: ksize must be 1 or 3 (got %d)", ksize);
   IRFD_CHECK_ARG(cin % 64 == 0 && cin > 0, "conv_gemm: Cin must be a multiple of 64 (got %d)", cin);
   IRFD_CHECK_ARG(cout % 64 == 0 && cout > 0, "conv_gemm: Cout must be a multiple of 64 (got %d)", cout);
   IRFD_CHECK_ARG(mode >= 0 && mode <= 5, "conv_gemm: bad mode %d", mode);
+  IRFD_CHECK_ARG(stride == 1 || (stride == 2 && h % 2 == 0 && w % 2 == 0 && mode != EPI_STYLE && !a_shared),
+                 "conv_gemm: stride 2 needs even H, W (got %dx%d), no STYLE epilogue and no shared A operand", h, w);
+  IRFD_CHECK_ARG(!add_s2 || (mode == EPI_PLAIN && ksize == 1 && stride == 1 && !bias),
+                 "conv_gemm: the in-place parity add is a plain 1x1 stride-1 GEMM");
+  const int ih = h, iw = w;
+  if (stride == 2) {
+    h /= 2;
+    w /= 2;
+  }
   const long long m_total_ll = (long long)n * h * w;
   IRFD_CHECK_ARG(m_total_ll > 0 && m_total_ll < (1ll << 31) - 256, "conv_gemm: bad pixel count");
   const int m_total = (int)m_total_ll;
@@ -1018,14 +1061,15 @@
   IRFD_CHECK_ARG(!a_shared || (ksize == 1 && wgroups > 1), "conv_gemm: a shared A operand needs ksize 1 and groups > 1");
 
   int H = h, W = w, NB = n;
-  if (ksize == 1) {
+  const bool spatial = stride == 2 || add_s2 != nullptr;
+  if (ksize == 1 && !spatial) {
     H = 1;
     W = a_shared ? m_total / wgroups : m_total;
     NB = 1;
   }
   int tw, th, tn;
   if (W >= 128) {
-    IRFD_CHECK_ARG(ksize == 1 || W % 128 == 0, "conv_gemm: W=%d must be a multiple of 128", W);
+    IRFD_CHECK_ARG((ksize == 1 && !spatial) || W % 128 == 0, "conv_gemm: W=%d must be a multiple of 128", W);
     tw = 128; th = 1; tn = 1;
   } else {
     IRFD_CHECK_ARG(128 % W == 0, "conv_gemm: W=%d must divide 128", W);
@@ -1063,6 +1107,12 @@
   }
   if (mode == EPI_STATS) IRFD_CHECK_ARG(stat_sum && stat_sq, "conv_gemm: STATS mode needs stat buffers");
   a.warp_epi = (mode != EPI_STYLE && m_total % 128 == 0 && warp_epi_mode() != 0) ? 1 : 0;
+  a.s2 = stride == 2;
+  a.add_s2 = reinterpret_cast<const __nv_bfloat16*>(add_s2);
+  if (add_s2) {
+    IRFD_CHECK_ARG(m_total % 128 == 0, "conv_gemm: the in-place parity add needs whole 128-pixel tiles");
+    a.warp_epi = 1;
+  }
   a.bn_z = nullptr;
   a.bn_mean = a.bn_rstd = nullptr;
   for (int i = 0; i < 4; ++i) a.bn_gamma[i] = a.bn_beta[i] = nullptr;
@@ -1107,13 +1157,13 @@
   IRFD_CHECK_ARG((block_n == 64 || block_n == 128 || block_n == 256) && cout % block_n == 0,
                  "conv_gemm: BLOCK_N %d incompatible with Cout %d", block_n, cout);
   const int hmode = halo_mode();
-  const bool use_halo = hmode != 0 && mode != EPI_BNBWD && mode != EPI_BNBWD_RES && wgroups == 1 && ksize == 3 && W % 128 == 0 && H % 2 == 0 &&
+  const bool use_halo = hmode != 0 && !spatial && mode != EPI_BNBWD && mode != EPI_BNBWD_RES && wgroups == 1 && ksize == 3 && W % 128 == 0 && H % 2 == 0 &&
                         (cout == 64 || cout == 128) &&
                         (force_block_n == 0 || force_block_n == cout);
   if (use_halo) block_n = cout;
   a.num_n_tiles = cout / block_n;
   int cluster = 1;
-  if (!use_halo && (cluster_mode() != 0 || mma2_mode() != 0) && block_n >= 128 && a.num_m_tiles % 2 == 0 &&
+  if (!use_halo && !spatial && (cluster_mode() != 0 || mma2_mode() != 0) && block_n >= 128 && a.num_m_tiles % 2 == 0 &&
       (wgroups == 1 || a.wg_tiles % 2 == 0) && (a.a_mod_tiles == 0 || a.a_mod_tiles % 2 == 0))
     cluster = (mma2_mode() != 0 && a.warp_epi && (mode == EPI_PLAIN || mode == EPI_STATS || mode == EPI_BNBWD)) ? 3 : 2;
 
@@ -1127,7 +1177,8 @@
       box[2] = kHaloRows;
       box[3] = 1;
     }
-    int rc = make_tmap_bf16(&ma, x, 4, dims, str, box, true);
+    int rc = stride == 2 ? make_tmap_parity_bf16(&ma, x, n, ih, iw, cin, tw, th, tn)
+                         : make_tmap_bf16(&ma, x, 4, dims, str, box, true);
     if (rc) return rc;
   }
   {
@@ -1146,6 +1197,10 @@
     if (rc) return rc;
     if (mode == EPI_STYLE) {
       rc = make_tmap_bf16(&mo2, out2 ? out2 : out, 2, dims, str, box, true);
+    } else if (add_s2) {
+      int sw, sh, sn;
+      IRFD_CHECK_ARG(pixel_box(h, w, 32, &sw, &sh, &sn), "conv_gemm: %dx%d does not tile into 32-pixel slabs", h, w);
+      rc = make_tmap_parity_bf16(&mo2, add_s2, n, 2 * h, 2 * w, cout, sw, sh, sn);
     } else {
       const uint32_t slab_box[2] = {64, 32};
       rc = make_tmap_bf16(&mo2, out, 2, dims, str, slab_box, true);
@@ -1239,3 +1294,23 @@
   return conv_gemm_impl(x, n, h, w, cin, wk, cout, ksize, out, nullptr, nullptr, EPI_AFFINE, shift, scale, nullptr, nullptr,
                         nullptr, nullptr, nullptr, res, relu, force_block_n, stream);
 }
+
+extern "C" int irfd_conv_gemm_s2_grouped(const void* x, int n, int h, int w, int cin, const void* wk, int cout,
+                                         int ksize, void* out, int mode, float* stat_sum, float* stat_sq,
+                                         const float* scale, const float* shift, int relu, int wgroups,
+                                         int force_block_n, cudaStream_t stream) {
+  IRFD_CHECK_ARG(mode == EPI_PLAIN || mode == EPI_STATS || mode == EPI_AFFINE,
+                 "conv_gemm_s2_grouped: mode must be 0 (plain), 1 (stats) or 3 (affine)");
+  return conv_gemm_impl(x, n, h, w, cin, wk, cout, ksize, out, nullptr, nullptr, mode,
+                        mode == EPI_AFFINE ? shift : nullptr, mode == EPI_AFFINE ? scale : nullptr, nullptr, nullptr,
+                        nullptr, stat_sum, stat_sq, nullptr, relu, force_block_n, stream, wgroups, 0, nullptr, 2);
+}
+
+extern "C" int irfd_conv_gemm_dgrad_add_s2_grouped(const void* dy, int n, int h, int w, int cin, const void* wk,
+                                                   int cout, void* d_in, int wgroups, int force_block_n,
+                                                   cudaStream_t stream) {
+  IRFD_CHECK_ARG(d_in != nullptr, "conv_gemm_dgrad_add_s2: null pointer");
+  return conv_gemm_impl(dy, n, h, w, cin, wk, cout, 1, d_in, nullptr, nullptr, EPI_PLAIN, nullptr, nullptr, nullptr,
+                        nullptr, nullptr, nullptr, nullptr, nullptr, 0, force_block_n, stream, wgroups, 0, nullptr, 1,
+                        d_in);
+}
diff --git a/speak_hack_b200/csrc/host_util.cu b/speak_hack_b200/csrc/host_util.cu
--- a/speak_hack_b200/csrc/host_util.cu
+++ b/speak_hack_b200/csrc/host_util.cu
@@ -69,6 +69,29 @@
   return IRFD_OK;
 }
 
+int make_tmap_parity_bf16(CUtensorMap* out, const void* x, int n, int h, int w, int c, int tw, int th, int tn) {
+  const uint64_t dims[5] = {2ull * c, (uint64_t)w / 2, 2, (uint64_t)h / 2, (uint64_t)n};
+  const uint64_t str[4] = {2ull * c * 2, (uint64_t)w * c * 2, 2ull * w * c * 2, (uint64_t)h * w * c * 2};
+  const uint32_t box[5] = {64, (uint32_t)tw, 1, (uint32_t)th, (uint32_t)tn};
+  return make_tmap_bf16(out, x, 5, dims, str, box, true);
+}
+
+bool pixel_box(int h, int w, int npix, int* tw, int* th, int* tn) {
+  if (w >= npix) {
+    *tw = npix; *th = 1; *tn = 1;
+    return w % npix == 0;
+  }
+  if (npix % w) return false;
+  *tw = w;
+  const int rows = npix / w;
+  if (h >= rows) {
+    *th = rows; *tn = 1;
+    return h % rows == 0;
+  }
+  *th = h; *tn = rows / h;
+  return rows % h == 0;
+}
+
 }
 
 extern "C" const char* irfd_last_error(void) { return irfd::g_last_error; }
diff --git a/speak_hack_b200/csrc/host_util.h b/speak_hack_b200/csrc/host_util.h
--- a/speak_hack_b200/csrc/host_util.h
+++ b/speak_hack_b200/csrc/host_util.h
@@ -19,6 +19,10 @@
 int make_tmap_bf16(CUtensorMap* out, const void* base, int rank, const uint64_t* dims, const uint64_t* strides_bytes,
                    const uint32_t* box, bool swizzle128);
 
+int make_tmap_parity_bf16(CUtensorMap* out, const void* x, int n, int h, int w, int c, int tw, int th, int tn);
+
+bool pixel_box(int h, int w, int npix, int* tw, int* th, int* tn);
+
 void prefer_max_shared_carveout(const void* kernel);
 
 #define IRFD_CHECK_ARG(cond, ...)            \
diff --git a/speak_hack_b200/csrc/ptx.cuh b/speak_hack_b200/csrc/ptx.cuh
--- a/speak_hack_b200/csrc/ptx.cuh
+++ b/speak_hack_b200/csrc/ptx.cuh
@@ -98,6 +98,21 @@
       "l"(reinterpret_cast<uint64_t>(m)), "r"(smem_u32(bar)), "r"(c0), "r"(c1), "r"(c2), "r"(c3)
       : "memory");
 }
+__device__ __forceinline__ void tma_load_5d(void* dst, const CUtensorMap* m, uint64_t* bar, int c0, int c1, int c2,
+                                            int c3, int c4) {
+  asm volatile(
+      "cp.async.bulk.tensor.5d.shared::cluster.global.tile.mbarrier::complete_tx::bytes [%0], [%1, {%3, %4, %5, %6, "
+      "%7}], [%2];" ::"r"(smem_u32(dst)),
+      "l"(reinterpret_cast<uint64_t>(m)), "r"(smem_u32(bar)), "r"(c0), "r"(c1), "r"(c2), "r"(c3), "r"(c4)
+      : "memory");
+}
+__device__ __forceinline__ void tma_store_5d(const CUtensorMap* m, const void* src, int c0, int c1, int c2, int c3,
+                                             int c4) {
+  asm volatile("cp.async.bulk.tensor.5d.global.shared::cta.tile.bulk_group [%0, {%2, %3, %4, %5, %6}], [%1];" ::"l"(
+                   reinterpret_cast<uint64_t>(m)),
+               "r"(smem_u32(src)), "r"(c0), "r"(c1), "r"(c2), "r"(c3), "r"(c4)
+               : "memory");
+}
 __device__ __forceinline__ void tma_store_2d(const CUtensorMap* m, const void* src, int c0, int c1) {
   asm volatile("cp.async.bulk.tensor.2d.global.shared::cta.tile.bulk_group [%0, {%2, %3}], [%1];" ::"l"(
                    reinterpret_cast<uint64_t>(m)),
diff --git a/speak_hack_b200/csrc/wgrad_gemm.cu b/speak_hack_b200/csrc/wgrad_gemm.cu
--- a/speak_hack_b200/csrc/wgrad_gemm.cu
+++ b/speak_hack_b200/csrc/wgrad_gemm.cu
@@ -13,6 +13,7 @@
   int H, W;
   float* partial;
   int groups, x_shared;
+  int s2;
 };
 
 constexpr int kMaxWgGroups = 4;
@@ -110,8 +111,15 @@
       uint8_t* sb = sa + Cfg::A_BYTES;
       if (elect_one_sync()) {
         mbar_expect_tx(&full_bar[stage], Cfg::STAGE_BYTES);
-        tma_load_4d(sa, &map_x, &full_bar[stage], c0[0], w0 + dw[0], h0 + dh[0], n0);
-        tma_load_4d(sa + 8192, &map_x, &full_bar[stage], c0[1], w0 + dw[1], h0 + dh[1], n0);
+        if (p.s2) {
+#pragma unroll
+          for (int i = 0; i < 2; ++i)
+            tma_load_5d(sa + i * 8192, &map_x, &full_bar[stage], (dw[i] & 1) * p.cin_chunks * 64 + c0[i],
+                        w0 + (dw[i] >> 1), dh[i] & 1, h0 + (dh[i] >> 1), n0);
+        } else {
+          tma_load_4d(sa, &map_x, &full_bar[stage], c0[0], w0 + dw[0], h0 + dh[0], n0);
+          tma_load_4d(sa + 8192, &map_x, &full_bar[stage], c0[1], w0 + dw[1], h0 + dh[1], n0);
+        }
 #pragma unroll
         for (int j = 0; j < BLOCK_N / 64; ++j)
           tma_load_2d(sb + j * 8192, &map_dy, &full_bar[stage], n_tile * BLOCK_N + j * 64, p0);
@@ -558,9 +566,9 @@
 
 using namespace irfd;
 
-static long long wgrad_ws_bytes(int n_g, int h, int w, int cin, int cout, int ksize, int groups) {
+static long long wgrad_ws_bytes(int n_g, int h, int w, int cin, int cout, int ksize, int groups, int stride = 1) {
   WgHaloArgs ha;
-  if (wgrad_halo_plan(n_g, h, w, cin, cout, ksize, &ha, groups))
+  if (stride == 1 && wgrad_halo_plan(n_g, h, w, cin, cout, ksize, &ha, groups))
     return (long long)groups * ha.splits * ha.K_total * ha.N_total * 4;
   WgradArgs a;
   int bn;
@@ -580,15 +588,16 @@
 
 static int conv_wgrad_impl(const void* x, const void* dy, int n, int h, int w, int cin, int cout, int ksize,
                            const WgDst& dws, int groups, int x_shared, float beta, int reduce_cin, int reduce_taps,
-                           void* workspace, long long workspace_bytes, cudaStream_t stream) {
+                           void* workspace, long long workspace_bytes, cudaStream_t stream, int stride = 1) {
   IRFD_CHECK_ARG(x && dy && workspace, "conv_wgrad: null pointer");
   IRFD_CHECK_ARG(ksize == 1 || ksize == 3, "conv_wgrad: ksize must be 1 or 3");
   IRFD_CHECK_ARG(cin % 64 == 0 && cout % 64 == 0, "conv_wgrad: channels must be multiples of 64");
   IRFD_CHECK_ARG(!x_shared || ksize == 1, "conv_wgrad: a shared x operand needs ksize 1");
+  IRFD_CHECK_ARG(stride == 1 || (stride == 2 && !x_shared), "conv_wgrad: stride 2 reads a stacked NHWC x");
   const long long m_group = (long long)n * h * w;
   IRFD_CHECK_ARG(groups == 1 || m_group % 128 == 0, "conv_wgrad: grouped launches need 128-pixel multiples per group");
   WgHaloArgs ha;
-  if (!x_shared && wgrad_halo_plan(n, h, w, cin, cout, ksize, &ha, groups)) {
+  if (!x_shared && stride == 1 && wgrad_halo_plan(n, h, w, cin, cout, ksize, &ha, groups)) {
     IRFD_CHECK_ARG(workspace_bytes >= (long long)groups * ha.splits * ha.K_total * ha.N_total * 4,
                    "conv_wgrad: workspace too small");
     ha.partial = reinterpret_cast<float*>(workspace);
@@ -627,18 +636,19 @@
   int block_n;
   wgrad_plan(n, h, w, cin, cout, ksize, &a, &block_n, groups);
   a.x_shared = x_shared;
+  a.s2 = stride == 2;
   IRFD_CHECK_ARG(workspace_bytes >= (long long)groups * a.splits * a.K_total * a.N_total * 4,
                  "conv_wgrad: workspace too small");
   a.partial = reinterpret_cast<float*>(workspace);
 
   const int xg = x_shared ? 1 : groups;
   int H = h, W = w, NB = n * xg;
-  if (ksize == 1) {
+  if (ksize == 1 && stride == 1) {
     H = 1; W = (int)(m_group * xg); NB = 1;
   }
   int tw, th, tn;
   if (W >= 64) {
-    IRFD_CHECK_ARG(ksize == 1 || W % 64 == 0, "conv_wgrad: W=%d must be a multiple of 64", W);
+    IRFD_CHECK_ARG((ksize == 1 && stride == 1) || W % 64 == 0, "conv_wgrad: W=%d must be a multiple of 64", W);
     tw = 64; th = 1; tn = 1;
   } else {
     IRFD_CHECK_ARG(64 % W == 0, "conv_wgrad: W=%d must divide 64", W);
@@ -659,7 +669,8 @@
     const uint64_t dims[4] = {(uint64_t)cin, (uint64_t)W, (uint64_t)H, (uint64_t)NB};
     const uint64_t str[3] = {(uint64_t)cin * 2, (uint64_t)W * cin * 2, (uint64_t)H * W * cin * 2};
     const uint32_t box[4] = {64, (uint32_t)tw, (uint32_t)th, (uint32_t)tn};
-    int rc = make_tmap_bf16(&mx, x, 4, dims, str, box, true);
+    int rc = stride == 2 ? make_tmap_parity_bf16(&mx, x, NB, 2 * H, 2 * W, cin, tw, th, tn)
+                         : make_tmap_bf16(&mx, x, 4, dims, str, box, true);
     if (rc) return rc;
   }
   {
@@ -709,3 +720,21 @@
   return conv_wgrad_impl(x, dy, ng, hg, wg, cin, cout, ksize, dws, groups, x_shared, beta, reduce_cin, reduce_taps,
                          workspace, workspace_bytes, stream);
 }
+
+extern "C" long long irfd_wgrad_workspace_bytes_s2_grouped(int n, int h, int w, int cin, int cout, int ksize,
+                                                           int groups) {
+  if (groups < 1 || groups > kMaxWgGroups || n % groups) return -1;
+  return wgrad_ws_bytes(n / groups, h, w, cin, cout, ksize, groups, 2);
+}
+
+extern "C" int irfd_conv_wgrad_s2_grouped(const void* x, const void* dy, int n, int h, int w, int cin, int cout,
+                                          int ksize, float* const* dw, int groups, void* workspace,
+                                          long long workspace_bytes, cudaStream_t stream) {
+  IRFD_CHECK_ARG(dw != nullptr && groups >= 1 && groups <= kMaxWgGroups && n % groups == 0,
+                 "conv_wgrad_s2_grouped: 1..4 groups of whole images");
+  WgDst dws;
+  for (int i = 0; i < kMaxWgGroups; ++i) dws.p[i] = i < groups ? dw[i] : nullptr;
+  for (int i = 0; i < groups; ++i) IRFD_CHECK_ARG(dws.p[i] != nullptr, "conv_wgrad_s2_grouped: null gradient pointer");
+  return conv_wgrad_impl(x, dy, n / groups, h, w, cin, cout, ksize, dws, groups, 0, 0.f, 0, 0, workspace,
+                         workspace_bytes, stream, 2);
+}
diff --git a/speak_hack_b200/encoder_group.py b/speak_hack_b200/encoder_group.py
--- a/speak_hack_b200/encoder_group.py
+++ b/speak_hack_b200/encoder_group.py
@@ -12,6 +12,19 @@
 
 fold_bn_reduce = os.environ.get("IRFD_BN_FOLD", "1") != "0"
 fold_bn3_reduce = os.environ.get("IRFD_BN3_FOLD", "0") != "0"
+s2_views = os.environ.get("IRFD_S2_VIEWS", "1") != "0"
+
+
+def _use_views(h, w):
+    if not s2_views:
+        return False
+    ho, wo = h // 2, w // 2
+    if wo >= 128:
+        return wo % 128 == 0
+    if 128 % wo:
+        return False
+    rows = 128 // wo
+    return ho % rows == 0 if ho >= rows else rows % ho == 0
 
 
 def _stack_pack(convs, mode, kpad=0):
@@ -46,17 +59,23 @@
             planes = a1.shape[-1]
             sc, sh = ops.bn_eval_affine_sets([b.bn2 for b in blks])
             wk2 = _stack_pack([b.conv2 for b in blks], ops.PACK_FPROP)
+            views = blks[0].stride == 2 and _use_views(hh, ww)
             if blks[0].stride == 1:
                 a2 = ops.conv_gemm_affine_grouped(a1, wk2, 3, sc, sh, relu=True, wgroups=E)
+            elif views:
+                a2 = ops.conv_gemm_s2_grouped(a1, wk2, 3, 3, sc, sh, relu=True, wgroups=E)
             else:
                 col2 = ops.im2col_3x3s2(a1)
                 a2 = ops.conv_gemm_affine_grouped(col2.view(1, 1, col2.shape[0], 9 * planes), wk2, 1, sc, sh, relu=True,
                                                   wgroups=E).view(nb, hh // 2, ww // 2, planes)
             if blks[0].downsample is not None:
-                xs = ops.subsample2(cur) if blks[0].stride == 2 else cur
                 sc, sh = ops.bn_eval_affine_sets([b.downsample[1] for b in blks])
-                idn = ops.conv_gemm_affine_grouped(xs, _stack_pack([b.downsample[0] for b in blks], ops.PACK_FPROP), 1,
-                                                   sc, sh, relu=False, wgroups=E)
+                wkd = _stack_pack([b.downsample[0] for b in blks], ops.PACK_FPROP)
+                if views:
+                    idn = ops.conv_gemm_s2_grouped(cur, wkd, 1, 3, sc, sh, relu=False, wgroups=E)
+                else:
+                    xs = ops.subsample2(cur) if blks[0].stride == 2 else cur
+                    idn = ops.conv_gemm_affine_grouped(xs, wkd, 1, sc, sh, relu=False, wgroups=E)
             else:
                 idn = cur
             sc, sh = ops.bn_eval_affine_sets([b.bn3 for b in blks])
@@ -112,9 +131,13 @@
                 planes = a1.shape[-1]
                 wk2 = _stack_pack([b.conv2 for b in blks], ops.PACK_FPROP)
                 col2 = None
+                views = blks[0].stride == 2 and _use_views(hh, ww)
                 if blks[0].stride == 1:
                     z2, s, q = ops.conv_gemm_grouped(a1, wk2, 3, ops.EPI_STATS, wgroups=E)
                     ho, wo = hh, ww
+                elif views:
+                    ho, wo = hh // 2, ww // 2
+                    z2, s, q = ops.conv_gemm_s2_grouped(a1, wk2, 3, ops.EPI_STATS, wgroups=E)
                 else:
                     col2 = ops.im2col_3x3s2(a1)
                     ho, wo = hh // 2, ww // 2
@@ -130,9 +153,12 @@
                 st3 = stats(bn3, s, q, nb * ho * wo)
                 xs = zd = std = None
                 if blks[0].downsample is not None:
-                    xs = ops.subsample2(xin) if blks[0].stride == 2 else xin
-                    zd, s, q = ops.conv_gemm_grouped(xs, _stack_pack([b.downsample[0] for b in blks], ops.PACK_FPROP), 1,
-                                                     ops.EPI_STATS, wgroups=E)
+                    wkd = _stack_pack([b.downsample[0] for b in blks], ops.PACK_FPROP)
+                    if views:
+                        zd, s, q = ops.conv_gemm_s2_grouped(xin, wkd, 1, ops.EPI_STATS, wgroups=E)
+                    else:
+                        xs = ops.subsample2(xin) if blks[0].stride == 2 else xin
+                        zd, s, q = ops.conv_gemm_grouped(xs, wkd, 1, ops.EPI_STATS, wgroups=E)
                     dbn = [b.downsample[1] for b in blks]
                     std = stats(dbn, s, q, nb * ho * wo)
                     out = apply(z3, st3, bn3, res=zd, want_mask=recorded,
@@ -192,9 +218,10 @@
 
         side = ops.side_stream(dfeat.device)
 
-        def wgrad(convs, xx, dy, ksize, **kw):
+        def wgrad(convs, xx, dy, ksize, s2=False, **kw):
             dws = [tgt(c.weight) for c in convs]
-            side.launch(lambda: ops.conv_wgrad_grouped(xx, dy, ksize, dws, **kw), xx, dy, *dws)
+            fn = ops.conv_wgrad_s2_grouped if s2 else ops.conv_wgrad_grouped
+            side.launch(lambda: fn(xx, dy, ksize, dws, **kw), xx, dy, *dws)
 
         cur_li = None
         pre = None
@@ -226,7 +253,10 @@
                 m2 = dz2.numel() // planes
                 dcol = ops.conv_gemm_grouped(dz2.view(1, 1, m2, planes),
                                              _stack_pack([b.conv2 for b in blks], ops.PACK_DCOL), 1, wgroups=E)
-                wgrad([b.conv2 for b in blks], col2, dz2.view(m2, planes), 1, reduce_cin=planes, reduce_taps=9)
+                if col2 is None:
+                    wgrad([b.conv2 for b in blks], a1, dz2, 3, s2=True)
+                else:
+                    wgrad([b.conv2 for b in blks], col2, dz2.view(m2, planes), 1, reduce_cin=planes, reduce_taps=9)
                 d_a1 = ops.col2im_3x3s2(dcol.view(m2, 9 * planes), nb, hh, ww, planes)
                 dz1 = bn_bwd([b.bn1 for b in blks], st1, d_a1, None, a1, z1, mask_from_z=True)
             wk1 = _stack_pack([b.conv1 for b in blks], ops.PACK_DGRAD)
@@ -240,13 +270,18 @@
             wgrad([b.conv1 for b in blks], xin, dz1, 1)
             if blks[0].downsample is not None:
                 dzd = bn_bwd([b.downsample[1] for b in blks], std, gmask, None, None, zd)
-                d_xs = ops.conv_gemm_grouped(dzd, _stack_pack([b.downsample[0] for b in blks], ops.PACK_DGRAD), 1,
-                                             wgroups=E)
-                wgrad([b.downsample[0] for b in blks], xs, dzd, 1)
-                if blks[0].stride == 2:
-                    g, g2 = ops.scatter_add_s2(d_in, d_xs), None
-                else:
-                    g, g2 = d_in, d_xs
+                wkd = _stack_pack([b.downsample[0] for b in blks], ops.PACK_DGRAD)
+                if xs is None:
+                    ops.conv_gemm_dgrad_add_s2_grouped(dzd, wkd, d_in, wgroups=E)
+                    wgrad([b.downsample[0] for b in blks], xin, dzd, 1, s2=True)
+                    g, g2 = d_in, None
+                else:
+                    d_xs = ops.conv_gemm_grouped(dzd, wkd, 1, wgroups=E)
+                    wgrad([b.downsample[0] for b in blks], xs, dzd, 1)
+                    if blks[0].stride == 2:
+                        g, g2 = ops.scatter_add_s2(d_in, d_xs), None
+                    else:
+                        g, g2 = d_in, d_xs
             else:
                 g, g2 = d_in, gmask
         if cb is not None and cur_li is not None:
diff --git a/speak_hack_b200/ops.py b/speak_hack_b200/ops.py
--- a/speak_hack_b200/ops.py
+++ b/speak_hack_b200/ops.py
@@ -298,6 +298,54 @@
     return out
 
 
+def conv_gemm_s2_grouped(x, wk, ksize, mode=EPI_PLAIN, scale=None, shift=None, relu=True, wgroups=3, force_block_n=0):
+    lib = _lib.load()
+    _chk(x, BF16, "x")
+    _chk(wk, BF16, "wk")
+    n, h, w, cin = x.shape
+    cout = wk.shape[0] // wgroups
+    if wk.shape[0] % wgroups or wk.shape[1] != ksize * ksize * cin:
+        raise _lib.IrfdError(f"conv_gemm_s2_grouped: wk {tuple(wk.shape)} does not match ksize={ksize}, cin={cin}, "
+                             f"{wgroups} groups")
+    ho, wo = h // 2, w // 2
+    out = torch.empty((n, ho, wo, cout), dtype=BF16, device=x.device)
+    ssum = ssq = None
+    if mode == EPI_STATS:
+        mt = lib.irfd_conv_gemm_m_tiles(n, ho, wo)
+        ssum = torch.empty((mt, cout), dtype=F32, device=x.device)
+        ssq = torch.empty((mt, cout), dtype=F32, device=x.device)
+    if mode == 3:
+        _chk(scale, F32, "scale")
+        _chk(shift, F32, "shift")
+        if scale.numel() != wgroups * cout or shift.numel() != wgroups * cout:
+            raise _lib.IrfdError("conv_gemm_s2_grouped: scale/shift must be [wgroups, Cout]")
+    m = n * ho * wo
+    nbytes = 2.0 * n * h * w * cin + 2.0 * m * cout + 2.0 * wgroups * cin * cout * ksize * ksize
+    with _timed("conv_gemm_kernel (tcgen05 fprop/dgrad)", 2.0 * m * cout * cin * ksize * ksize, nbytes):
+        _call("irfd_conv_gemm_s2_grouped", x.data_ptr(), n, h, w, cin, wk.data_ptr(), cout, ksize, out.data_ptr(), mode,
+              _ptr(ssum), _ptr(ssq), _ptr(scale), _ptr(shift), int(relu), wgroups, force_block_n, _stream())
+    if mode == EPI_STATS:
+        return out, ssum, ssq
+    return out
+
+
+def conv_gemm_dgrad_add_s2_grouped(dy, wk, d_in, wgroups=3, force_block_n=0):
+    _chk(dy, BF16, "dy")
+    _chk(wk, BF16, "wk")
+    _chk(d_in, BF16, "d_in")
+    n, h, w, cin = dy.shape
+    cout = wk.shape[0] // wgroups
+    if wk.shape[0] % wgroups or wk.shape[1] != cin or d_in.shape != (n, 2 * h, 2 * w, cout):
+        raise _lib.IrfdError(f"conv_gemm_dgrad_add_s2_grouped: wk {tuple(wk.shape)} / d_in {tuple(d_in.shape)} do not "
+                             f"match dy {tuple(dy.shape)}")
+    m = n * h * w
+    nbytes = 2.0 * m * cin + 2 * 2.0 * m * cout + 2.0 * wgroups * cin * cout
+    with _timed("conv_gemm_kernel (tcgen05 fprop/dgrad)", 2.0 * m * cout * cin, nbytes):
+        _call("irfd_conv_gemm_dgrad_add_s2_grouped", dy.data_ptr(), n, h, w, cin, wk.data_ptr(), cout, d_in.data_ptr(),
+              wgroups, force_block_n, _stream())
+    return d_in
+
+
 def bn_eval_affine(bn):
     c = bn.weight.numel()
     scale = torch.empty(c, dtype=F32, device=bn.weight.device)
@@ -356,6 +404,29 @@
     with _timed("wgrad_gemm_kernel (tcgen05 split-K + reduce)", 2.0 * m * cout * cin * ksize * ksize, nbytes):
         _call("irfd_conv_wgrad_grouped", x.data_ptr(), dy.data_ptr(), n, h, w, cin, cout, ksize, _ptr_array(dws), 0.0,
               reduce_cin, reduce_taps, groups, 1 if x_shared else 0, ws.data_ptr(), ws.numel(), _stream(), launches=2)
+    return dws
+
+
+def conv_wgrad_s2_grouped(x, dy, ksize, dws):
+    lib = _lib.load()
+    _chk(x, BF16, "x")
+    _chk(dy, BF16, "dy")
+    groups = len(dws)
+    for d in dws:
+        _chk(d, F32, "dw")
+    n, h, w, cout = dy.shape
+    cin = x.shape[-1]
+    if x.shape != (n, 2 * h, 2 * w, cin):
+        raise _lib.IrfdError(f"conv_wgrad_s2_grouped: x {tuple(x.shape)} is not the stride-2 input of dy {tuple(dy.shape)}")
+    need = lib.irfd_wgrad_workspace_bytes_s2_grouped(n, h, w, cin, cout, ksize, groups)
+    if need < 0:
+        raise _lib.IrfdError(f"conv_wgrad_s2_grouped: {groups} groups of {n} images not supported")
+    ws = workspace(need, x.device)
+    m = n * h * w
+    nbytes = 2.0 * m * cout + 2.0 * x.numel() + 4.0 * groups * cin * cout * ksize * ksize
+    with _timed("wgrad_gemm_kernel (tcgen05 split-K + reduce)", 2.0 * m * cout * cin * ksize * ksize, nbytes):
+        _call("irfd_conv_wgrad_s2_grouped", x.data_ptr(), dy.data_ptr(), n, h, w, cin, cout, ksize, _ptr_array(dws),
+              groups, ws.data_ptr(), ws.numel(), _stream(), launches=2)
     return dws
 
 
```

New measurement: 928.2 (median of 6 runs). 1.4% higher.
